# pcodec/pcodec

Hardware: AMD Instinct MI355X
Metric: encode+decode GB/s (uncompressed) per chunk, u64/f64 2^18-elem (higher is better)
Workload: dtype u64

## Files before the change

### include/pco_gfx.h

```cpp
#ifndef PCO_GFX_H
#define PCO_GFX_H

#include <stddef.h>
#include <stdint.h>

#if defined(__cplusplus)
extern "C" {
#endif


#define PCO_TYPE_U32 1
#define PCO_TYPE_U64 2
#define PCO_TYPE_I32 3
#define PCO_TYPE_I64 4
#define PCO_TYPE_F32 5
#define PCO_TYPE_F64 6
#define PCO_TYPE_U16 7
#define PCO_TYPE_I16 8
#define PCO_TYPE_F16 9
#define PCO_TYPE_U8 10
#define PCO_TYPE_I8 11

typedef enum PcoError {
  PcoSuccess,
  PcoInvalidType,
  PcoCompressionError,
  PcoDecompressionError,
} PcoError;

typedef struct PcoChunkConfig {
  unsigned int compression_level;
  size_t max_page_n;
} PcoChunkConfig;

size_t pco_standalone_guarantee_file_size(size_t n, unsigned char dtype);

enum PcoError pco_standalone_simple_compress_into(const void* nums, size_t n, unsigned char dtype,
                                                  const struct PcoChunkConfig* config, void* dst,
                                                  size_t dst_cap, size_t* n_written);

enum PcoError pco_standalone_simple_decompress_into(const void* compressed, size_t compressed_len,
                                                    unsigned char dtype, void* dst, size_t dst_cap,
                                                    size_t* n_written);


enum PcoModeSpecKind {
  PCO_MODE_AUTO = 0,
  PCO_MODE_CLASSIC = 1,
  PCO_MODE_TRY_FLOAT_MULT = 2,
  PCO_MODE_TRY_FLOAT_QUANT = 3,
  PCO_MODE_TRY_INT_MULT = 4,
  PCO_MODE_TRY_DICT = 5,
};
enum PcoDeltaSpecKind {
  PCO_DELTA_AUTO = 0,
  PCO_DELTA_NOOP = 1,
  PCO_DELTA_TRY_CONSECUTIVE = 2,
  PCO_DELTA_TRY_LOOKBACK = 3,
  PCO_DELTA_TRY_CONV1 = 4,
};
typedef struct PcoChunkConfigEx {
  uint32_t compression_level;
  uint32_t mode_kind;
  double mode_f64;
  uint64_t mode_u64;
  uint32_t delta_kind;
  uint32_t delta_order;
  uint64_t max_page_n;
  uint32_t enable_8_bit;
  uint32_t flags;
} PcoChunkConfigEx;
#define PCO_GFX_CFG_STRICT_HISTOGRAM 1u
#define PCO_GFX_CFG_CONV1 2u
#define PCO_GFX_CFG_DICT 4u

enum PcoGfxStatus {
  PCO_GFX_OK = 0,
  PCO_GFX_CORRUPTION = 1,
  PCO_GFX_INSUFFICIENT_DATA = 2,
  PCO_GFX_INVALID_ARGUMENT = 3,
  PCO_GFX_UNSUPPORTED = 4,
  PCO_GFX_DEVICE_ERROR = 5,
};
int pco_gfx_last_status(void);
const char* pco_gfx_last_error(void);
int pco_gfx_device_count(void);

enum PcoError pco_gfx_simple_compress_into_ex(const void* nums, size_t n, unsigned char dtype,
                                              const PcoChunkConfigEx* config, int uniform_type,
                                              void* dst, size_t dst_cap, size_t* n_written);
enum PcoError pco_gfx_simple_compress_into_exact(const void* nums, size_t n, unsigned char dtype, const PcoChunkConfigEx* config,
                                                 int uniform_type, const size_t* page_sizes, size_t n_pages, void* dst,
                                                 size_t dst_cap, size_t* n_written);
size_t pco_gfx_guarantee_file_size(size_t n, unsigned char dtype, uint64_t max_page_n);
size_t pco_gfx_guarantee_chunk_size(size_t n, unsigned char dtype);


typedef struct PcoGfxEncodeTask {
  const void* src;
  uint64_t n;
  void* dst;
  uint64_t dst_cap;
  uint32_t dtype;
  uint32_t reserved;
} PcoGfxEncodeTask;

typedef struct PcoGfxDecodeTask {
  const void* src;
  uint64_t src_len;
  void* dst;
  uint64_t dst_cap;
  uint32_t dtype;
  uint32_t flags;
} PcoGfxDecodeTask;
#define PCO_GFX_TASK_HAS_FILE_HEADER 1u
#define PCO_GFX_TASK_WRAPPED_PAGE 2u
#define PCO_GFX_TASK_META_ONLY 4u
#define PCO_GFX_TASK_ONE_CHUNK 8u

typedef struct PcoGfxTaskResult {
  uint64_t n_out;
  uint64_t consumed;
  uint32_t status;
  uint32_t aux;
} PcoGfxTaskResult;

enum PcoError pco_gfx_compress_chunks(size_t n_tasks, const PcoGfxEncodeTask* tasks,
                                      const PcoChunkConfigEx* config, PcoGfxTaskResult* results,
                                      PcoGfxTaskResult* d_results, void* stream);
enum PcoError pco_gfx_decompress_chunks(size_t n_tasks, const PcoGfxDecodeTask* tasks,
                                        PcoGfxTaskResult* results, PcoGfxTaskResult* d_results,
                                        void* stream);

enum PcoError pco_gfx_compact_chunks(size_t n_tasks, const PcoGfxEncodeTask* tasks, const PcoGfxTaskResult* d_results, void* d_dst,
                                     uint64_t dst_cap, uint64_t dst_offset, uint64_t* d_offsets, uint64_t* total, void* stream);

size_t pco_gfx_write_standalone_header(void* dst, size_t dst_cap, uint64_t n_hint, unsigned char uniform_dtype);
size_t pco_gfx_write_standalone_footer(void* dst, size_t dst_cap);

void pco_gfx_release_workspace(void);
size_t pco_gfx_workspace_bytes(void);
unsigned long long pco_gfx_strict_histogram_fallbacks(void);
unsigned long long pco_gfx_trail_givebacks(void);
unsigned long long pco_gfx_trail_marked(void);

void pco_gfx_profile_begin(void);
int pco_gfx_profile_end(char* names, size_t names_cap, float* ms, int cap);

typedef struct PcoGfxChunkCompressor PcoGfxChunkCompressor;
typedef struct PcoGfxChunkDecompressor PcoGfxChunkDecompressor;

size_t pco_wrapped_write_header(void* dst, size_t dst_cap);
enum PcoError pco_wrapped_read_header(const void* src, size_t len, size_t* consumed,
                                      uint8_t* major, uint8_t* minor);
enum PcoError pco_chunk_compressor_new(const void* nums, size_t n, unsigned char dtype,
                                       const PcoChunkConfigEx* config,
                                       PcoGfxChunkCompressor** out);
enum PcoError pco_chunk_compressor_new_exact(const void* nums, size_t n, unsigned char dtype, const PcoChunkConfigEx* config,
                                             const size_t* page_sizes, size_t n_pages, PcoGfxChunkCompressor** out);
size_t pco_chunk_compressor_n_pages(const PcoGfxChunkCompressor*);
size_t pco_chunk_compressor_meta_size(const PcoGfxChunkCompressor*);
size_t pco_chunk_compressor_page_size(const PcoGfxChunkCompressor*, size_t page_idx);
size_t pco_chunk_compressor_page_n(const PcoGfxChunkCompressor*, size_t page_idx);
size_t pco_chunk_compressor_meta_size_hint(const PcoGfxChunkCompressor*);
size_t pco_chunk_compressor_page_size_hint(const PcoGfxChunkCompressor*, size_t page_idx);
enum PcoError pco_chunk_compressor_write_meta(const PcoGfxChunkCompressor*, void* dst, size_t dst_cap, size_t* n_written);
enum PcoError pco_chunk_compressor_write_page(const PcoGfxChunkCompressor*, size_t page_idx, void* dst, size_t dst_cap, size_t* n_written);
void pco_chunk_compressor_free(PcoGfxChunkCompressor*);

enum PcoError pco_chunk_decompressor_new(const void* src, size_t len, unsigned char dtype,
                                         uint8_t format_major, PcoGfxChunkDecompressor** out,
                                         size_t* consumed);
enum PcoError pco_chunk_decompressor_read_page(PcoGfxChunkDecompressor*, const void* src, size_t len,
                                               size_t page_n, void* dst, size_t dst_cap,
                                               size_t* n_processed, size_t* consumed);
void pco_chunk_decompressor_free(PcoGfxChunkDecompressor*);

typedef struct PcoGfxPageDecompressor PcoGfxPageDecompressor;
enum PcoError pco_page_decompressor_new(PcoGfxChunkDecompressor*, const void* src, size_t len, size_t page_n, PcoGfxPageDecompressor** out);
enum PcoError pco_page_decompressor_read(PcoGfxPageDecompressor*, void* dst, size_t dst_len, size_t* n_processed, int* finished);
size_t pco_page_decompressor_consumed(const PcoGfxPageDecompressor*);
void pco_page_decompressor_free(PcoGfxPageDecompressor*);

typedef struct PcoGfxPageInfo {
  uint64_t offset;
  uint64_t len;
  uint64_t n;
  uint32_t status;
  uint32_t aux;
} PcoGfxPageInfo;
size_t pco_gfx_wrapped_n_pages(size_t n, uint64_t max_page_n);
size_t pco_gfx_wrapped_chunk_cap(size_t n, unsigned char dtype, const PcoChunkConfigEx* config);
enum PcoError pco_gfx_compress_wrapped_chunks(size_t n_tasks, const PcoGfxEncodeTask* tasks, const PcoChunkConfigEx* config,
                                              PcoGfxPageInfo* infos, void* stream);

typedef struct PcoGfxWrappedTask {
  const void* src;
  uint64_t n;
  void* dst;
  uint64_t dst_cap;
  uint32_t dtype;
  uint32_t n_pages;
  const uint64_t* page_sizes;
} PcoGfxWrappedTask;
size_t pco_gfx_wrapped_chunk_cap_exact(const uint64_t* page_sizes, size_t n_pages, unsigned char dtype, const PcoChunkConfigEx* config);
enum PcoError pco_gfx_compress_wrapped_chunks_ex(size_t n_tasks, const PcoGfxWrappedTask* tasks, const PcoChunkConfigEx* config,
                                                 PcoGfxPageInfo* infos, PcoGfxPageInfo* d_infos, void* stream);
size_t pco_gfx_wrapped_scratch_estimate(size_t n_tasks, const PcoGfxWrappedTask* tasks, const PcoChunkConfigEx* config);
enum PcoError pco_gfx_compact_wrapped_chunks(size_t n_tasks, const PcoGfxWrappedTask* tasks, const PcoChunkConfigEx* config,
                                             const PcoGfxPageInfo* d_infos, uint32_t gap, void* d_dst, uint64_t dst_cap, uint64_t dst_offset,
                                             uint64_t* d_offsets, uint64_t* total, void* stream);

typedef struct PcoGfxPageTask {
  const void* meta;
  uint64_t meta_len;
  const void* page;
  uint64_t page_len;
  void* dst;
  uint64_t page_n;
  uint32_t dtype;
  uint32_t format_major;
} PcoGfxPageTask;
enum PcoError pco_gfx_decompress_pages(size_t n_tasks, const PcoGfxPageTask* tasks, PcoGfxTaskResult* results,
                                       PcoGfxTaskResult* d_results, void* stream);

typedef struct PcoGfxPageRangeTask {
  const void* meta;
  uint64_t meta_len;
  const void* page;
  uint64_t page_len;
  void* dst;
  uint64_t page_n;
  uint64_t first, count;
  uint32_t dtype;
  uint32_t format_major;
} PcoGfxPageRangeTask;
enum PcoError pco_gfx_decompress_page_ranges(size_t n_tasks, const PcoGfxPageRangeTask* tasks, PcoGfxTaskResult* results,
                                             PcoGfxTaskResult* d_results, void* stream);

typedef struct PcoGfxChunkMetaInfo {
  uint32_t mode_kind;
  uint32_t mode_k;
  uint64_t mode_base_latent;
  uint32_t delta_kind;
  uint32_t delta_order;
  uint32_t window_n_log, state_n_log;
  uint32_t secondary_uses_delta;
  uint32_t n_vars_parsed;
  uint32_t present[3], ans_size_log[3], n_bins[3];
  uint64_t meta_bytes;
} PcoGfxChunkMetaInfo;
enum PcoError pco_gfx_chunk_meta_info(const void* meta, size_t len, unsigned char dtype, uint8_t format_major, PcoGfxChunkMetaInfo* out);
enum PcoError pco_chunk_compressor_meta_info(const PcoGfxChunkCompressor*, unsigned char dtype, PcoGfxChunkMetaInfo* out);
enum PcoError pco_chunk_decompressor_meta_info(const PcoGfxChunkDecompressor*, PcoGfxChunkMetaInfo* out);
enum PcoError pco_gfx_chunk_meta_conv1(const void* meta, size_t len, unsigned char dtype, uint8_t format_major, uint32_t* quantization,
                                       int64_t* bias, int32_t* weights, uint32_t* order);
enum PcoError pco_gfx_chunk_meta_dict(const void* meta, size_t len, unsigned char dtype, uint8_t format_major, uint32_t* n_unique, void* values,
                                      size_t cap);

typedef struct PcoGfxComm PcoGfxComm;
enum PcoError pco_gfx_comm_unique_id(void* id128);
enum PcoError pco_gfx_comm_init(const void* id128, int n_ranks, int rank, PcoGfxComm** out);
void pco_gfx_comm_free(PcoGfxComm*);
int pco_gfx_comm_rank(const PcoGfxComm*);
int pco_gfx_comm_size(const PcoGfxComm*);
enum PcoError pco_gfx_gather_chunks(PcoGfxComm*, int root, const void* d_stream, uint64_t n_bytes, void* d_file, uint64_t file_cap,
                                    uint64_t file_offset, uint64_t* offsets, void* stream);
enum PcoError pco_gfx_scatter_chunks(PcoGfxComm*, int root, const void* d_file, uint64_t file_offset, const uint64_t* offsets,
                                     void* d_stream, uint64_t stream_cap, uint64_t* n_bytes, void* stream);

int pco_gfx_debug_float_screen(const void* values, size_t n, uint32_t dtype, uint32_t* out);

#if defined(__cplusplus)
}
#endif
#endif
```

### pcodec_amd/_lib.py

```python
import ctypes as C
import os

HERE = os.path.dirname(os.path.abspath(__file__))
LIB_PATH = os.environ.get("PCO_GFX_LIB", os.path.join(HERE, "libpco_gfx.so"))

PcoSuccess, PcoInvalidType, PcoCompressionError, PcoDecompressionError = range(4)
ST_OK, ST_CORRUPTION, ST_INSUFFICIENT_DATA, ST_INVALID_ARGUMENT, ST_UNSUPPORTED, ST_DEVICE_ERROR = range(6)
TASK_HAS_FILE_HEADER = 1

MODE_AUTO, MODE_CLASSIC, MODE_TRY_FLOAT_MULT, MODE_TRY_FLOAT_QUANT, MODE_TRY_INT_MULT, MODE_TRY_DICT = range(6)
DELTA_AUTO, DELTA_NOOP, DELTA_TRY_CONSECUTIVE, DELTA_TRY_LOOKBACK, DELTA_TRY_CONV1 = range(5)

CFG_STRICT_HISTOGRAM = 1
CFG_CONV1 = 2
CFG_DICT = 4

DTYPE_BYTE = {"uint32": 1, "uint64": 2, "int32": 3, "int64": 4, "float32": 5, "float64": 6,
              "uint16": 7, "int16": 8, "float16": 9, "uint8": 10, "int8": 11}
DTYPE_BYTES = {1: 4, 2: 8, 3: 4, 4: 8, 5: 4, 6: 8, 7: 2, 8: 2, 9: 2, 10: 1, 11: 1}


class PcoChunkConfig(C.Structure):
    _fields_ = [("compression_level", C.c_uint), ("max_page_n", C.c_size_t)]


class PcoChunkConfigEx(C.Structure):
    _fields_ = [("compression_level", C.c_uint32), ("mode_kind", C.c_uint32), ("mode_f64", C.c_double),
                ("mode_u64", C.c_uint64), ("delta_kind", C.c_uint32), ("delta_order", C.c_uint32),
                ("max_page_n", C.c_uint64), ("enable_8_bit", C.c_uint32), ("flags", C.c_uint32)]


class EncodeTask(C.Structure):
    _fields_ = [("src", C.c_void_p), ("n", C.c_uint64), ("dst", C.c_void_p), ("dst_cap", C.c_uint64),
                ("dtype", C.c_uint32), ("reserved", C.c_uint32)]


class DecodeTask(C.Structure):
    _fields_ = [("src", C.c_void_p), ("src_len", C.c_uint64), ("dst", C.c_void_p), ("dst_cap", C.c_uint64),
                ("dtype", C.c_uint32), ("flags", C.c_uint32)]


class TaskResult(C.Structure):
    _fields_ = [("n_out", C.c_uint64), ("consumed", C.c_uint64), ("status", C.c_uint32), ("aux", C.c_uint32)]


KIND_NAMES = {ST_CORRUPTION: "Corruption", ST_INSUFFICIENT_DATA: "InsufficientData", ST_INVALID_ARGUMENT: "InvalidArgument",
              ST_UNSUPPORTED: "Unsupported", ST_DEVICE_ERROR: "DeviceError"}


class PageInfo(C.Structure):
    _fields_ = [("offset", C.c_uint64), ("len", C.c_uint64), ("n", C.c_uint64), ("status", C.c_uint32), ("aux", C.c_uint32)]


class PageTask(C.Structure):
    _fields_ = [("meta", C.c_void_p), ("meta_len", C.c_uint64), ("page", C.c_void_p), ("page_len", C.c_uint64),
                ("dst", C.c_void_p), ("page_n", C.c_uint64), ("dtype", C.c_uint32), ("format_major", C.c_uint32)]


class PageRangeTask(C.Structure):
    _fields_ = [("meta", C.c_void_p), ("meta_len", C.c_uint64), ("page", C.c_void_p), ("page_len", C.c_uint64),
                ("dst", C.c_void_p), ("page_n", C.c_uint64), ("first", C.c_uint64), ("count", C.c_uint64),
                ("dtype", C.c_uint32), ("format_major", C.c_uint32)]


class WrappedTask(C.Structure):
    _fields_ = [("src", C.c_void_p), ("n", C.c_uint64), ("dst", C.c_void_p), ("dst_cap", C.c_uint64),
                ("dtype", C.c_uint32), ("n_pages", C.c_uint32), ("page_sizes", C.c_void_p)]


class PcoGfxError(RuntimeError):

    def __init__(self, code, status, msg):
        super().__init__(f"pco error: pco {KIND_NAMES.get(status, status)} error: {msg} (libpco_gfx code={code} status={status})")
        self.code, self.status = code, status


_lib = None


def lib():
    global _lib
    if _lib is None:
        if not os.path.exists(LIB_PATH):
            raise ImportError(f"{LIB_PATH} is missing: build it with `python -m pcodec_amd.build` (needs hipcc). "
                              "pcodec_amd has no CPU fallback.")
        try:
            import torch
        except Exception:
            pass
        L = C.CDLL(LIB_PATH)
        L.pco_gfx_last_error.restype = C.c_char_p
        L.pco_standalone_guarantee_file_size.restype = C.c_size_t
        L.pco_standalone_guarantee_file_size.argtypes = [C.c_size_t, C.c_ubyte]
        L.pco_gfx_guarantee_file_size.restype = C.c_size_t
        L.pco_gfx_guarantee_file_size.argtypes = [C.c_size_t, C.c_ubyte, C.c_uint64]
        L.pco_gfx_guarantee_chunk_size.restype = C.c_size_t
        L.pco_gfx_workspace_bytes.restype = C.c_size_t
        L.pco_gfx_workspace_bytes.argtypes = []
        L.pco_gfx_strict_histogram_fallbacks.restype = C.c_ulonglong
        L.pco_gfx_strict_histogram_fallbacks.argtypes = []
        L.pco_gfx_trail_givebacks.restype = C.c_ulonglong
        L.pco_gfx_trail_givebacks.argtypes = []
        L.pco_gfx_trail_marked.restype = C.c_ulonglong
        L.pco_gfx_trail_marked.argtypes = []
        L.pco_gfx_guarantee_chunk_size.argtypes = [C.c_size_t, C.c_ubyte]
        L.pco_standalone_simple_compress_into.argtypes = [C.c_void_p, C.c_size_t, C.c_ubyte, C.c_void_p, C.c_void_p,
                                                          C.c_size_t, C.POINTER(C.c_size_t)]
        L.pco_standalone_simple_decompress_into.argtypes = [C.c_void_p, C.c_size_t, C.c_ubyte, C.c_void_p, C.c_size_t,
                                                            C.POINTER(C.c_size_t)]
        L.pco_gfx_simple_compress_into_ex.argtypes = [C.c_void_p, C.c_size_t, C.c_ubyte, C.c_void_p, C.c_int,
                                                      C.c_void_p, C.c_size_t, C.POINTER(C.c_size_t)]
        L.pco_gfx_compress_chunks.argtypes = [C.c_size_t, C.c_void_p, C.c_void_p, C.c_void_p, C.c_void_p, C.c_void_p]
        L.pco_gfx_decompress_chunks.argtypes = [C.c_size_t, C.c_void_p, C.c_void_p, C.c_void_p, C.c_void_p]
        L.pco_gfx_write_standalone_header.restype = C.c_size_t
        L.pco_gfx_write_standalone_header.argtypes = [C.c_void_p, C.c_size_t, C.c_uint64, C.c_ubyte]
        L.pco_gfx_write_standalone_footer.restype = C.c_size_t
        L.pco_gfx_write_standalone_footer.argtypes = [C.c_void_p, C.c_size_t]
        L.pco_wrapped_write_header.restype = C.c_size_t
        L.pco_wrapped_write_header.argtypes = [C.c_void_p, C.c_size_t]
        L.pco_gfx_wrapped_n_pages.restype = C.c_size_t
        L.pco_gfx_wrapped_n_pages.argtypes = [C.c_size_t, C.c_uint64]
        L.pco_gfx_wrapped_chunk_cap.restype = C.c_size_t
        L.pco_gfx_wrapped_chunk_cap.argtypes = [C.c_size_t, C.c_ubyte, C.c_void_p]
        L.pco_gfx_compress_wrapped_chunks.argtypes = [C.c_size_t, C.c_void_p, C.c_void_p, C.c_void_p, C.c_void_p]
        L.pco_gfx_decompress_pages.argtypes = [C.c_size_t, C.c_void_p, C.c_void_p, C.c_void_p, C.c_void_p]
        L.pco_gfx_decompress_page_ranges.argtypes = [C.c_size_t, C.c_void_p, C.c_void_p, C.c_void_p, C.c_void_p]
        L.pco_gfx_wrapped_chunk_cap_exact.restype = C.c_size_t
        L.pco_gfx_wrapped_chunk_cap_exact.argtypes = [C.c_void_p, C.c_size_t, C.c_ubyte, C.c_void_p]
        L.pco_gfx_compress_wrapped_chunks_ex.argtypes = [C.c_size_t, C.c_void_p, C.c_void_p, C.c_void_p, C.c_void_p, C.c_void_p]
        L.pco_gfx_wrapped_scratch_estimate.restype = C.c_size_t
        L.pco_gfx_wrapped_scratch_estimate.argtypes = [C.c_size_t, C.c_void_p, C.c_void_p]
        L.pco_gfx_compact_wrapped_chunks.argtypes = [C.c_size_t, C.c_void_p, C.c_void_p, C.c_void_p, C.c_uint32, C.c_void_p, C.c_uint64, C.c_uint64,
                                                     C.c_void_p, C.c_void_p, C.c_void_p]
        _lib = L
    return _lib


def check(code):
    if code != PcoSuccess:
        L = lib()
        raise PcoGfxError(code, L.pco_gfx_last_status(), (L.pco_gfx_last_error() or b"").decode())


def make_config(level=8, mode=MODE_AUTO, mode_f64=0.0, mode_u64=0, delta=DELTA_AUTO, delta_order=0, max_page_n=0,
                enable_8_bit=False, strict_histogram=False, conv1=False, dict=False):
    return PcoChunkConfigEx(level, mode, mode_f64, mode_u64, delta, delta_order, max_page_n, 1 if enable_8_bit else 0,
                            (CFG_STRICT_HISTOGRAM if strict_histogram else 0) | (CFG_CONV1 if conv1 else 0) | (CFG_DICT if dict else 0))


def chunk_meta_conv1(meta, dtype_byte, format_major=4):
    buf = (C.c_uint8 * max(len(meta), 1)).from_buffer_copy(bytes(meta) or b"\0")
    q, b, order, w = C.c_uint32(), C.c_int64(), C.c_uint32(), (C.c_int32 * 32)()
    rc = lib().pco_gfx_chunk_meta_conv1(buf, C.c_size_t(len(meta)), C.c_ubyte(dtype_byte), C.c_uint8(format_major), C.byref(q), C.byref(b), w,
                                        C.byref(order))
    if rc != 0:
        raise PcoGfxError(rc, lib().pco_gfx_last_status(), lib().pco_gfx_last_error().decode())
    return None if order.value == 0 else (q.value, b.value, list(w[:order.value]))


def chunk_meta_dict(meta, dtype_byte, format_major=4):
    import numpy as np
    buf = (C.c_uint8 * max(len(meta), 1)).from_buffer_copy(bytes(meta) or b"\0")
    width = {1: 4, 2: 8, 3: 4, 4: 8, 5: 4, 6: 8, 7: 2, 8: 2, 9: 2, 10: 1, 11: 1}[dtype_byte]
    cap = max(len(meta) // width, 1)
    out = np.zeros(cap, dtype={1: np.uint8, 2: np.uint16, 4: np.uint32, 8: np.uint64}[width])
    k = C.c_uint32()
    rc = lib().pco_gfx_chunk_meta_dict(buf, C.c_size_t(len(meta)), C.c_ubyte(dtype_byte), C.c_uint8(format_major), C.byref(k),
                                       out.ctypes.data_as(C.c_void_p), C.c_size_t(cap))
    if rc != 0:
        raise PcoGfxError(rc, lib().pco_gfx_last_status(), lib().pco_gfx_last_error().decode())
    return None if k.value == 0 else out[:k.value].copy()
```

### pcodec_amd/csrc/encode_kernels.hip

```cpp
#include <type_traits>

#include "pco_dev.h"

namespace pcogfx {

constexpr uint32_t kC16KeyRange = 32768u;

#ifndef PCO_LDS
#define PCO_LDS __attribute__((address_space(3)))
#endif

constexpr uint32_t kMaxUnoptBinsLog = 8;
constexpr uint32_t kMaxBins = 1u << kMaxUnoptBinsLog;
constexpr uint32_t kMaxEncTableLog = 12;
constexpr uint32_t kDirectHistRange = 4096;
constexpr uint32_t kFastEncMaxAsl = 10;

struct EncVar {
  uint32_t present, latent_bits, n_lat, lat_start;
  unsigned long long minv, maxv;
  uint32_t n_hist, n_bins, ans_size_log, max_ob;
  uint32_t is_trivial, needs_ans, hist_path, walk_pending;
};
static_assert(sizeof(EncVar) == 64, "EncVar");
struct EncChunk {
  uint64_t n;
  uint32_t dtype, status;
  uint32_t mode_kind, mode_k;
  uint64_t mode_base;
  uint64_t mode_aux;
  uint64_t mode_aux2;
  uint32_t delta_kind, delta_order, window_n_log, state_n_log;
  uint32_t fallback, unopt_bins_log;
  uint32_t n_pages, page_low, page_r, page_first;
  uint32_t fast_ok;
  uint32_t c16_ok;
  uint32_t exact_paging;
  uint32_t big;
  uint64_t c16_ref[2];
  EncVar v[3];
  uint32_t dict_dtype;
  uint32_t dict_k;
};
static_assert(sizeof(EncChunk) % 8 == 0, "EncChunk");

struct EncPage {
  uint32_t chunk, page_idx;
  uint64_t start, n;
  void* dst; uint64_t dst_cap;
  uint32_t flags, pad;
  uint64_t moments[8];
};
constexpr uint32_t kPageFlagPreamble = 1u, kPageFlagMetaOnly = 2u;

constexpr uint32_t kConv1MaxOrder = 32;
struct EncConv {
  double dots[kConv1MaxOrder + 1];
  int64_t isum;
  uint64_t vmax;
  uint64_t center;
  int64_t bias, w[kConv1MaxOrder];
  uint32_t quant, order, planned, pad;
};

struct DictTask {
  const void* src;
  uint32_t* idx;
  uint8_t* values;
  uint64_t n;
  uint32_t dtype, k;
  uint32_t hslot;
  uint32_t pad;
};

__device__ __forceinline__ uint64_t page_start_of(uint64_t i, uint32_t low, uint32_t r) {
  const uint64_t boundary = (uint64_t)r * (low + 1);
  if (i < boundary) return (i / (low + 1)) * (low + 1);
  return boundary + ((i - boundary) / low) * low;
}

constexpr uint32_t kBigBins = 1u << 12;
__host__ __device__ constexpr uint64_t plan_bytes_for(uint32_t cap) { return ((uint64_t)cap * (24 + 16 + 1) + (2ull << kMaxEncTableLog) + 63) & ~63ull; }
struct PlanRef {
  uint8_t PCO_GLOBAL* base; uint32_t cap;
  __device__ __forceinline__ uint64_t PCO_GLOBAL* hlower() const { return (uint64_t PCO_GLOBAL*)base; }
  __device__ __forceinline__ uint64_t PCO_GLOBAL* hupper() const { return (uint64_t PCO_GLOBAL*)base + cap; }
  __device__ __forceinline__ uint64_t PCO_GLOBAL* blower() const { return (uint64_t PCO_GLOBAL*)base + 2 * (uint64_t)cap; }
  __device__ __forceinline__ uint32_t PCO_GLOBAL* hcount() const { return (uint32_t PCO_GLOBAL*)(base + 24ull * cap); }
  __device__ __forceinline__ uint32_t PCO_GLOBAL* bweight() const { return (uint32_t PCO_GLOBAL*)(base + 28ull * cap); }
  __device__ __forceinline__ uint32_t PCO_GLOBAL* bcount() const { return (uint32_t PCO_GLOBAL*)(base + 32ull * cap); }
  __device__ __forceinline__ uint32_t PCO_GLOBAL* syminfo() const { return (uint32_t PCO_GLOBAL*)(base + 36ull * cap); }
  __device__ __forceinline__ uint16_t PCO_GLOBAL* next_states() const { return (uint16_t PCO_GLOBAL*)(base + 40ull * cap); }
  __device__ __forceinline__ uint8_t PCO_GLOBAL* bob() const { return (uint8_t PCO_GLOBAL*)(base + 40ull * cap + (2ull << kMaxEncTableLog)); }
};
struct EncWorkspace {
  EncChunk* chunks;
  uint8_t* plans;
  uint32_t plan_cap, pad_cap;
  EncPage* pages;
  uint8_t* lat;
  uint8_t* lat2;
  uint32_t* lat_slot;
  uint32_t* lat_used;
  uint32_t lat_cap1;
  uint32_t lat_esz;
  uint8_t* sort;
  uint8_t* walk;
  uint32_t* dissect;
  uint64_t n_stride;
  uint32_t n_slots;
  uint32_t slot_of_var[3];
  uint32_t* need_sort;
  uint32_t* need_full0;
  EncConv* conv;
  uint32_t* conv_state;
  DictTask* dict;
};

__device__ __forceinline__ uint8_t PCO_LDS* enc_lds_base() {
  extern __shared__ __attribute__((aligned(16))) uint8_t pco_lds[];
  return (uint8_t PCO_LDS*)pco_lds;
}
__device__ __forceinline__ void enc_wave_sync() {
  __builtin_amdgcn_fence(__ATOMIC_RELEASE, "workgroup");
  __builtin_amdgcn_wave_barrier();
}

__device__ __forceinline__ PlanRef plan_ref(const EncWorkspace& ws, uint32_t task, uint32_t var) {
  return PlanRef{(uint8_t PCO_GLOBAL*)ws.plans + ((uint64_t)task * 3 + var) * plan_bytes_for(ws.plan_cap), ws.plan_cap};
}
constexpr uint32_t kNoLatSlot = 0xffffffffu;
template <class L> __device__ __forceinline__ L PCO_GLOBAL* lat_ptr(const EncWorkspace& ws, uint32_t task, uint32_t var) {
  uint32_t s = ws.lat_slot[task];
  if (s == kNoLatSlot) s = 0;
  const uint64_t per_var = ws.n_stride * ws.lat_esz, per_slot = (uint64_t)ws.n_slots * per_var;
  uint8_t* base = s < ws.lat_cap1 ? ws.lat + (uint64_t)s * per_slot : ws.lat2 + (uint64_t)(s - ws.lat_cap1) * per_slot;
  return (L PCO_GLOBAL*)(base + (uint64_t)ws.slot_of_var[var] * per_var);
}
__device__ __forceinline__ uint32_t PCO_GLOBAL* dissect_ptr(const EncWorkspace& ws, uint32_t task, uint32_t var) {
  return (uint32_t PCO_GLOBAL*)(ws.dissect + ((uint64_t)task * ws.n_slots + ws.slot_of_var[var]) * ws.n_stride);
}
__device__ __forceinline__ uint16_t PCO_GLOBAL* clat_ptr(const EncWorkspace& ws, uint32_t task, uint32_t var) {
  return (uint16_t PCO_GLOBAL*)dissect_ptr(ws, task, var);
}
template <class L> __device__ __forceinline__ L PCO_GLOBAL* sort_ptr(const EncWorkspace& ws, uint32_t task, uint32_t which) {
  return (L PCO_GLOBAL*)(ws.sort + ((uint64_t)task * 2 + which) * ws.n_stride * ws.lat_esz);
}

__host__ __device__ inline uint32_t choose_unoptimized_bins_log(uint32_t level, uint64_t n) {
  const uint32_t log_n = 63u - (uint32_t)__builtin_clzll(n);
  const uint32_t fast = log_n >= 4 ? log_n - 4 : 0;
  if (level <= fast) return level;
  return fast + (level - fast) / 2;
}

struct EncModePlan {
  uint32_t mode_kind, mode_k; uint64_t mode_base, mode_aux, mode_aux2;
  uint32_t delta_kind, delta_order, window_n_log, state_n_log;
  uint32_t n_pages, page_low, page_r, page_first;
  uint32_t ubl_override, exact_paging;
};

__global__ void enc_init_kernel(EncWorkspace ws, const PcoGfxEncodeTask* tasks, const EncModePlan* plans, uint32_t n_tasks, uint32_t level, uint32_t c16_enable) {
  const uint32_t t = blockIdx.x * blockDim.x + threadIdx.x;
  if (t >= n_tasks) return;
  const PcoGfxEncodeTask task = tasks[t];
  const EncModePlan mp = plans[t];
  EncChunk c{};
  c.n = task.n; c.dtype = task.dtype; c.status = PCO_GFX_OK;
  c.mode_kind = mp.mode_kind; c.mode_k = mp.mode_k; c.mode_base = mp.mode_base; c.mode_aux = mp.mode_aux; c.mode_aux2 = mp.mode_aux2;
  c.delta_kind = mp.delta_kind; c.delta_order = mp.delta_order; c.window_n_log = mp.window_n_log; c.state_n_log = mp.state_n_log;
  c.unopt_bins_log = mp.ubl_override != 0xffffffffu ? mp.ubl_override : choose_unoptimized_bins_log(level, task.n);
  const uint32_t lbits = (uint32_t)dtype_bits(task.dtype);
  const uint32_t nlps = (mp.delta_kind == kDeltaConsecutive || mp.delta_kind == kDeltaConv1) ? mp.delta_order : (mp.delta_kind == kDeltaLookback ? (1u << mp.state_n_log) : 0u);
  const uint64_t n = task.n;
  c.n_pages = mp.n_pages; c.page_low = mp.page_low; c.page_r = mp.page_r; c.page_first = mp.page_first;
  uint64_t stored = 0;
  for (uint32_t p = 0; p < mp.n_pages; p++) { const uint64_t pn = mp.exact_paging ? ws.pages[mp.page_first + p].n : (uint64_t)(mp.page_low + (p < mp.page_r ? 1u : 0u)); stored += pn > nlps ? pn - nlps : 0; }
  c.exact_paging = mp.exact_paging;
  for (int v = 0; v < 3; v++) { c.v[v].minv = ~0ull; c.v[v].maxv = 0; }
  c.v[0].present = mp.delta_kind == kDeltaLookback; c.v[0].latent_bits = 32;
  c.v[0].lat_start = nlps; c.v[0].n_lat = (uint32_t)stored;
  c.v[1].present = 1; c.v[1].latent_bits = lbits; c.v[1].lat_start = nlps; c.v[1].n_lat = (uint32_t)stored;
  c.v[2].present = mp.mode_kind == kIntMult || mp.mode_kind == kFloatMult || mp.mode_kind == kFloatQuant;
  c.v[2].latent_bits = lbits; c.v[2].lat_start = 0; c.v[2].n_lat = (uint32_t)n;
  c.big = c.unopt_bins_log > kMaxUnoptBinsLog ? 1u : 0u;
  if (c.unopt_bins_log > 12 || (c.big && ws.plan_cap < kBigBins)) c.status = PCO_GFX_INVALID_ARGUMENT;
  c.c16_ok = c16_enable && mp.delta_kind != kDeltaLookback && mp.delta_kind != kDeltaConv1 && !c.big ? 1u : 0u;
  if (ws.dict) { c.dict_dtype = ws.dict[t].dtype; c.dict_k = ws.dict[t].k; }
  ws.chunks[t] = c;
}

struct GatherTask { const void* src; void* dst; const uint32_t* idx; uint32_t n_idx, elem_bytes; };
__global__ __launch_bounds__(256) void gather_kernel(const GatherTask* tasks, uint32_t blocks_per_task) {
  const uint32_t t = blockIdx.x / blocks_per_task;
  const GatherTask g = tasks[t];
  const uint32_t k = (blockIdx.x - t * blocks_per_task) * 256 + threadIdx.x;
  if (k >= g.n_idx) return;
  const uint32_t i = g.idx[k];
  if (g.elem_bytes == 8) ((uint64_t*)g.dst)[k] = ((const uint64_t*)g.src)[i];
  else if (g.elem_bytes == 4) ((uint32_t*)g.dst)[k] = ((const uint32_t*)g.src)[i];
  else if (g.elem_bytes == 2) ((uint16_t*)g.dst)[k] = ((const uint16_t*)g.src)[i];
  else ((uint8_t*)g.dst)[k] = ((const uint8_t*)g.src)[i];
}

struct TrialSummary {
  uint32_t status, fallback;
  uint32_t asl[2], n_bins[2], n_lat[2];
  double avg[2];
};
__global__ __launch_bounds__(64) void enc_trial_summary_kernel(EncWorkspace ws, TrialSummary* out, uint32_t n_tasks, const double* log2_of_weight) {
  const uint32_t t = blockIdx.x * 64 + threadIdx.x;
  if (t >= n_tasks) return;
  const EncChunk* ch = ws.chunks + t;
  TrialSummary o;
  o.status = ch->status; o.fallback = ch->fallback;
  for (int v = 0; v < 2; v++) {
    const PlanRef plan = plan_ref(ws, t, v);
    const uint32_t nb = ch->v[v].present ? ch->v[v].n_bins : 0, asl = ch->v[v].ans_size_log;
    o.asl[v] = asl; o.n_bins[v] = nb; o.n_lat[v] = ch->v[v].present ? ch->v[v].n_lat : 0;
    double avg = 0.0; const double tw = (double)(1ull << asl);
    for (uint32_t b = 0; b < nb; b++) {
      const uint32_t wi = plan.bweight()[b];
      const double w = (double)wi;
      avg += ((double)asl - log2_of_weight[wi] + (double)plan.bob()[b]) * w / tw;
    }
    o.avg[v] = avg;
  }
  out[t] = o;
}

template <class L, int MODE>
__device__ __forceinline__ void split_one(uint32_t num_kind, L mode_base, uint32_t mode_k, uint64_t aux_inv, uint64_t aux_base, L bits, L& p, L& s) {
  s = 0;
  if constexpr (MODE == kClassic) p = to_latent_ordered<L>(bits, num_kind);
  else if constexpr (MODE == kIntMult) { const L u = to_latent_ordered<L>(bits, num_kind); p = (L)(u / mode_base); s = (L)(u % mode_base); }
  else if constexpr (MODE == kFloatQuant) {
    const L num_ = to_latent_ordered<L>(bits, kFloat);
    const L lowmax = (L)(((L)1 << mode_k) - 1);
    p = (L)(num_ >> mode_k);
    const L low = (L)(num_ & lowmax);
    s = (bits & lmid<L>()) ? (L)(lowmax - low) : low;
  } else {
    if constexpr (sizeof(L) >= 4) {
      typedef typename FloatOf<L>::F F;
      const F num = bits_to_float(bits);
      const F inv_base = bits_to_float((L)aux_inv), base = bits_to_float((L)aux_base);
      const F mult = round_half_away(num * inv_base);
      p = int_float_to_latent<L>(mult);
      s = (L)(to_latent_ordered<L>(bits, kFloat) - to_latent_ordered<L>(float_to_bits(mult * base), kFloat) + lmid<L>());
    } else if constexpr (sizeof(L) == 2) {
      const uint32_t mult = half_round(half_mul((uint32_t)bits, (uint32_t)aux_inv));
      p = (L)half_int_float_to_latent(mult);
      s = (L)(to_latent_ordered<L>(bits, kFloat) - to_latent_ordered<L>((L)half_mul(mult, (uint32_t)aux_base), kFloat) + lmid<L>());
    } else p = 0;
  }
}

struct SplitGatherTask { const void* src; void* dst; const uint32_t* idx; uint32_t n_idx, dtype, mode_kind, mode_k; uint64_t mode_base, mode_aux, mode_aux2; };
template <class L> __device__ __forceinline__ void split_gather_one(const SplitGatherTask& g, uint32_t k, uint32_t num_kind) {
  const L bits = ((const L PCO_GLOBAL*)g.src)[g.idx[k]];
  L p = 0, s = 0;
  switch (g.mode_kind) {
    case kIntMult: split_one<L, kIntMult>(num_kind, (L)g.mode_base, g.mode_k, g.mode_aux, g.mode_aux2, bits, p, s); break;
    case kFloatMult: split_one<L, kFloatMult>(num_kind, (L)g.mode_base, g.mode_k, g.mode_aux, g.mode_aux2, bits, p, s); break;
    case kFloatQuant: split_one<L, kFloatQuant>(num_kind, (L)g.mode_base, g.mode_k, g.mode_aux, g.mode_aux2, bits, p, s); break;
    default: split_one<L, kClassic>(num_kind, (L)g.mode_base, g.mode_k, g.mode_aux, g.mode_aux2, bits, p, s); break;
  }
  ((L PCO_GLOBAL*)g.dst)[k] = p;
}
__global__ __launch_bounds__(256) void split_gather_kernel(const SplitGatherTask* tasks, uint32_t blocks_per_task) {
  const uint32_t t = blockIdx.x / blocks_per_task;
  const SplitGatherTask g = tasks[t];
  const uint32_t k = (blockIdx.x - t * blocks_per_task) * 256 + threadIdx.x;
  if (k >= g.n_idx) return;
  const uint32_t num_kind = dtype_kind(g.dtype); const int bits = dtype_bits(g.dtype);
  if (bits == 64) split_gather_one<uint64_t>(g, k, num_kind);
  else if (bits == 32) split_gather_one<uint32_t>(g, k, num_kind);
  else if (bits == 16) split_gather_one<uint16_t>(g, k, num_kind);
  else split_gather_one<uint8_t>(g, k, num_kind);
}

constexpr uint32_t kSplitE = 8, kSplitTile = 256 * kSplitE;
constexpr uint32_t kSplitLdsPrev = 0;
constexpr uint32_t kSplitLdsRed = 257 * 7 * 8;
constexpr uint32_t kSplitLdsBytes = kSplitLdsRed + 128;

template <class L, int MODE, bool kSpec>
__device__ __forceinline__ void enc_split_body(const EncWorkspace& ws, const PcoGfxEncodeTask& task, uint32_t t, EncPage PCO_GLOBAL* pg, uint32_t tile) {
  EncChunk PCO_GLOBAL* ch = (EncChunk PCO_GLOBAL*)ws.chunks + t;
  const uint64_t n = uni((uint64_t)pg->n), pstart = uni((uint64_t)pg->start);
  const uint32_t num_kind = dtype_kind(uni(task.dtype));
  const uint32_t mode_k = uni(ch->mode_k);
  const L mode_base = (L)uni((uint64_t)ch->mode_base); const uint64_t aux_inv = uni((uint64_t)ch->mode_aux), aux_base = uni((uint64_t)ch->mode_aux2);
  const uint32_t delta_kind = uni(ch->delta_kind);
  const uint32_t order = delta_kind == kDeltaConsecutive ? uni(ch->delta_order) : 0;
  constexpr bool has_sec = MODE != kClassic;
  const L PCO_GLOBAL* src = (const L PCO_GLOBAL*)task.src + pstart;
  const bool lookback = delta_kind == kDeltaLookback || delta_kind == kDeltaConv1;
  L PCO_GLOBAL* lat1 = kSpec ? nullptr : (lookback ? sort_ptr<L>(ws, t, 0) : lat_ptr<L>(ws, t, 1)) + pstart;
  L PCO_GLOBAL* lat2 = has_sec && !kSpec ? lat_ptr<L>(ws, t, 2) + pstart : nullptr;
  uint8_t PCO_LDS* smem = enc_lds_base();
  const uint32_t tid = threadIdx.x;
  const uint64_t tile0 = (uint64_t)tile * kSplitTile;
  const uint64_t e0 = tile0 + (uint64_t)tid * kSplitE;
  L raw[kSplitE], a[7 + kSplitE], sec[kSplitE];
  const bool full = e0 + kSplitE <= n;
  if (full) {
#pragma unroll
    for (uint32_t k = 0; k < kSplitE; k++) raw[k] = src[e0 + k];
  } else {
#pragma unroll
    for (uint32_t k = 0; k < kSplitE; k++) raw[k] = e0 + k < n ? src[e0 + k] : (L)0;
  }
  L halo_raw = 0;
  const bool halo_on = order > 0 && tid >= 249 && tile0 + tid >= 256 && tile0 + tid - 256 < n;
  if (halo_on) halo_raw = src[tile0 + tid - 256];
#pragma unroll
  for (uint32_t k = 0; k < kSplitE; k++) split_one<L, MODE>(num_kind, mode_base, mode_k, aux_inv, aux_base, raw[k], a[7 + k], sec[k]);
#pragma unroll
  for (uint32_t jj = 0; jj < 7; jj++) a[jj] = 0;
  if (order > 0) {
    L PCO_LDS* prevbuf = (L PCO_LDS*)(smem + kSplitLdsPrev);
#pragma unroll
    for (uint32_t jj = 0; jj < 7; jj++) if (jj + order >= 7) prevbuf[(tid + 1) * 7 + jj] = a[8 + jj];
    if (tid >= 249) { L hp = 0, hs; if (halo_on) split_one<L, MODE>(num_kind, mode_base, mode_k, aux_inv, aux_base, halo_raw, hp, hs); prevbuf[tid - 249] = hp; }
    __syncthreads();
#pragma unroll
    for (uint32_t jj = 0; jj < 7; jj++) if (jj + order >= 7) a[jj] = prevbuf[tid * 7 + jj];
    for (uint32_t r = 0; r < order; r++) {
#pragma unroll
      for (uint32_t idx = 6 + kSplitE; idx >= 1; idx--) a[idx] = (L)(a[idx] - a[idx - 1]);
    }
  }
  L mn1 = (L)~(L)0, mx1 = 0, mn2 = (L)~(L)0, mx2 = 0;
  L d[kSplitE];
  const L toggle = order > 0 ? lmid<L>() : (L)0;
#pragma unroll
  for (uint32_t k = 0; k < kSplitE; k++) d[k] = (L)(a[7 + k] + toggle);
  if (kSpec) {
  } else if (full && e0 >= order) {
#pragma unroll
    for (uint32_t k = 0; k < kSplitE; k++) {
      mn1 = d[k] < mn1 ? d[k] : mn1; mx1 = d[k] > mx1 ? d[k] : mx1;
      if (has_sec) { mn2 = sec[k] < mn2 ? sec[k] : mn2; mx2 = sec[k] > mx2 ? sec[k] : mx2; }
    }
  } else {
#pragma unroll
    for (uint32_t k = 0; k < kSplitE; k++) {
      const uint64_t i = e0 + k;
      if (i < n) {
        if (i >= order) { mn1 = d[k] < mn1 ? d[k] : mn1; mx1 = d[k] > mx1 ? d[k] : mx1; }
        if (has_sec) { mn2 = sec[k] < mn2 ? sec[k] : mn2; mx2 = sec[k] > mx2 ? sec[k] : mx2; }
      }
    }
  }
  if (lookback) { mn1 = (L)~(L)0; mx1 = 0; }
  if (kSpec) {
    constexpr L kBias = sizeof(L) == 1 ? (L)0 : (L)16384, kLmax = (L)~(L)0;
    auto clamp_ref = [&](L x) { return sizeof(L) == 1 ? (L)0 : (x < kBias ? kBias : (x > (L)(kLmax - kBias) ? (L)(kLmax - kBias) : x)); };
    L ref1 = sizeof(L) == 1 ? (L)0 : toggle, ref2 = 0;
    if (order == 0 || has_sec) { L p0, s0; split_one<L, MODE>(num_kind, mode_base, mode_k, aux_inv, aux_base, ((const L PCO_GLOBAL*)task.src)[0], p0, s0); if (order == 0) ref1 = clamp_ref(p0); ref2 = clamp_ref(s0); }
    const L lo1 = (L)(ref1 - kBias), lo2 = (L)(ref2 - kBias);
    if (pstart == 0 && e0 == 0) { ch->c16_ref[0] = (uint64_t)lo1; ch->c16_ref[1] = (uint64_t)lo2; }
    uint16_t PCO_GLOBAL* c1 = clat_ptr(ws, t, 1) + pstart;
    uint16_t PCO_GLOBAL* c2 = has_sec ? clat_ptr(ws, t, 2) + pstart : nullptr;
    uint32_t bad = 0, rmin1 = 0xffffffffu, rmax1 = 0, rmin2 = 0xffffffffu, rmax2 = 0;
    uint16_t w1[kSplitE], w2[kSplitE];
#pragma unroll
    for (uint32_t k = 0; k < kSplitE; k++) {
      const uint64_t i = e0 + k;
      const L t1 = (L)(d[k] - lo1);
      const uint32_t u1 = (uint32_t)t1;
      w1[k] = (uint16_t)u1;
      if (i < n && i >= order) { if ((uint64_t)t1 >= kC16KeyRange) bad = 1; rmin1 = u1 < rmin1 ? u1 : rmin1; rmax1 = u1 > rmax1 ? u1 : rmax1; }
      if (has_sec) {
        const L t2 = (L)(sec[k] - lo2);
        const uint32_t u2 = (uint32_t)t2;
        w2[k] = (uint16_t)u2;
        if (i < n) { if ((uint64_t)t2 >= kC16KeyRange) bad = 1; rmin2 = u2 < rmin2 ? u2 : rmin2; rmax2 = u2 > rmax2 ? u2 : rmax2; }
      }
    }
    if (full) {
      typedef uint32_t u32x4 __attribute__((ext_vector_type(4)));
      typedef u32x4 __attribute__((aligned(2))) u32x4_a2;
      static_assert(kSplitE == 8, "eight 16-bit latents per thread");
      u32x4 q1; q1.x = w1[0] | ((uint32_t)w1[1] << 16); q1.y = w1[2] | ((uint32_t)w1[3] << 16); q1.z = w1[4] | ((uint32_t)w1[5] << 16); q1.w = w1[6] | ((uint32_t)w1[7] << 16);
      *(u32x4_a2 PCO_GLOBAL*)(c1 + e0) = q1;
      if (has_sec) {
        u32x4 q2; q2.x = w2[0] | ((uint32_t)w2[1] << 16); q2.y = w2[2] | ((uint32_t)w2[3] << 16); q2.z = w2[4] | ((uint32_t)w2[5] << 16); q2.w = w2[6] | ((uint32_t)w2[7] << 16);
        *(u32x4_a2 PCO_GLOBAL*)(c2 + e0) = q2;
      }
    } else {
#pragma unroll
      for (uint32_t k = 0; k < kSplitE; k++) if (e0 + k < n) { c1[e0 + k] = w1[k]; if (has_sec) c2[e0 + k] = w2[k]; }
    }
    {
      auto umin = [](uint32_t p, uint32_t q) { return p < q ? p : q; }; auto umax = [](uint32_t p, uint32_t q) { return p > q ? p : q; };
      rmin1 = wave_reduce_u32(rmin1, umin); rmax1 = wave_reduce_u32(rmax1, umax);
      if (has_sec) { rmin2 = wave_reduce_u32(rmin2, umin); rmax2 = wave_reduce_u32(rmax2, umax); }
    }
    const uint32_t wbad = __any(bad != 0) ? 1u : 0u;
    uint32_t PCO_LDS* red32 = (uint32_t PCO_LDS*)(smem + kSplitLdsRed);
    if (lane_id() == 0) { const uint32_t w = tid >> 6; red32[w * 5 + 0] = rmin1; red32[w * 5 + 1] = rmax1; red32[w * 5 + 2] = rmin2; red32[w * 5 + 3] = rmax2; red32[w * 5 + 4] = wbad; }
    __syncthreads();
    if (tid == 0) {
      uint32_t m1 = 0xffffffffu, x1 = 0, m2 = 0xffffffffu, x2 = 0, anybad = 0;
      for (uint32_t w = 0; w < 4; w++) {
        m1 = red32[w * 5] < m1 ? red32[w * 5] : m1; x1 = red32[w * 5 + 1] > x1 ? red32[w * 5 + 1] : x1;
        m2 = red32[w * 5 + 2] < m2 ? red32[w * 5 + 2] : m2; x2 = red32[w * 5 + 3] > x2 ? red32[w * 5 + 3] : x2;
        anybad |= red32[w * 5 + 4];
      }
      if (anybad) atomicCAS(&ws.chunks[t].c16_ok, 1u, 2u);
      else {
        if (m1 <= x1) { atomicMin((unsigned long long*)&ws.chunks[t].v[1].minv, (unsigned long long)(L)(lo1 + (L)m1)); atomicMax((unsigned long long*)&ws.chunks[t].v[1].maxv, (unsigned long long)(L)(lo1 + (L)x1)); }
        if (has_sec && m2 <= x2) { atomicMin((unsigned long long*)&ws.chunks[t].v[2].minv, (unsigned long long)(L)(lo2 + (L)m2)); atomicMax((unsigned long long*)&ws.chunks[t].v[2].maxv, (unsigned long long)(L)(lo2 + (L)x2)); }
      }
    }
  } else if (full) {
#pragma unroll
    for (uint32_t k = 0; k < kSplitE; k++) lat1[e0 + k] = d[k];
    if (has_sec) {
#pragma unroll
      for (uint32_t k = 0; k < kSplitE; k++) lat2[e0 + k] = sec[k];
    }
  } else {
#pragma unroll
    for (uint32_t k = 0; k < kSplitE; k++) if (e0 + k < n) { lat1[e0 + k] = d[k]; if (has_sec) lat2[e0 + k] = sec[k]; }
  }
  if (e0 == 0 && order > 0) {
    L q[8];
    for (uint32_t jj = 0; jj < 8; jj++) {
      if (jj < order && jj < n) { L pp, ss; split_one<L, MODE>(num_kind, mode_base, mode_k, aux_inv, aux_base, src[jj], pp, ss); q[jj] = pp; } else q[jj] = 0;
    }
    for (uint32_t oo = 0; oo < order; oo++) {
      pg->moments[oo] = oo < n ? (uint64_t)q[0] : 0ull;
      for (uint32_t jj = 0; jj + 1 < 8; jj++) q[jj] = (L)(q[jj + 1] - q[jj]);
    }
  }
  if (kSpec) return;
  for (int dlt = 32; dlt >= 1; dlt >>= 1) {
    L o1 = shfl_idx(mn1, (int)(lane_id() ^ dlt)); mn1 = o1 < mn1 ? o1 : mn1;
    L o2 = shfl_idx(mx1, (int)(lane_id() ^ dlt)); mx1 = o2 > mx1 ? o2 : mx1;
    if (has_sec) {
      L o3 = shfl_idx(mn2, (int)(lane_id() ^ dlt)); mn2 = o3 < mn2 ? o3 : mn2;
      L o4 = shfl_idx(mx2, (int)(lane_id() ^ dlt)); mx2 = o4 > mx2 ? o4 : mx2;
    }
  }
  uint64_t PCO_LDS* red = (uint64_t PCO_LDS*)(smem + kSplitLdsRed);
  if (lane_id() == 0) { const uint32_t w = tid >> 6; red[w * 4 + 0] = (uint64_t)mn1; red[w * 4 + 1] = (uint64_t)mx1; red[w * 4 + 2] = (uint64_t)mn2; red[w * 4 + 3] = (uint64_t)mx2; }
  __syncthreads();
  if (tid == 0) {
    uint64_t m1 = ~0ull, x1 = 0, m2 = ~0ull, x2 = 0;
    for (uint32_t w = 0; w < 4; w++) {
      m1 = red[w * 4] < m1 ? red[w * 4] : m1; x1 = red[w * 4 + 1] > x1 ? red[w * 4 + 1] : x1;
      m2 = red[w * 4 + 2] < m2 ? red[w * 4 + 2] : m2; x2 = red[w * 4 + 3] > x2 ? red[w * 4 + 3] : x2;
    }
    if (m1 <= x1) { atomicMin((unsigned long long*)&ws.chunks[t].v[1].minv, (unsigned long long)m1); atomicMax((unsigned long long*)&ws.chunks[t].v[1].maxv, (unsigned long long)x1); }
    if (has_sec && m2 <= x2) { atomicMin((unsigned long long*)&ws.chunks[t].v[2].minv, (unsigned long long)m2); atomicMax((unsigned long long*)&ws.chunks[t].v[2].maxv, (unsigned long long)x2); }
  }
}

template <class L, bool kSpec>
__device__ __forceinline__ void enc_split_mode(const EncWorkspace& ws, const PcoGfxEncodeTask& task, uint32_t t, EncPage PCO_GLOBAL* pg, uint32_t tile, uint32_t mode_kind) {
  if (mode_kind == kClassic) enc_split_body<L, kClassic, kSpec>(ws, task, t, pg, tile);
  else if (mode_kind == kIntMult) enc_split_body<L, kIntMult, kSpec>(ws, task, t, pg, tile);
  else if (mode_kind == kFloatQuant) enc_split_body<L, kFloatQuant, kSpec>(ws, task, t, pg, tile);
  else enc_split_body<L, kFloatMult, kSpec>(ws, task, t, pg, tile);
}

template <bool kSpec, bool kLoop>
__global__ __launch_bounds__(256, kLoop ? 1 : 8) void enc_split_kernel(EncWorkspace ws, const PcoGfxEncodeTask* tasks, uint32_t tiles_per_page, uint32_t tiles_per_block, uint32_t want) {
  const uint32_t blocks_per_page = kLoop ? (tiles_per_page + tiles_per_block - 1) / tiles_per_block : tiles_per_page;
  const uint32_t page = blockIdx.x / blocks_per_page, tile0 = (blockIdx.x % blocks_per_page) * (kLoop ? tiles_per_block : 1u);
  EncPage PCO_GLOBAL* pg = (EncPage PCO_GLOBAL*)ws.pages + page;
  if (uni(pg->flags) & kPageFlagMetaOnly) return;
  const uint32_t t = uni(pg->chunk);
  if (uni(ws.chunks[t].status) != PCO_GFX_OK) return;
  if (uni(__hip_atomic_load(&ws.chunks[t].c16_ok, __ATOMIC_RELAXED, __HIP_MEMORY_SCOPE_AGENT)) != want) return;
  const PcoGfxEncodeTask task = tasks[t];
  const int bits = dtype_bits(uni(task.dtype));
  const uint32_t mode_kind = uni(ws.chunks[t].mode_kind);
  if (!kLoop) {
    if ((uint64_t)tile0 * kSplitTile >= uni((uint64_t)pg->n)) return;
    if (bits == 64) enc_split_mode<uint64_t, kSpec>(ws, task, t, pg, tile0, mode_kind);
    else if (bits == 32) enc_split_mode<uint32_t, kSpec>(ws, task, t, pg, tile0, mode_kind);
    else if (bits == 16) enc_split_mode<uint16_t, kSpec>(ws, task, t, pg, tile0, mode_kind);
    else if (bits == 8) enc_split_mode<uint8_t, kSpec>(ws, task, t, pg, tile0, mode_kind);
    return;
  }
  for (uint32_t tile = tile0; tile < tile0 + tiles_per_block && (uint64_t)tile * kSplitTile < uni((uint64_t)pg->n); tile++) {
    if (tile != tile0) __syncthreads();
    if (bits == 64) enc_split_mode<uint64_t, kSpec>(ws, task, t, pg, tile, mode_kind);
    else if (bits == 32) enc_split_mode<uint32_t, kSpec>(ws, task, t, pg, tile, mode_kind);
    else if (bits == 16) enc_split_mode<uint16_t, kSpec>(ws, task, t, pg, tile, mode_kind);
    else if (bits == 8) enc_split_mode<uint8_t, kSpec>(ws, task, t, pg, tile, mode_kind);
  }
}

template <class L, int MODE>
__device__ __forceinline__ bool presample_bad(const PcoGfxEncodeTask& task, const EncChunk PCO_GLOBAL* ch) {
  const uint32_t lane = lane_id();
  const uint32_t num_kind = dtype_kind(uni(task.dtype));
  const uint32_t mode_k = uni(ch->mode_k);
  const L mode_base = (L)uni((uint64_t)ch->mode_base); const uint64_t aux_inv = uni((uint64_t)ch->mode_aux), aux_base = uni((uint64_t)ch->mode_aux2);
  const uint32_t order = uni(ch->delta_kind) == kDeltaConsecutive ? uni(ch->delta_order) : 0;
  constexpr bool has_sec = MODE != kClassic;
  const uint64_t n = uni((uint64_t)ch->n);
  const L PCO_GLOBAL* src = (const L PCO_GLOBAL*)task.src;
  constexpr L kBias = sizeof(L) == 1 ? (L)0 : (L)16384, kLmax = (L)~(L)0;
  if (sizeof(L) == 1) return false;
  auto clamp_ref = [&](L x) { return x < kBias ? kBias : (x > (L)(kLmax - kBias) ? (L)(kLmax - kBias) : x); };
  L ref1 = order > 0 ? lmid<L>() : (L)0, ref2 = 0;
  if (order == 0 || has_sec) { L p0, s0; split_one<L, MODE>(num_kind, mode_base, mode_k, aux_inv, aux_base, src[0], p0, s0); if (order == 0) ref1 = clamp_ref(p0); ref2 = clamp_ref(s0); }
  const uint64_t pos = (uint64_t)lane * ((n - 8) / 64);
  L a[8];
  L sec_last = 0;
#pragma unroll
  for (uint32_t k = 0; k < 8; k++) { L pp = 0, ss = 0; if (k <= order) split_one<L, MODE>(num_kind, mode_base, mode_k, aux_inv, aux_base, src[pos + k], pp, ss); a[k] = pp; if (k == order) sec_last = ss; }
  for (uint32_t r = 0; r < order; r++) {
#pragma unroll
    for (uint32_t idx = 7; idx >= 1; idx--) a[idx] = (L)(a[idx] - a[idx - 1]);
  }
  L d = 0;
#pragma unroll
  for (uint32_t k = 0; k < 8; k++) if (k == order) d = a[k];
  d = (L)(d + (order > 0 ? lmid<L>() : (L)0));
  bool bad = (uint64_t)(L)(d - (L)(ref1 - kBias)) >= kC16KeyRange;
  if (has_sec) bad = bad || (uint64_t)(L)(sec_last - (L)(ref2 - kBias)) >= kC16KeyRange;
  return __any(bad) != 0;
}
template <class L>
__device__ __forceinline__ bool presample_mode(const PcoGfxEncodeTask& task, const EncChunk PCO_GLOBAL* ch, uint32_t mode_kind) {
  if (mode_kind == kClassic) return presample_bad<L, kClassic>(task, ch);
  if (mode_kind == kIntMult) return presample_bad<L, kIntMult>(task, ch);
  if (mode_kind == kFloatQuant) return presample_bad<L, kFloatQuant>(task, ch);
  return presample_bad<L, kFloatMult>(task, ch);
}
__global__ __launch_bounds__(64) void enc_presample_kernel(EncWorkspace ws, const PcoGfxEncodeTask* tasks, uint32_t n_tasks) {
  const uint32_t t = blockIdx.x;
  if (t >= n_tasks) return;
  EncChunk PCO_GLOBAL* ch = (EncChunk PCO_GLOBAL*)ws.chunks + t;
  if (uni(ch->status) != PCO_GFX_OK || uni(ch->c16_ok) != 1 || uni(ch->n_pages) != 1 || uni((uint64_t)ch->n) < 4096) return;
  const PcoGfxEncodeTask task = tasks[t];
  const int bits = dtype_bits(uni(task.dtype));
  const uint32_t mode_kind = uni(ch->mode_kind);
  bool bad = false;
  if (bits == 64) bad = presample_mode<uint64_t>(task, ch, mode_kind);
  else if (bits == 32) bad = presample_mode<uint32_t>(task, ch, mode_kind);
  else if (bits == 16) bad = presample_mode<uint16_t>(task, ch, mode_kind);
  if (bad && lane_id() == 0) { ch->c16_ok = 0; atomicAdd(ws.need_full0, 1u); }
}
__global__ __launch_bounds__(64) void enc_lat_slots_kernel(EncWorkspace ws, uint32_t n_tasks, uint32_t want) {
  const uint32_t t = blockIdx.x * blockDim.x + threadIdx.x;
  if (t >= n_tasks) return;
  if (ws.chunks[t].c16_ok != want || ws.lat_slot[t] != kNoLatSlot) return;
  ws.lat_slot[t] = atomicAdd(ws.lat_used, 1u);
}

template <uint32_t kCounts, uint32_t kRingN> struct LbCfg {
  static constexpr uint32_t kLbCountsLds = kCounts;
  static constexpr uint32_t kLbRing = kRingN;
  static constexpr uint32_t kLbLdsCounts = 0;
  static constexpr uint32_t kLbLdsHp = kCounts * 4;
  static constexpr uint32_t kLbLdsRing = kLbLdsHp + 64 * 6 * 4;
  static constexpr uint32_t kLbLdsHpOther = kLbLdsRing + kRingN * 8;
  static constexpr uint32_t kLbLdsHpCnt = kLbLdsHpOther + 64 * 6 * 8;
  static constexpr uint32_t kLbLdsBig = kLbLdsHpCnt + 64 * 6 * 4;
  static constexpr uint32_t kLbLdsBytes = kLbLdsBig + 64 * 4;
};
typedef LbCfg<1024, 1024> LbFull;
typedef LbCfg<256, 256> LbSmall;
constexpr uint32_t kLbSmallMaxPage = 8192;

struct LookbackScratch { uint32_t* hash; uint32_t* counts; };

constexpr int kLbScope = __HIP_MEMORY_SCOPE_WORKGROUP;
__device__ __forceinline__ void lb_sync() {
  __builtin_amdgcn_fence(__ATOMIC_ACQ_REL, "wavefront");
  __builtin_amdgcn_wave_barrier();
}
template <class L, class Cfg>
__device__ void lookback_page(const EncWorkspace& ws, uint32_t t, EncPage PCO_GLOBAL* pg, uint32_t PCO_GLOBAL* hash_tbl, uint32_t PCO_GLOBAL* gcounts) {
  constexpr uint32_t kLbCountsLds = Cfg::kLbCountsLds, kLbRing = Cfg::kLbRing, kLbLdsCounts = Cfg::kLbLdsCounts, kLbLdsHp = Cfg::kLbLdsHp, kLbLdsRing = Cfg::kLbLdsRing;
  constexpr uint32_t kLbLdsHpOther = Cfg::kLbLdsHpOther, kLbLdsHpCnt = Cfg::kLbLdsHpCnt, kLbLdsBig = Cfg::kLbLdsBig;
  EncChunk PCO_GLOBAL* ch = (EncChunk PCO_GLOBAL*)ws.chunks + t;
  const uint32_t lane = lane_id();
  const uint32_t wlog = uni(ch->window_n_log), state_n = 1u << uni(ch->state_n_log);
  const uint32_t window_n = 1u << wlog, hash_table_n = 2u << wlog, hash_mask = hash_table_n - 1;
  const uint32_t n = (uint32_t)uni((uint64_t)pg->n); const uint64_t pstart = uni((uint64_t)pg->start);
  const L PCO_GLOBAL* pre = sort_ptr<L>(ws, t, 0) + pstart;
  uint32_t PCO_GLOBAL* lbs = lat_ptr<uint32_t>(ws, t, 0) + pstart;
  L PCO_GLOBAL* out = lat_ptr<L>(ws, t, 1) + pstart;
  uint32_t PCO_LDS* lcounts = (uint32_t PCO_LDS*)(enc_lds_base() + kLbLdsCounts);
  uint32_t PCO_LDS* hp = (uint32_t PCO_LDS*)(enc_lds_base() + kLbLdsHp);
  uint64_t PCO_LDS* ring = (uint64_t PCO_LDS*)(enc_lds_base() + kLbLdsRing);
  uint64_t PCO_LDS* hp_other = (uint64_t PCO_LDS*)(enc_lds_base() + kLbLdsHpOther);
  uint32_t PCO_LDS* hp_cnt = (uint32_t PCO_LDS*)(enc_lds_base() + kLbLdsHpCnt);
  uint32_t PCO_LDS* big = (uint32_t PCO_LDS*)(enc_lds_base() + kLbLdsBig);
  if (lane == 0) for (uint32_t i = 0; i < state_n && i < 8; i++) pg->moments[i] = i < n ? (uint64_t)pre[i] : 0ull;
  if (n <= state_n) return;
  for (uint32_t i = lane; i < state_n; i += 64) ring[i & (kLbRing - 1)] = (uint64_t)pre[i];
  const uint32_t n_counts = window_n < n ? window_n : n;
  for (uint32_t i = lane; i < kLbCountsLds; i += 64) lcounts[i] = 1;
  for (uint32_t i = kLbCountsLds + lane; i < n_counts; i += 64) gcounts[i] = 1;
  for (uint32_t i = lane; i < 2 * hash_table_n; i += 64) hash_tbl[i] = 0;
  __threadfence_block();
  enc_wave_sync();
  auto hash_fn = [&](uint64_t x) { x = (x ^ (x >> 32)) * 11400714819323197441ull; x = x ^ (x >> 32); return (uint32_t)x & hash_mask; };
  uint32_t proposed = 1;
  if (lane < 16) proposed = (lane + 1) < state_n ? (lane + 1) : state_n;
  uint32_t best_lookback = 1, repeating_idx = 0;
  uint32_t ring_lb0 = 1, ring_lb1 = 1, ring_lb2 = 1, ring_lb3 = 1, ring_c0 = 1, ring_c1 = 1, ring_c2 = 1, ring_c3 = 1, cnt_best = 1;
  L mn1 = (L)~(L)0, mx1 = 0; uint32_t mn0 = 0xffffffffu, mx0 = 0;
  auto latent_back = [&](uint32_t i, uint32_t lb) { return lb < kLbRing - 64 ? (L)ring[(i - lb) & (kLbRing - 1)] : pre[i - lb]; };
  auto lz_of = [&](L l, L other) { const L d1 = (L)(l - other), d2 = (L)(other - l); const L dlt = d1 < d2 ? d1 : d2; return LBits<L>::v - bitlen<L>(dlt); };
  auto tile_slots = [&](uint64_t lv_, uint32_t (&slot_)[6]) {
#pragma unroll
    for (int c = 0; c < 2; c++) {
      const uint64_t bucket = lv_ >> (c == 0 ? 0 : 8);
      slot_[3 * c + 0] = c * hash_table_n + hash_fn(bucket - 1);
      slot_[3 * c + 1] = c * hash_table_n + hash_fn(bucket);
      slot_[3 * c + 2] = c * hash_table_n + hash_fn(bucket + 1);
    }
  };
  auto tile_latent = [&](uint32_t i0t) { return i0t < n && lane < n - i0t ? (uint64_t)pre[i0t + lane] : 0ull; };
  auto tile_fetch = [&](uint32_t i0t, uint64_t lv_, uint32_t (&val_)[6]) {
    const bool a = i0t < n && lane < n - i0t;
    uint32_t sl[6]; tile_slots(lv_, sl);
#pragma unroll
    for (int r = 0; r < 6; r++) val_[r] = a ? __hip_atomic_load(&hash_tbl[sl[r]], __ATOMIC_RELAXED, kLbScope) : 0u;
  };
  uint64_t pf_lv = tile_latent(state_n), pf2_lv = tile_latent(state_n + 64); uint32_t pf_val[6];
  tile_fetch(state_n, pf_lv, pf_val);
  bool pend_act = false; uint32_t pend_ie = 0; L pend_lv = 0, pend_other = 0;
  auto apply_pending = [&]() {
    if (pend_act) { const L d = (L)(pend_lv - pend_other + lmid<L>()); out[pend_ie] = d; mn1 = d < mn1 ? d : mn1; mx1 = d > mx1 ? d : mx1; }
    pend_act = false;
  };
  for (uint32_t i0 = state_n; i0 < n; i0 += 64) {
    const uint32_t tile_n = n - i0 < 64 ? n - i0 : 64;
    const bool first_tile = i0 == state_n;
    const uint32_t ie = i0 + lane;
    const bool act = lane < tile_n;
    const uint64_t lv = pf_lv;
    if (act) ring[ie & (kLbRing - 1)] = lv;
    uint32_t slot[6], val[6], plb[6];
    tile_slots(lv, slot);
#pragma unroll
    for (int r = 0; r < 6; r++) val[r] = pf_val[r];
    {
      uint64_t vote[2][8];
#pragma unroll
      for (int c = 0; c < 2; c++) {
#pragma unroll
        for (int b = 0; b < 8; b++) vote[c][b] = __ballot(act && ((slot[3 * c + 1] >> b) & 1u));
      }
      const uint64_t earlier = __ballot(act) & (((uint64_t)1 << lane) - 1);
      uint64_t cand[6];
#pragma unroll
      for (int r = 0; r < 6; r++) {
        uint64_t m = earlier;
#pragma unroll
        for (int b = 0; b < 8; b++) m &= ((slot[r] >> b) & 1u) ? vote[r / 3][b] : ~vote[r / 3][b];
        cand[r] = act ? m : 0ull;
      }
      for (;;) {
        bool any = false;
#pragma unroll
        for (int r = 0; r < 6; r++) any = any || cand[r] != 0;
        if (!__any(any)) break;
#pragma unroll
        for (int r = 0; r < 6; r++) {
          const uint32_t j = cand[r] ? 63u - (uint32_t)__builtin_clzll(cand[r]) : 0u;
          const uint32_t theirs = (uint32_t)__shfl((int)slot[3 * (r / 3) + 1], (int)j, 64);
          if (cand[r]) {
            if (theirs == slot[r]) { val[r] = i0 + j; cand[r] = 0; }
            else cand[r] &= ~((uint64_t)1 << j);
          }
        }
      }
    }
    if (act) { (void)__hip_atomic_fetch_max(&hash_tbl[slot[1]], ie, __ATOMIC_RELAXED, kLbScope); (void)__hip_atomic_fetch_max(&hash_tbl[slot[4]], ie, __ATOMIC_RELAXED, kLbScope); }
    pf_lv = pf2_lv; pf2_lv = tile_latent(i0 + 128);
    tile_fetch(i0 + 64, pf_lv, pf_val);
#pragma unroll
    for (int r = 0; r < 6; r++) {
      const uint32_t lb = ie - val[r];
      const uint32_t pidx = 10 + r;
      plb[r] = lb <= window_n ? lb : (pidx < ie ? pidx : ie);
    }
    uint32_t my_lb = 1;
    if (first_tile) {
#pragma unroll
      for (int r = 0; r < 6; r++) {
        hp[lane * 6 + r] = plb[r];
        if (act && plb[r] >= kLbRing - 64) hp_other[lane * 6 + r] = (uint64_t)pre[ie - plb[r]];
        if (act && plb[r] - 1 >= kLbCountsLds) hp_cnt[lane * 6 + r] = __hip_atomic_load(&gcounts[plb[r] - 1], __ATOMIC_RELAXED, kLbScope);
      }
      uint32_t n_big = 0;
      lb_sync();
      for (uint32_t e = 0; e < tile_n; e++) {
        const uint32_t i = i0 + e;
        const L l = (L)ring[i & (kLbRing - 1)];
// ... 285 lines not shown
  const uint64_t n64 = n_lat;
  auto c_count = [&](uint32_t b) { return (uint32_t)((((uint64_t)b + 1) * n64 + B - 1) >> bins_log); };
  const bool mine_ok = tid >= B || ren[tid] <= c_count(tid);
  const bool simple = __syncthreads_and(mine_ok && n_lat >= B) != 0;
  if (simple) {
    if (tid < B) {
      const uint32_t c0 = tid == 0 ? 0u : c_count(tid - 1), c1 = c_count(tid);
      plan.hcount()[tid] = c1 - c0; plan.hlower()[tid] = (uint64_t)(tid == 0 ? first_value : rnext[tid - 1]); plan.hupper()[tid] = (uint64_t)rv[tid];
    }
    if (tid == 0) { ev->n_hist = B; ev->hist_path = path; }
  } else {
    uint32_t p6[6] = {0, 0, 0, 0, 0, 0};
    if (tid < B) hist_precompute(tid, n_lat, bins_log, rst[tid], ren[tid], p6);
    if (defer != nullptr) {
      if (tid < B) {
        uint32_t PCO_GLOBAL* g32 = (uint32_t PCO_GLOBAL*)defer;
#pragma unroll
        for (uint32_t k = 0; k < 6; k++) g32[k * 256 + tid] = p6[k];
        g32[6 * 256 + tid] = rst[tid]; g32[7 * 256 + tid] = ren[tid];
        uint64_t PCO_GLOBAL* g64 = (uint64_t PCO_GLOBAL*)(defer + 8192);
        g64[tid] = (uint64_t)rv[tid]; g64[256 + tid] = (uint64_t)rnext[tid]; g64[512 + tid] = (uint64_t)rpred[tid]; g64[768 + tid] = (uint64_t)rsucc[tid];
      }
      if (tid == 0) { ev->hist_path = path; ev->walk_pending = 1u; }
      return;
    }
    if (tid < B) hist_pack_record(pre, tid, p6, rst[tid], ren[tid], (uint64_t)rv[tid], (uint64_t)rnext[tid], (uint64_t)rpred[tid], (uint64_t)rsucc[tid]);
    __syncthreads();
    if (tid == 0) { const uint32_t nh = hist_walk_rec<L>(n_lat, first_value, pre, plan); ev->n_hist = nh; ev->hist_path = path; }
  }
}

constexpr uint32_t kHistLdsRecV = 0;
constexpr uint32_t kHistLdsCounts = 4 * 2048 + 2 * 1024 + 2048;
constexpr uint32_t kWideHistRange = 32768, kMidHistRange = 16384;
constexpr uint32_t kSelBucketsLog = 13, kSelBuckets = 1u << kSelBucketsLog, kSelMaxNeeded = 1600;
constexpr uint32_t kSmallHistCap = 8192;
__host__ __device__ constexpr uint32_t hist_lds_bytes(uint32_t range) { return kHistLdsCounts + (range + 8) * 4; }
constexpr uint32_t kHistLdsBytes = hist_lds_bytes(kDirectHistRange);
constexpr uint32_t kHistSortLdsBytes = kHistLdsCounts + (2048 + kSelBuckets + 8 + kSelBuckets / 32 + 2 * (kSelMaxNeeded + 1)) * 4;

template <bool B> struct BoolC { static constexpr bool value = B; };
__device__ __forceinline__ void hist_count(uint32_t PCO_LDS* counts, uint32_t c, bool on, bool aggregate) {
  if (!aggregate) { if (on) atomicAdd((uint32_t*)&counts[c], 1u); return; }
  const uint64_t act = __ballot(on);
  if (act == 0) return;
  const uint32_t c0 = (uint32_t)__builtin_amdgcn_readlane((int)c, (int)__builtin_ctzll(act));
  const uint64_t same = __ballot(on && c == c0);
  if (on) {
    if (c != c0) atomicAdd((uint32_t*)&counts[c], 1u);
    else if ((same & (((uint64_t)1 << lane_id()) - 1)) == 0) atomicAdd((uint32_t*)&counts[c0], (uint32_t)__popcll(same));
  }
}

template <class L, uint32_t T, uint32_t R, bool kWide, bool kSort>
__device__ void hist_var(const EncWorkspace& ws, uint32_t t, uint32_t var, uint32_t bins_log) {
  EncChunk PCO_GLOBAL* ch = (EncChunk PCO_GLOBAL*)ws.chunks + t;
  EncVar PCO_GLOBAL* ev = &ch->v[var];
  const PlanRef plan = plan_ref(ws, t, var);
  const uint32_t tid = threadIdx.x, lane = lane_id(), wave = tid >> 6;
  const uint32_t n_lat = ev->n_lat;
  if (n_lat == 0) { if (tid == 0) ev->n_hist = 0; return; }
  const L minv = (L)ev->minv, maxv = (L)ev->maxv;
  const L range = (L)(maxv - minv);
  if (!kSort && !kWide && ch->big != 0 && tid == 0) atomicOr(ws.need_sort, 1u);
  if (!kSort && !kWide && ch->big == 0 && (uint64_t)range >= kDirectHistRange && tid == 0) atomicOr(ws.need_sort, n_lat <= kSmallHistCap ? 8u : ((uint64_t)range >= kWideHistRange ? 1u : ((uint64_t)range >= kMidHistRange ? 4u : 2u)));
  const bool big = ch->big != 0;
  if (!kSort && big) return;
  if (!big && (kWide || kSort) && n_lat <= kSmallHistCap) return;
  if (!big && (kSort ? (uint64_t)range < kWideHistRange : (kWide ? ((uint64_t)range < (R == kWideHistRange ? kMidHistRange : kDirectHistRange) || (uint64_t)range >= R) : (uint64_t)range >= kDirectHistRange))) return;
  if (kSort && !big && ev->hist_path != 2) return;
  const L PCO_GLOBAL* lat = lat_ptr<L>(ws, t, var);
  const uint32_t n_all = (uint32_t)ch->n, skip = ev->lat_start, plow = ch->page_low, pr = ch->page_r;
  const bool single_page = ch->n_pages == 1;
  const bool exact_paging = ch->exact_paging != 0; const uint32_t n_pg = ch->n_pages;
  const EncPage PCO_GLOBAL* pgl = (const EncPage PCO_GLOBAL*)ws.pages + ch->page_first;
  auto exact_start = [&](uint32_t i) {
    uint32_t lo = 0, hi = n_pg;
    while (hi - lo > 1) { const uint32_t mid = (lo + hi) >> 1; if ((uint64_t)pgl[mid].start <= i) lo = mid; else hi = mid; }
    return (uint64_t)pgl[lo].start;
  };
  auto stored = [&](uint32_t i) { return skip == 0 || (single_page ? i >= skip : (uint64_t)i - (exact_paging ? exact_start(i) : page_start_of(i, plow, pr)) >= skip); };
  uint8_t PCO_LDS* smem = enc_lds_base();
  uint32_t PCO_LDS* counts = (uint32_t PCO_LDS*)(smem + kHistLdsCounts);
  L PCO_LDS* rv = (L PCO_LDS*)(smem + kHistLdsRecV);
  L PCO_LDS* rnext = (L PCO_LDS*)(smem + kHistLdsRecV + 2048);
  L PCO_LDS* rpred = (L PCO_LDS*)(smem + kHistLdsRecV + 4096);
  L PCO_LDS* rsucc = (L PCO_LDS*)(smem + kHistLdsRecV + 6144);
  uint32_t PCO_LDS* rst = (uint32_t PCO_LDS*)(smem + kHistLdsRecV + 8192);
  uint32_t PCO_LDS* ren = (uint32_t PCO_LDS*)(smem + kHistLdsRecV + 9216);
  uint32_t PCO_LDS* scan = (uint32_t PCO_LDS*)(smem + kHistLdsRecV + 10240);
  const uint32_t B = 1u << bins_log;
  const uint64_t n64 = n_lat;
  auto c_count = [&](uint32_t b) { return (uint32_t)((((uint64_t)b + 1) * n64 + B - 1) >> bins_log); };
  __syncthreads();
  if ((uint64_t)range < R && !big) {
    constexpr uint32_t PER = R / T;
    for (uint32_t i = tid; i < R + 8; i += T) counts[i] = 0;
    __syncthreads();
    {
      uint16_t PCO_GLOBAL* clat = clat_ptr(ws, t, var);
      const bool agg = uni((uint32_t)(((uint64_t)range < 256 || var == 0) ? 1u : 0u)) != 0;
      const bool c16 = uni(ch->c16_ok) == 1 && var != 0;
      const uint16_t c16_off = (uint16_t)((uint64_t)minv - (uint64_t)ch->c16_ref[var == 2 ? 1 : 0]);
      auto count_all = [&](auto agg_c) {
        constexpr bool kAgg = decltype(agg_c)::value;
        uint32_t base = 0;
        if (c16) {
          if (((uint64_t)(uintptr_t)clat & 15u) == 0 && n_all >= 8 * T) {
            typedef uint32_t u32x4 __attribute__((ext_vector_type(4)));
            const u32x4 PCO_GLOBAL* c4 = (const u32x4 PCO_GLOBAL*)clat;
            const uint32_t n_it = n_all / (8 * T);
            auto fetch = [&](uint32_t it) { return c4[(uint64_t)(it < n_it ? it : n_it - 1) * T + tid]; };
            u32x4 cur = fetch(0), nx1 = fetch(1);
            for (uint32_t it = 0; it < n_it; it++) {
              const u32x4 nx2 = fetch(it + 2);
              const uint32_t w[4] = {cur[0], cur[1], cur[2], cur[3]};
#pragma unroll
              for (uint32_t k = 0; k < 8; k++) {
                const uint32_t c = (uint32_t)(uint16_t)(((k & 1u) ? w[k >> 1] >> 16 : w[k >> 1]) - c16_off);
                hist_count(counts, c, c < R, kAgg);
              }
              cur = nx1; nx1 = nx2;
            }
            base = n_it * 8 * T;
          }
          for (; base + 8 * T <= n_all; base += 8 * T) {
            uint16_t x[8];
#pragma unroll
            for (int k = 0; k < 8; k++) x[k] = clat[base + k * T + tid];
#pragma unroll
            for (int k = 0; k < 8; k++) { const uint32_t c = (uint32_t)(uint16_t)(x[k] - c16_off); hist_count(counts, c, c < R, kAgg); }
          }
        } else {
          for (; base + 8 * T <= n_all; base += 8 * T) {
            L x[8];
#pragma unroll
            for (int k = 0; k < 8; k++) x[k] = lat[base + k * T + tid];
#pragma unroll
            for (int k = 0; k < 8; k++) {
              const L d = (L)(x[k] - minv);
              clat[base + k * T + tid] = (uint16_t)d;
              hist_count(counts, (uint32_t)d, (uint64_t)d < R, kAgg);
            }
          }
        }
        for (uint32_t i0 = base; i0 < n_all; i0 += T) {
          const uint32_t i = i0 + tid;
          const uint64_t d = i < n_all ? (c16 ? (uint64_t)(uint16_t)(clat[i] - c16_off) : (uint64_t)(L)(lat[i] - minv)) : 0ull;
          if (i < n_all && !c16) clat[i] = (uint16_t)d;
          hist_count(counts, (uint32_t)d, i < n_all && d < R, kAgg);
        }
      };
      const bool constant16 = (uint64_t)range == 0 && c16;
      if (constant16) { if (tid == 0) counts[0] = n_lat; }
      else if (agg) count_all(BoolC<true>{}); else count_all(BoolC<false>{});
      if (skip != 0 && !constant16) {
        __syncthreads();
        for (uint32_t q = tid; q < n_pg * skip; q += T) {
          const uint32_t pi = q / skip, j = q - pi * skip;
          const uint64_t pst = pgl[pi].start;
          if (j < (uint64_t)pgl[pi].n) {
            const uint64_t d = c16 ? (uint64_t)(uint16_t)(clat[pst + j] - c16_off) : (uint64_t)(L)(lat[pst + j] - minv);
            if (d < R) atomicSub((uint32_t*)&counts[(uint32_t)d], 1u);
          }
        }
      }
    }
    __syncthreads();
    uint32_t s = 0;
    for (uint32_t k = 0; k < PER; k++) s += counts[tid * PER + k];
    uint32_t incl = wave_incl_scan(s);
    if (lane == 63) scan[wave] = incl;
    __syncthreads();
    uint32_t wbase = 0; for (uint32_t w = 0; w < wave; w++) wbase += scan[w];
    uint32_t run = wbase + incl - s;
    for (uint32_t k = 0; k < PER; k++) { const uint32_t c = counts[tid * PER + k]; counts[tid * PER + k] = run; run += c; }
    if (tid == T - 1) counts[R] = run;
    __syncthreads();
    auto lookup = [&](uint32_t r, L& value, uint32_t& st, uint32_t& en) {
      uint32_t lo = 0, hi = R;
      while (hi - lo > 1) { const uint32_t mid = (lo + hi) >> 1; if (counts[mid] <= r) lo = mid; else hi = mid; }
      value = (L)(minv + (L)lo); st = counts[lo]; en = counts[lo + 1];
    };
    if (tid < B) {
      const uint32_t c = c_count(tid);
      L v; uint32_t st, en; lookup(c - 1, v, st, en);
      rv[tid] = v; rst[tid] = st; ren[tid] = en;
      L x; uint32_t a, b2;
      if (c < n_lat) { lookup(c, x, a, b2); rnext[tid] = x; } else rnext[tid] = 0;
      if (st > 0) { lookup(st - 1, x, a, b2); rpred[tid] = x; } else rpred[tid] = 0;
      if (en < n_lat) { lookup(en, x, a, b2); rsucc[tid] = x; } else rsucc[tid] = 0;
    }
    __syncthreads();
    hist_emit<L>(n_lat, bins_log, minv, rv, rst, ren, rnext, rpred, rsucc, plan, ev, 0u, (uint32_t PCO_LDS*)(smem + kHistLdsCounts),
                 ws.walk != nullptr ? (uint8_t PCO_GLOBAL*)ws.walk + ((uint64_t)t * 3 + var) * kWalkRecBytes : (uint8_t PCO_GLOBAL*)nullptr);
    __syncthreads();
    return;
  }
  if constexpr (!kSort) return;
  if constexpr (kSort) {
  constexpr uint32_t NB = kSelBuckets;
  const uint32_t sig_bits = bitlen<L>(range);
  const uint32_t bshift = sig_bits > kSelBucketsLog ? sig_bits - kSelBucketsLog : 0u;
  const uint32_t npass = sig_bits == 0 ? 1u : (sig_bits + 7) / 8;
  L PCO_GLOBAL* bufA = sort_ptr<L>(ws, t, 0);
  L PCO_GLOBAL* bufB = sort_ptr<L>(ws, t, 1);
  uint32_t PCO_LDS* cnt = counts;
  uint32_t PCO_LDS* cursor = counts + 1024;
  uint32_t PCO_LDS* P = counts + 2048;
  uint32_t PCO_LDS* need = P + NB + 8;
  uint32_t PCO_LDS* nl_k = need + NB / 32;
  uint32_t PCO_LDS* nl_oc = nl_k + kSelMaxNeeded;
  auto bucket_of = [&](L x) { return (uint32_t)((L)(x - minv) >> bshift); };
  for (uint32_t i = tid; i < NB + 8; i += 256) P[i] = 0;
  for (uint32_t i = tid; i < NB / 32; i += 256) need[i] = 0;
  __syncthreads();
  {
    uint32_t base = 0;
    for (; base + 8 * 256 <= n_all; base += 8 * 256) {
      L x[8];
#pragma unroll
      for (int k = 0; k < 8; k++) x[k] = lat[base + k * 256 + tid];
#pragma unroll
      for (int k = 0; k < 8; k++) if (stored(base + k * 256 + tid)) atomicAdd((uint32_t*)&P[bucket_of(x[k])], 1u);
    }
    for (uint32_t i = base + tid; i < n_all; i += 256) if (stored(i)) atomicAdd((uint32_t*)&P[bucket_of(lat[i])], 1u);
  }
  __syncthreads();
  {
    constexpr uint32_t PER = NB / 256;
    uint32_t s0 = 0;
    for (uint32_t k = 0; k < PER; k++) s0 += P[tid * PER + k];
    const uint32_t incl = wave_incl_scan(s0);
    if (lane == 63) scan[wave] = incl;
    __syncthreads();
    uint32_t wbase = 0; for (uint32_t w = 0; w < wave; w++) wbase += scan[w];
    uint32_t run = wbase + incl - s0;
    for (uint32_t k = 0; k < PER; k++) { const uint32_t c = P[tid * PER + k]; P[tid * PER + k] = run; run += c; }
    if (tid == 255) P[NB] = run;
  }
  __syncthreads();
  auto bucket_of_rank = [&](uint32_t r) {
    uint32_t lo = 0, hi = NB;
    while (hi - lo > 1) { const uint32_t mid = (lo + hi) >> 1; if (P[mid] <= r) lo = mid; else hi = mid; }
    return lo;
  };
  for (uint32_t bq = tid; bq < B; bq += 256) {
    const uint32_t c = c_count(bq);
    for (uint32_t which = 0; which < 2; which++) {
      const uint32_t r = c - 1 + which;
      if (r >= n_lat) continue;
      const uint32_t k = bucket_of_rank(r);
      atomicOr((uint32_t*)&need[k >> 5], 1u << (k & 31));
      if (P[k] > 0) { const uint32_t kp = bucket_of_rank(P[k] - 1); atomicOr((uint32_t*)&need[kp >> 5], 1u << (kp & 31)); }
      if (P[k + 1] < n_lat) { const uint32_t kn = bucket_of_rank(P[k + 1]); atomicOr((uint32_t*)&need[kn >> 5], 1u << (kn & 31)); }
    }
  }
  __syncthreads();
  uint32_t n_need = 0, n_sub = 0;
  {
    const uint32_t word = need[tid];
    uint32_t nb_here = __popc(word), el_here = 0;
    for (uint32_t w = word; w; w &= w - 1) { const uint32_t k = tid * 32 + (uint32_t)__builtin_ctz(w); el_here += P[k + 1] - P[k]; }
    const uint32_t i_nb = wave_incl_scan(nb_here), i_el = wave_incl_scan(el_here);
    if (lane == 63) { scan[wave] = i_nb; scan[16 + wave] = i_el; }
    __syncthreads();
    uint32_t b_nb = 0, b_el = 0; for (uint32_t w = 0; w < wave; w++) { b_nb += scan[w]; b_el += scan[16 + w]; }
    uint32_t slot = b_nb + i_nb - nb_here, off = b_el + i_el - el_here;
    for (uint32_t w = word; w; w &= w - 1) {
      const uint32_t k = tid * 32 + (uint32_t)__builtin_ctz(w);
      if (slot < kSelMaxNeeded) { nl_k[slot] = k; nl_oc[slot] = off; }
      slot++; off += P[k + 1] - P[k];
    }
    n_need = scan[0] + scan[1] + scan[2] + scan[3]; n_sub = scan[16] + scan[17] + scan[18] + scan[19];
  }
  __syncthreads();
  if (tid == 0) nl_oc[n_need < kSelMaxNeeded ? n_need : kSelMaxNeeded] = n_sub;
  const bool subset = n_need <= kSelMaxNeeded;
  auto needed = [&](L x) { const uint32_t k = bucket_of(x); return !subset || ((need[k >> 5] >> (k & 31)) & 1u) != 0; };
  const uint32_t n_sort = subset ? n_sub : n_lat;
  __syncthreads();
  if (subset) {
    uint32_t PCO_LDS* fill = scan + 32;
    if (tid == 0) *fill = 0;
    __syncthreads();
    auto gather_group = [&](uint32_t i, L x, bool in_range) {
      const bool act = in_range && stored(i) && needed(x);
      const uint64_t m = __ballot(act);
      if (m == 0) return;
      uint32_t base0 = 0;
      if (lane == 0) base0 = atomicAdd((uint32_t*)fill, (uint32_t)__popcll(m));
      base0 = (uint32_t)__builtin_amdgcn_readfirstlane((int)base0);
      if (act) bufB[base0 + __popcll(m & (((uint64_t)1 << lane) - 1))] = x;
    };
    uint32_t i0 = 0;
    for (; i0 + 8 * 256 <= n_all; i0 += 8 * 256) {
      L x[8];
#pragma unroll
      for (int k = 0; k < 8; k++) x[k] = lat[i0 + 256 * k + tid];
#pragma unroll
      for (int k = 0; k < 8; k++) gather_group(i0 + 256 * k + tid, x[k], true);
    }
    for (; i0 < n_all; i0 += 256) { const uint32_t i = i0 + tid; gather_group(i, i < n_all ? lat[i] : (L)0, i < n_all); }
    __threadfence_block();
    __syncthreads();
  }
  for (uint32_t p = 0; p < npass; p++) {
    const L PCO_GLOBAL* in = p == 0 ? (subset ? bufB : lat) : ((p & 1) ? bufA : bufB);
    L PCO_GLOBAL* out = (p & 1) ? bufB : bufA;
    const uint32_t shift = 8 * p;
    const bool raw0 = p == 0 && !subset;
    const uint32_t n_in = raw0 ? n_all : n_sort;
    const uint32_t q = (n_in + 3) / 4;
    const uint32_t w_begin = wave * q < n_in ? wave * q : n_in;
    const uint32_t w_end = (wave + 1) * q < n_in ? (wave + 1) * q : n_in;
    for (uint32_t i = tid; i < 1024; i += 256) cnt[i] = 0;
// ... 903 lines not shown
```

### pcodec_amd/csrc/pco_gfx.hip

```cpp
#include "pco_host.h"
#include "pco_half.h"

#include <algorithm>
#include <atomic>
#include <chrono>
#include <thread>
#include <mutex>
#include <condition_variable>
#include <functional>
#include <sched.h>
#include <pthread.h>
#include <sys/syscall.h>
#include <unistd.h>
#include <cstdlib>
#include <cstring>
#include <memory>
#include <unordered_map>

#include "pco_auto_host.inc"
#include "decode_kernel.hip"
#include "decode_trail.hip"
#include "encode_kernels.hip"
#include "encode_lookback.hip"
#include "encode_conv1.hip"
// ... 150 lines not shown
    d_sym = (uint8_t*)ws.dec_sym.ensure(n_tasks * 3 * sym_stride + 64);
    d_offpos = (uint64_t*)ws.dec_offpos.ensure(n_tasks * 3 * offpos_stride * 8);
  }
  const uint32_t need_hist = results ? kStatusNeedHist : (uint32_t)PCO_GFX_UNSUPPORTED;
  for (int g = 0; g < 4; g++) {
    if (ids[g].empty()) continue;
    const uint32_t cnt = (uint32_t)ids[g].size();
    const uint32_t grid = (uint32_t)std::min<size_t>(cnt, kGeneralGrid);
    const uint32_t* idp = mixed ? d_ids + id_off[g] : nullptr;
    const uint32_t* filt = fast ? (const uint32_t*)d_plans : nullptr;
    const uint32_t fstride = (uint32_t)(sizeof(DecPlan) / 4);
    if (fast) {
      const uint32_t n_wb = (cnt + 7) / 8;
      uint32_t* d_progress = nullptr;
      uint32_t* d_givebacks = nullptr;
      constexpr uint32_t kTrailMinChunks = 1024;
      const bool use_trail = g_decode_trail && (cnt >= kTrailMinChunks || g_trail_debug != '\0' || g_trail_always);
      if (use_trail) {
        ensure_side_stream(ws);
        d_progress = (uint32_t*)ws.dec_progress.ensure((size_t)n_wb * kTrailProgressStride * sizeof(uint32_t));
        PCO_HIP_CHECK(hipMemsetAsync(d_progress, 0, (size_t)n_wb * kTrailProgressStride * sizeof(uint32_t), stream));
        if (!ws.dec_stats.p) { ws.dec_stats.ensure(256); PCO_HIP_CHECK(hipMemsetAsync(ws.dec_stats.p, 0, 256, stream)); }
        d_givebacks = (uint32_t*)ws.dec_stats.p;
      }
      const uint32_t trail_grid = use_trail ? std::min<uint32_t>(n_wb, (uint32_t)ws.n_cus * 4u) : 0u;
#define PCO_FAST_DECODE(L, name)                                                                                                                          \
      {                                                                                                                                                   \
        static const bool _walk_ok = hipFuncSetAttribute((const void*)dec_walk_kernel<L, 8>, hipFuncAttributeMaxDynamicSharedMemorySize, (int)(4 * WalkCfg<8>::kWalkLdsBytes)) == hipSuccess && \
                                     hipFuncSetAttribute((const void*)dec_walk_kernel<L, 4>, hipFuncAttributeMaxDynamicSharedMemorySize, (int)(4 * WalkCfg<4>::kWalkLdsBytes)) == hipSuccess;   \
        if (!_walk_ok) throw HostError{PCO_GFX_DEVICE_ERROR, "cannot reserve LDS for dec_walk_kernel"};                                                   \
      }                                                                                                                                                   \
      if (use_trail) {                                                                                                                                    \
        ScopedKernelTimer _span("dec_walk+trail<" name ">", stream);                                                                                      \
        if (g_trail_debug == 'd') {    \
          hipLaunchKernelGGL((dec_trail_kernel<L, false>), dim3(trail_grid), dim3(64 * kTrailWaves), 0, stream, d_tasks, idp, cnt, d_plans, d_bins, d_sym, sym_stride, d_offpos, offpos_stride, d_progress, n_wb, d_metas); \
          hipLaunchKernelGGL((dec_trail_kernel<L, true>), dim3(trail_grid), dim3(64 * kTrailWaves), 0, stream, d_tasks, idp, cnt, d_plans, d_bins, d_sym, sym_stride, d_offpos, offpos_stride, d_progress, n_wb, d_metas);  \
        }                                                                                                                                                 \
        PCO_HIP_CHECK(hipEventRecord(ws.fork_event, stream));                                                                                             \
                              \
        static const bool _quad_ok = hipFuncSetAttribute((const void*)dec_walk_trail_kernel<L>, hipFuncAttributeMaxDynamicSharedMemorySize, (int)(4 * WalkCfg<8>::kWalkLdsBytes)) == hipSuccess; \
        if (!_quad_ok) throw HostError{PCO_GFX_DEVICE_ERROR, "cannot reserve LDS for dec_walk_trail_kernel"};                                             \
        PCO_TIMED_LAUNCH("~dec_walk_kernel<" name ">", stream, (dec_walk_trail_kernel<L>), dim3((n_wb + 3) / 4), dim3(256), 4 * WalkCfg<8>::kWalkLdsBytes, stream, \
                         d_tasks, idp, cnt, d_plans, d_bins, d_sym, sym_stride, d_offpos, offpos_stride, d_results, d_progress, d_metas);                 \
                  \
        PCO_HIP_CHECK(hipStreamWaitEvent(ws.side_stream2, ws.fork_event, 0));                                                                             \
        PCO_TIMED_LAUNCH("~dec_walk_kernel(rest)<" name ">", ws.side_stream2, (dec_walk_kernel<L, 8>), dim3((n_wb + 3) / 4), dim3(256), 4 * WalkCfg<8>::kWalkLdsBytes, ws.side_stream2, \
                         d_tasks, idp, cnt, d_plans, d_bins, d_sym, sym_stride, d_offpos, offpos_stride, 0u, d_results, d_progress, d_metas);             \
        PCO_HIP_CHECK(hipEventRecord(ws.join_event2, ws.side_stream2));                                                                                   \
        hipStream_t ts = g_trail_debug == 's' ? stream : ws.side_stream;                                                                                  \
        PCO_HIP_CHECK(hipStreamWaitEvent(ws.side_stream, ws.fork_event, 0));                                                                              \
                                                                 \
        if (g_trail_debug != 'n' && g_trail_debug != 'd') PCO_TIMED_LAUNCH("~dec_trail_kernel<" name ">", ts, (dec_trail_kernel<L, false>), dim3(trail_grid), dim3(64 * kTrailWaves), 0, ts, \
                         d_tasks, idp, cnt, d_plans, d_bins, d_sym, sym_stride, d_offpos, offpos_stride, d_progress, n_wb, d_metas);                               \
        if (g_trail_debug != 'n' && g_trail_debug != 'd') PCO_TIMED_LAUNCH("~dec_trail2_kernel<" name ">", ts, (dec_trail_kernel<L, true>), dim3(trail_grid), dim3(64 * kTrailWaves), 0, ts, \
                         d_tasks, idp, cnt, d_plans, d_bins, d_sym, sym_stride, d_offpos, offpos_stride, d_progress, n_wb, d_metas);                               \
        PCO_HIP_CHECK(hipEventRecord(ws.join_event, ws.side_stream));                                                                                     \
        PCO_HIP_CHECK(hipStreamWaitEvent(stream, ws.join_event, 0));                                                                                      \
        PCO_HIP_CHECK(hipStreamWaitEvent(stream, ws.join_event2, 0));                                                                                     \
      } else PCO_TIMED_LAUNCH("dec_walk_kernel<" name ">", stream, (dec_walk_kernel<L, 8>), dim3((n_wb + 3) / 4), dim3(256), 4 * WalkCfg<8>::kWalkLdsBytes, stream, \
                       d_tasks, idp, cnt, d_plans, d_bins, d_sym, sym_stride, d_offpos, offpos_stride, 0u, d_results, (uint32_t*)nullptr, d_metas);       \
      PCO_TIMED_LAUNCH("dec_walk4_kernel<" name ">", stream, (dec_walk_kernel<L, 4>), dim3((cnt + 15) / 16), dim3(256), 4 * WalkCfg<4>::kWalkLdsBytes, stream, \
                       d_tasks, idp, cnt, d_plans, d_bins, d_sym, sym_stride, d_offpos, offpos_stride, kStatusRetryK4, d_results, (uint32_t*)nullptr, d_metas); \
      PCO_TIMED_LAUNCH("dec_expand_kernel<" name ">", stream, (dec_expand_kernel<L, false>), dim3(grid), dim3(256), kExpLdsBytes, stream,               \
                       d_tasks, d_results, idp, cnt, d_plans, d_bins, d_sym, sym_stride, d_offpos, offpos_stride, (const uint32_t*)d_progress, d_givebacks);    \
      PCO_TIMED_LAUNCH("dec_expand_lb_kernel<" name ">", stream, (dec_expand_kernel<L, true>), dim3(grid), dim3(256), kExpLbLdsBytes, stream,           \
                       d_tasks, d_results, idp, cnt, d_plans, d_bins, d_sym, sym_stride, d_offpos, offpos_stride, (const uint32_t*)d_progress, d_givebacks);
      if (g == 0) { PCO_FAST_DECODE(uint64_t, "u64") } else if (g == 1) { PCO_FAST_DECODE(uint32_t, "u32") } else if (g == 2) { PCO_FAST_DECODE(uint16_t, "u16") } else { PCO_FAST_DECODE(uint8_t, "u8") }
#undef PCO_FAST_DECODE
    }
    if (g == 0) PCO_TIMED_LAUNCH("pco_decode_kernel<u64>", stream, pco_decode_kernel<uint64_t>, dim3(grid), dim3(64), g_decode_lds_bytes, stream, d_tasks, d_results, idp, cnt, budget, tbl, filt, fstride, kStatusRetryLegacy, (uint8_t*)nullptr, (const uint64_t*)nullptr, need_hist, d_metas);
    else if (g == 1) PCO_TIMED_LAUNCH("pco_decode_kernel<u32>", stream, pco_decode_kernel<uint32_t>, dim3(grid), dim3(64), g_decode_lds_bytes, stream, d_tasks, d_results, idp, cnt, budget, tbl, filt, fstride, kStatusRetryLegacy, (uint8_t*)nullptr, (const uint64_t*)nullptr, need_hist, d_metas);
    else if (g == 2) PCO_TIMED_LAUNCH("pco_decode_kernel<u16>", stream, pco_decode_kernel<uint16_t>, dim3(grid), dim3(64), g_decode_lds_bytes, stream, d_tasks, d_results, idp, cnt, budget, tbl, filt, fstride, kStatusRetryLegacy, (uint8_t*)nullptr, (const uint64_t*)nullptr, need_hist, d_metas);
    else PCO_TIMED_LAUNCH("pco_decode_kernel<u8>", stream, pco_decode_kernel<uint8_t>, dim3(grid), dim3(64), g_decode_lds_bytes, stream, d_tasks, d_results, idp, cnt, budget, tbl, filt, fstride, kStatusRetryLegacy, (uint8_t*)nullptr, (const uint64_t*)nullptr, need_hist, d_metas);
    PCO_HIP_CHECK(hipGetLastError());
  }
  if (results) {
    PCO_HIP_CHECK(hipMemcpyAsync(results, d_results, n_tasks * sizeof(PcoGfxTaskResult), hipMemcpyDeviceToHost, stream));
    PCO_HIP_CHECK(hipStreamSynchronize(stream));
    std::vector<uint32_t> again[4]; size_t n_again = 0;
    for (size_t i = 0; i < n_tasks; i++) if (results[i].status == kStatusNeedHist) {
      const int b = dtype_bits(tasks[i].dtype);
      again[b == 64 ? 0 : (b == 32 ? 1 : (b == 16 ? 2 : 3))].push_back((uint32_t)i); n_again++;
    }
    if (n_again) {
      std::vector<uint32_t> flat_ids; std::vector<uint64_t> offs; uint64_t hist_bytes = 0;
      size_t goff[4];
      for (int g = 0; g < 4; g++) { goff[g] = flat_ids.size(); for (uint32_t i : again[g]) { flat_ids.push_back(i); offs.push_back(hist_bytes); hist_bytes += ((tasks[i].dst_cap * (uint64_t)(dtype_bits(tasks[i].dtype) / 8)) + 255) & ~(uint64_t)255; } }
      uint8_t* d_hist = (uint8_t*)ws.dec_hist.ensure(hist_bytes + n_again * 12 + 256);
      uint64_t* d_hoff = (uint64_t*)(d_hist + ((hist_bytes + 15) & ~(uint64_t)15));
      uint32_t* d_again = (uint32_t*)(d_hoff + n_again);
      PCO_HIP_CHECK(hipMemcpyAsync(d_hoff, offs.data(), n_again * 8, hipMemcpyHostToDevice, stream));
      PCO_HIP_CHECK(hipMemcpyAsync(d_again, flat_ids.data(), n_again * 4, hipMemcpyHostToDevice, stream));
      uint8_t* tbl2 = (uint8_t*)ws.tbl_ws.ensure(std::min<size_t>(n_again, kGeneralGrid) * kTblWsBytes);
      for (int g = 0; g < 4; g++) {
        if (again[g].empty()) continue;
        const uint32_t cnt = (uint32_t)again[g].size(), grid = (uint32_t)std::min<size_t>(cnt, kGeneralGrid);
        const uint32_t* idp = d_again + goff[g]; const uint64_t* hop = d_hoff + goff[g];
        if (g == 0) PCO_TIMED_LAUNCH("pco_decode_kernel<u64>", stream, pco_decode_kernel<uint64_t>, dim3(grid), dim3(64), g_decode_lds_bytes, stream, d_tasks, d_results, idp, cnt, budget, tbl2, (const uint32_t*)nullptr, 0u, 0u, d_hist, hop, (uint32_t)PCO_GFX_UNSUPPORTED, d_metas);
        else if (g == 1) PCO_TIMED_LAUNCH("pco_decode_kernel<u32>", stream, pco_decode_kernel<uint32_t>, dim3(grid), dim3(64), g_decode_lds_bytes, stream, d_tasks, d_results, idp, cnt, budget, tbl2, (const uint32_t*)nullptr, 0u, 0u, d_hist, hop, (uint32_t)PCO_GFX_UNSUPPORTED, d_metas);
        else if (g == 2) PCO_TIMED_LAUNCH("pco_decode_kernel<u16>", stream, pco_decode_kernel<uint16_t>, dim3(grid), dim3(64), g_decode_lds_bytes, stream, d_tasks, d_results, idp, cnt, budget, tbl2, (const uint32_t*)nullptr, 0u, 0u, d_hist, hop, (uint32_t)PCO_GFX_UNSUPPORTED, d_metas);
        else PCO_TIMED_LAUNCH("pco_decode_kernel<u8>", stream, pco_decode_kernel<uint8_t>, dim3(grid), dim3(64), g_decode_lds_bytes, stream, d_tasks, d_results, idp, cnt, budget, tbl2, (const uint32_t*)nullptr, 0u, 0u, d_hist, hop, (uint32_t)PCO_GFX_UNSUPPORTED, d_metas);
      }
      PCO_HIP_CHECK(hipGetLastError());
      PCO_HIP_CHECK(hipMemcpyAsync(results, d_results, n_tasks * sizeof(PcoGfxTaskResult), hipMemcpyDeviceToHost, stream));
      PCO_HIP_CHECK(hipStreamSynchronize(stream));
    }
  }
}

}

using namespace pcogfx;

extern "C" {

int pco_gfx_last_status(void) { return g_err.status; }
const char* pco_gfx_last_error(void) { return g_err.msg.c_str(); }
int pco_gfx_device_count(void) { int n = 0; if (hipGetDeviceCount(&n) != hipSuccess) return 0; return n; }
void pco_gfx_release_workspace(void) {
  try { Workspace& w = workspace(); if (w.has_last && w.last_event) (void)hipEventSynchronize(w.last_event); w.release_all(); } catch (...) {}
}

size_t pco_gfx_workspace_bytes(void) {
  try {
    static const bool trace = std::getenv("PCO_GFX_TRACE") != nullptr;
    if (trace) fprintf(stderr, "[pco_gfx trace] workspace: %s\n", workspace().device_report().c_str());
    return workspace().device_bytes();
  } catch (...) { return 0; }
}

static unsigned long long trail_stat(int which) {
  try {
    Workspace& w = workspace();
    const unsigned long long acc = which == 0 ? w.acc_givebacks : w.acc_marked;
    if (!w.dec_stats.p) return acc;
    if (w.has_last && w.last_event) (void)hipEventSynchronize(w.last_event);
    uint32_t v[2] = {0, 0};
    if (hipMemcpy(v, w.dec_stats.p, 8, hipMemcpyDeviceToHost) != hipSuccess) return acc;
    return acc + v[which];
  } catch (...) { return 0; }
}
unsigned long long pco_gfx_trail_givebacks(void) { return trail_stat(0); }
unsigned long long pco_gfx_trail_marked(void) { return trail_stat(1); }
unsigned long long pco_gfx_strict_histogram_fallbacks(void) {
  try {
    Workspace& w = workspace();
    if (!w.enc_strict.p) return w.acc_strict;
    if (w.has_last && w.last_event) (void)hipEventSynchronize(w.last_event);
    uint32_t v = 0;
    if (hipMemcpy(&v, w.enc_strict.p, 4, hipMemcpyDeviceToHost) != hipSuccess) return w.acc_strict;
    return w.acc_strict + v;
  } catch (...) { return 0; }
}

void pco_gfx_profile_begin(void) {
  for (auto& r : g_prof.recs) { g_prof.give(r.a); g_prof.give(r.b); }
  g_prof.recs.clear(); g_prof.on = true;
}
int pco_gfx_profile_end(char* names, size_t names_cap, float* ms, int cap) {
  g_prof.on = false;
  int n = 0; size_t pos = 0;
  for (auto& r : g_prof.recs) {
    float t = 0.f;
    (void)hipEventSynchronize(r.b);
    (void)hipEventElapsedTime(&t, r.a, r.b);
    if (n < cap) {
      const size_t len = std::strlen(r.name) + 1;
      if (names && pos + len <= names_cap) { std::memcpy(names + pos, r.name, len); pos += len; }
      if (ms) ms[n] = t;
      n++;
    }
    g_prof.give(r.a); g_prof.give(r.b);
  }
  g_prof.recs.clear();
  return n;
}

size_t pco_gfx_guarantee_file_size(size_t n, unsigned char dtype, uint64_t max_page_n) {
  const int bits = dtype_bits(dtype);
  if (!bits) return 0;
  std::vector<size_t> pages;
  n_per_page(max_page_n, n, pages);
  size_t res = guarantee_standalone_header_size() + 1;
  for (size_t p : pages) res += guarantee_standalone_chunk_size(bits, p);
  return res;
}
size_t pco_standalone_guarantee_file_size(size_t n, unsigned char dtype) { return pco_gfx_guarantee_file_size(n, dtype, 0); }
size_t pco_gfx_guarantee_chunk_size(size_t n, unsigned char dtype) {
  const int bits = dtype_bits(dtype);
  return bits ? guarantee_standalone_chunk_size(bits, n) : 0;
}

size_t pco_gfx_write_standalone_header(void* dst, size_t dst_cap, uint64_t n_hint, unsigned char uniform_dtype) {
  HostBitWriter w;
  w.write(0x216f6370u, 32); w.write(3, 8); w.write(uniform_dtype, 8);
  const uint32_t power = n_hint == 0 ? 1 : (64 - (uint32_t)__builtin_clzll(n_hint));
  w.write(power - 1, kBitsVarintPower); w.write(n_hint, power); w.finish_byte();
  w.write(4, 8); w.write(1, 8);
  if (w.bytes() > dst_cap) return 0;
  std::memcpy(dst, w.buf.data(), w.bytes());
  return w.bytes();
}
size_t pco_gfx_write_standalone_footer(void* dst, size_t dst_cap) {
  if (dst_cap < 1) return 0;
  *(uint8_t*)dst = 0;
  return 1;
}
size_t pco_wrapped_write_header(void* dst, size_t dst_cap) {
  if (dst_cap < 2) return 0;
  ((uint8_t*)dst)[0] = 4; ((uint8_t*)dst)[1] = 1;
  return 2;
}
enum PcoError pco_wrapped_read_header(const void* src, size_t len, size_t* consumed, uint8_t* major, uint8_t* minor) {
  clear_error();
  const uint8_t* p = (const uint8_t*)src;
  if (len < 1) { set_error(PCO_GFX_INSUFFICIENT_DATA, "empty header"); return PcoDecompressionError; }
  uint8_t mj = p[0], mn = 0; size_t used = 1;
  if (mj >= 4) { if (len < 2) { set_error(PCO_GFX_INSUFFICIENT_DATA, "short header"); return PcoDecompressionError; } mn = p[1]; used = 2; }
  if (mj > 4) { set_error(PCO_GFX_CORRUPTION, "file's format version definitely cannot be decompressed"); return PcoDecompressionError; }
  if (consumed) *consumed = used; if (major) *major = mj; if (minor) *minor = mn;
  return PcoSuccess;
}

enum PcoError pco_gfx_decompress_chunks(size_t n_tasks, const PcoGfxDecodeTask* tasks, PcoGfxTaskResult* results,
                                        PcoGfxTaskResult* d_results, void* stream) {
  clear_error();
  try {
    require_device();
    { WorkspaceUse use(workspace(), (hipStream_t)stream); launch_decode(n_tasks, tasks, results, d_results, (hipStream_t)stream); }
    if (results) for (size_t i = 0; i < n_tasks; i++) if (results[i].status != PCO_GFX_OK) {
      set_error((int)results[i].status, "decode task " + std::to_string(i) + " failed");
      return PcoDecompressionError;
    }
    return PcoSuccess;
  } catch (const HostError& e) { return fail_with(e, PcoDecompressionError); }
}

enum PcoError pco_gfx_decompress_pages(size_t n_tasks, const PcoGfxPageTask* tasks, PcoGfxTaskResult* results, PcoGfxTaskResult* d_results, void* stream) {
  clear_error();
  try {
    require_device();
    std::vector<PcoGfxDecodeTask> dt(n_tasks); std::vector<MetaRef> refs(n_tasks);
    for (size_t i = 0; i < n_tasks; i++) {
      const PcoGfxPageTask& t = tasks[i];
      if (t.format_major > 4) throw HostError{PCO_GFX_CORRUPTION, "page task " + std::to_string(i) + ": the file's format version definitely cannot be decompressed"};
      if (t.meta == nullptr || t.page == nullptr) throw HostError{PCO_GFX_INVALID_ARGUMENT, "page task " + std::to_string(i) + ": null ChunkMeta or page"};
      dt[i] = PcoGfxDecodeTask{t.page, t.page_len, t.dst, t.page_n, t.dtype, PCO_GFX_TASK_WRAPPED_PAGE | (t.format_major << 8)};
      refs[i] = MetaRef{t.meta, t.meta_len};
    }
    { WorkspaceUse use(workspace(), (hipStream_t)stream); launch_decode(n_tasks, dt.data(), results, d_results, (hipStream_t)stream, refs.data()); }
    if (results) for (size_t i = 0; i < n_tasks; i++) if (results[i].status != PCO_GFX_OK) {
      set_error((int)results[i].status, "page task " + std::to_string(i) + " failed");
      return PcoDecompressionError;
    }
    return PcoSuccess;
  } catch (const HostError& e) { return fail_with(e, PcoDecompressionError); }
}

enum PcoError pco_gfx_compact_chunks(size_t n_tasks, const PcoGfxEncodeTask* tasks, const PcoGfxTaskResult* d_results, void* d_dst,
                                     uint64_t dst_cap, uint64_t dst_offset, uint64_t* d_offsets, uint64_t* total, void* stream_) {
  clear_error();
  try {
    require_device();
    hipStream_t stream = (hipStream_t)stream_;
    if (!d_results || !d_offsets || (!d_dst && dst_cap)) throw HostError{PCO_GFX_INVALID_ARGUMENT, "compact: null device array"};
    if (n_tasks >= (1ull << 31)) throw HostError{PCO_GFX_INVALID_ARGUMENT, "compact: too many chunks"};
    Workspace& ws = workspace();
    WorkspaceUse use(ws, stream);
    uint8_t* d_base = (uint8_t*)ws.compact_tasks.ensure(n_tasks * sizeof(PcoGfxEncodeTask) + 64);
    uint32_t* d_over = (uint32_t*)d_base; PcoGfxEncodeTask* d_tasks = (PcoGfxEncodeTask*)(d_base + 64);
    uint64_t max_cap = 0;
    for (size_t i = 0; i < n_tasks; i++) max_cap = std::max<uint64_t>(max_cap, tasks[i].dst_cap);
    if (n_tasks) PCO_HIP_CHECK(hipMemcpyAsync(d_tasks, tasks, n_tasks * sizeof(PcoGfxEncodeTask), hipMemcpyHostToDevice, stream));
    PCO_TIMED_LAUNCH("compact_scan_kernel", stream, compact_scan_kernel, dim3(1), dim3(1024), 0, stream, d_results, (uint32_t)n_tasks, dst_offset, dst_cap, d_offsets, d_over);
    if (n_tasks) {
      const uint64_t slice = 64 * 1024;
      const uint32_t slices = (uint32_t)std::max<uint64_t>(1, (max_cap + slice - 1) / slice);
      if ((uint64_t)slices * n_tasks >= (1ull << 31)) throw HostError{PCO_GFX_INVALID_ARGUMENT, "compact: too many chunks for one call"};
      PCO_TIMED_LAUNCH("compact_copy_kernel", stream, compact_copy_kernel, dim3((uint32_t)(slices * n_tasks)), dim3(256), 0, stream, d_tasks, d_results, d_offsets, (uint8_t*)d_dst, d_over, (uint32_t)n_tasks, slice, slices);
    }
    PCO_HIP_CHECK(hipGetLastError());
    if (total) {
      uint32_t over = 0;
      PCO_HIP_CHECK(hipMemcpyAsync(total, d_offsets + n_tasks, 8, hipMemcpyDeviceToHost, stream));
      PCO_HIP_CHECK(hipMemcpyAsync(&over, d_over, 4, hipMemcpyDeviceToHost, stream));
      PCO_HIP_CHECK(hipStreamSynchronize(stream));
      if (over) throw HostError{PCO_GFX_INVALID_ARGUMENT, "compact: destination too small"};
    }
    return PcoSuccess;
  } catch (const HostError& e) { return fail_with(e, PcoCompressionError); }
}

static bool parse_standalone_header_host(const uint8_t* p, size_t len, unsigned char dtype, size_t& off, uint32_t& fmt_major) {
  if (len < 6 || p[0] != 'p' || p[1] != 'c' || p[2] != 'o' || p[3] != '!') return false;
  const uint32_t sv = p[4];
  if (sv < 2 || sv > 3) return false;
  size_t pos = 5;
  if (sv >= 3) { const uint32_t uniform = p[pos++]; if (uniform != 0 && uniform != dtype) return false; }
  if (pos + 9 > len) return false;
  uint64_t bits = 0; for (int i = 0; i < 9 && i < 8; i++) bits |= (uint64_t)p[pos + i] << (8 * i);
  const uint32_t power = 1 + (uint32_t)(bits & 63u);
  const uint32_t vbits = kBitsVarintPower + power, vbytes = (vbits + 7) / 8;
  if (vbits & 7) {
    const uint32_t last = p[pos + vbytes - 1];
    if ((last >> (vbits & 7)) != 0) return false;
  }
// ... 87 lines not shown
```

### pcodec_amd/csrc/pco_gfx_encode_api.inc

```
namespace pcogfx {

struct ResolvedConfig {
  uint32_t level;
  uint32_t mode_kind; double mode_f64; uint64_t mode_u64;
  uint32_t delta_kind, delta_order;
  uint64_t max_page_n; bool enable_8_bit;
  bool strict_hist;
  bool conv1 = false;
  bool dict = false;
  DictTask* d_dict = nullptr;
  uint32_t unknown_flags = 0;
};

static bool g_strict_hist_env = env_is_one("PCO_GFX_STRICT_HISTOGRAM");
static ResolvedConfig resolve_config(const PcoChunkConfigEx* c) {
  ResolvedConfig r{8, PCO_MODE_AUTO, 0.0, 0, PCO_DELTA_AUTO, 0, 1u << 18, true, g_strict_hist_env};
  if (c) {
    r.level = c->compression_level; r.mode_kind = c->mode_kind; r.mode_f64 = c->mode_f64; r.mode_u64 = c->mode_u64;
    r.delta_kind = c->delta_kind; r.delta_order = c->delta_order; r.max_page_n = c->max_page_n ? c->max_page_n : (1u << 18);
    r.enable_8_bit = c->enable_8_bit != 0;
    r.strict_hist = g_strict_hist_env || (c->flags & PCO_GFX_CFG_STRICT_HISTOGRAM) != 0;
    r.conv1 = (c->flags & PCO_GFX_CFG_CONV1) != 0;
    r.dict = (c->flags & PCO_GFX_CFG_DICT) != 0;
    r.unknown_flags = c->flags & ~(uint32_t)(PCO_GFX_CFG_STRICT_HISTOGRAM | PCO_GFX_CFG_CONV1 | PCO_GFX_CFG_DICT);
  }
  return r;
}

static void validate_config(const ResolvedConfig& c, int latent_bits) {
  if (c.unknown_flags) throw HostError{PCO_GFX_INVALID_ARGUMENT, "PcoChunkConfigEx::flags holds bits this library does not know (zero-initialise the struct)"};
  if (c.level > 12) throw HostError{PCO_GFX_INVALID_ARGUMENT, "compression level may not exceed 12"};
  if (c.delta_kind == PCO_DELTA_TRY_CONSECUTIVE && c.delta_order > 7) throw HostError{PCO_GFX_INVALID_ARGUMENT, "consecutive delta order may not exceed 7"};
  if (c.delta_kind == PCO_DELTA_TRY_CONV1 && !c.conv1) throw HostError{PCO_GFX_UNSUPPORTED, "Conv1 delta encoding is outside the hot-path scope"};
  if (c.delta_kind == PCO_DELTA_TRY_CONV1) {
    if (c.delta_order > kConv1MaxOrder) throw HostError{PCO_GFX_INVALID_ARGUMENT, "conv1 delta order may not exceed 32 (was " + std::to_string(c.delta_order) + ")"};
    if (latent_bits > 32) throw HostError{PCO_GFX_INVALID_ARGUMENT, "Conv1 delta encoding is only supported for types with 32 or fewer bits"};
  }
  if (c.delta_kind > PCO_DELTA_TRY_CONV1 || c.mode_kind > PCO_MODE_TRY_DICT) throw HostError{PCO_GFX_INVALID_ARGUMENT, "unknown mode / delta spec"};
  if (c.mode_kind == PCO_MODE_TRY_DICT && !c.dict) throw HostError{PCO_GFX_UNSUPPORTED, "Dict mode is outside the hot-path scope"};
  if (c.mode_kind == PCO_MODE_TRY_DICT && c.delta_kind == PCO_DELTA_TRY_CONV1) throw HostError{PCO_GFX_UNSUPPORTED, "Conv1 delta on Dict mode is outside the hot-path scope"};
  if (latent_bits == 8 && !c.enable_8_bit) throw HostError{PCO_GFX_INVALID_ARGUMENT, "compressing 8-bit types with Pco is often a mistake; enable them on the ChunkConfig"};
}

static void plan_mode_explicit(EncModePlan& p, const ResolvedConfig& c, uint32_t dtype) {
  const uint32_t kind = dtype_kind(dtype); const int bits = dtype_bits(dtype);
  p.ubl_override = 0xffffffffu;
  switch (c.mode_kind) {
    case PCO_MODE_CLASSIC: p.mode_kind = kClassic; break;
    case PCO_MODE_TRY_INT_MULT: {
      if (kind == kFloat) throw HostError{PCO_GFX_INVALID_ARGUMENT, "unable to use int mult mode on floats"};
      p.mode_kind = kIntMult; p.mode_base = bits == 64 ? c.mode_u64 : (bits == 32 ? (uint64_t)(uint32_t)c.mode_u64 : (bits == 16 ? (uint64_t)(uint16_t)c.mode_u64 : (uint64_t)(uint8_t)c.mode_u64));
      if (p.mode_base == 0) throw HostError{PCO_GFX_INVALID_ARGUMENT, "The chosen mode was invalid for the number type"};
      break;
    }
    case PCO_MODE_TRY_FLOAT_MULT: {
      if (kind != kFloat) throw HostError{PCO_GFX_INVALID_ARGUMENT, "unable to use float mode for ints"};
      p.mode_kind = kFloatMult;
      if (bits == 64) {
        const double base = c.mode_f64, inv = 1.0 / base;
        if (!std::isfinite(base) || base == 0.0) throw HostError{PCO_GFX_INVALID_ARGUMENT, "The chosen mode was invalid for the number type"};
        uint64_t b; std::memcpy(&b, &base, 8); p.mode_aux2 = b; uint64_t iv; std::memcpy(&iv, &inv, 8); p.mode_aux = iv;
        p.mode_base = (b & (1ull << 63)) ? ~b : (b ^ (1ull << 63));
      } else if (bits == 32) {
        const float base = (float)c.mode_f64, inv = 1.0f / base;
        if (!std::isfinite(base) || base == 0.0f) throw HostError{PCO_GFX_INVALID_ARGUMENT, "The chosen mode was invalid for the number type"};
        uint32_t b; std::memcpy(&b, &base, 4); p.mode_aux2 = b; uint32_t iv; std::memcpy(&iv, &inv, 4); p.mode_aux = iv;
        p.mode_base = (b & 0x80000000u) ? (uint32_t)~b : (b ^ 0x80000000u);
      } else {
        const F16 base = F16::from_f64(c.mode_f64), inv = F16(1.0) / base;
        if ((base.bits & 0x7c00u) == 0x7c00u || (base.bits & 0x7fffu) == 0) throw HostError{PCO_GFX_INVALID_ARGUMENT, "The chosen mode was invalid for the number type"};
        p.mode_aux2 = base.bits; p.mode_aux = inv.bits;
        p.mode_base = (base.bits & 0x8000u) ? (uint16_t)~base.bits : (uint16_t)(base.bits ^ 0x8000u);
      }
      break;
    }
    case PCO_MODE_TRY_FLOAT_QUANT: {
      if (kind != kFloat) throw HostError{PCO_GFX_INVALID_ARGUMENT, "unable to use float mode for ints"};
      const uint32_t prec = bits == 64 ? 52 : (bits == 32 ? 23 : 10);
      if (c.mode_u64 == 0 || c.mode_u64 > prec) throw HostError{PCO_GFX_INVALID_ARGUMENT, "The chosen mode was invalid for the number type"};
      p.mode_kind = kFloatQuant; p.mode_k = (uint32_t)c.mode_u64; break;
    }
    default: throw HostError{PCO_GFX_INVALID_ARGUMENT, "ModeSpec::Auto must be resolved before planning"};
  }
}
static uint32_t lookback_window_log(uint64_t n) {
  const uint32_t m = (uint32_t)n - 1; const uint32_t b = m == 0 ? 0 : 32 - (uint32_t)__builtin_clz(m);
  return b < 4 ? 4 : (b > 15 ? 15 : b);
}
static void plan_delta_explicit(EncModePlan& p, const ResolvedConfig& c, uint64_t n) {
  p.delta_kind = kDeltaNone; p.delta_order = 0; p.window_n_log = 0; p.state_n_log = 0;
  switch (c.delta_kind) {
    case PCO_DELTA_NOOP: p.delta_kind = kDeltaNone; break;
    case PCO_DELTA_TRY_CONSECUTIVE: if (c.delta_order == 0) p.delta_kind = kDeltaNone; else { p.delta_kind = kDeltaConsecutive; p.delta_order = c.delta_order; } break;
    case PCO_DELTA_TRY_LOOKBACK: p.delta_kind = kDeltaLookback; p.window_n_log = lookback_window_log(n); p.state_n_log = 0; break;
    case PCO_DELTA_TRY_CONV1:
      if (c.delta_order == 0) p.delta_kind = kDeltaNone; else { p.delta_kind = kDeltaConv1; p.delta_order = c.delta_order; }
      break;
    default: throw HostError{PCO_GFX_INVALID_ARGUMENT, "DeltaSpec::Auto must be resolved before planning"};
  }
}

static const bool g_trace = std::getenv("PCO_GFX_TRACE") != nullptr;
struct TracePhase {
  const char* name; hipStream_t stream; std::chrono::steady_clock::time_point t0;
  TracePhase(const char* n, hipStream_t s) : name(n), stream(s) { if (g_trace) { (void)hipStreamSynchronize(s); t0 = std::chrono::steady_clock::now(); } }
  ~TracePhase() { if (g_trace) { (void)hipStreamSynchronize(stream); fprintf(stderr, "[pco_gfx trace] %-28s %8.3f ms\n", name, std::chrono::duration<double, std::milli>(std::chrono::steady_clock::now() - t0).count()); } }
};

static uint32_t* strict_fell_back_counter(hipStream_t stream) {
  Workspace& w = workspace();
  if (!w.enc_strict.p) { w.enc_strict.ensure(256); PCO_HIP_CHECK(hipMemsetAsync(w.enc_strict.p, 0, 256, stream)); }
  return (uint32_t*)w.enc_strict.p;
}
static void run_encode(size_t n_tasks, const PcoGfxEncodeTask* tasks, std::vector<EncModePlan>& plans, std::vector<EncPage>& pages,
                       const ResolvedConfig& cfg, PcoGfxTaskResult* results, PcoGfxTaskResult* d_results_user, hipStream_t stream,
                       EncWorkspace* ws_out = nullptr, int stop_after = 0 , PcoGfxPageInfo* d_infos = nullptr ) {
  Workspace& wsp = workspace();
  uint64_t n_max = 0, page_max = 0; bool any_sec = false, any_lookback = false, any_conv1 = false;
  for (size_t i = 0; i < n_tasks; i++) {
    n_max = std::max<uint64_t>(n_max, tasks[i].n);
    any_sec |= plans[i].mode_kind != kClassic; any_lookback |= plans[i].delta_kind == kDeltaLookback; any_conv1 |= plans[i].delta_kind == kDeltaConv1;
  }
  for (auto& p : pages) page_max = std::max<uint64_t>(page_max, p.n);
  const size_t n_pages = pages.size();
  EncWorkspace ws{};
  ws.dict = cfg.d_dict;
  ws.n_stride = ((n_max + 255) & ~(uint64_t)255) + 256;
  ws.n_slots = 0;
  ws.slot_of_var[0] = any_lookback ? ws.n_slots++ : 0xffffffffu;
  ws.slot_of_var[1] = ws.n_slots++;
  ws.slot_of_var[2] = any_sec ? ws.n_slots++ : 0xffffffffu;
  const size_t state_bytes = n_tasks * sizeof(EncChunk) + 256;
  bool any_big = false;
  for (size_t i = 0; i < n_tasks; i++) any_big |= (plans[i].ubl_override != 0xffffffffu ? plans[i].ubl_override : choose_unoptimized_bins_log(cfg.level, tasks[i].n)) > kMaxUnoptBinsLog;
  ws.plan_cap = any_big ? kBigBins : kMaxBins;
  const size_t plan_bytes = n_tasks * 3 * plan_bytes_for(ws.plan_cap);
  const size_t off_plans = (n_tasks * sizeof(PcoGfxEncodeTask) + 63) & ~(size_t)63;
  const size_t off_pages = (off_plans + n_tasks * sizeof(EncModePlan) + 63) & ~(size_t)63;
  const size_t off_flags = (off_pages + n_pages * sizeof(EncPage) + 63) & ~(size_t)63;
  const size_t off_slots = off_flags + 64;
  uint8_t* d_small = (uint8_t*)wsp.enc_small.ensure(off_slots + n_tasks * sizeof(uint32_t) + 256);
  ws.need_sort = (uint32_t*)(d_small + off_flags);
  ws.need_full0 = ws.need_sort + 1;
  ws.lat_used = ws.need_sort + 2;
  ws.lat_slot = (uint32_t*)(d_small + off_slots);
  PCO_HIP_CHECK(hipMemsetAsync(ws.need_sort, 0, 12, stream));
  PCO_HIP_CHECK(hipMemsetAsync(ws.lat_slot, 0xff, n_tasks * sizeof(uint32_t), stream));
  PcoGfxEncodeTask* d_tasks = (PcoGfxEncodeTask*)d_small;
  EncModePlan* d_plans = (EncModePlan*)(d_small + off_plans);
  ws.pages = (EncPage*)(d_small + off_pages);
  uint8_t* d_state = (uint8_t*)wsp.enc_state.ensure(state_bytes + plan_bytes);
  ws.chunks = (EncChunk*)d_state;
  ws.plans = d_state + ((n_tasks * sizeof(EncChunk) + 255) & ~(size_t)255);
  ws.lat_esz = 4; for (size_t i = 0; i < n_tasks; i++) if (dtype_bits(tasks[i].dtype) == 64) ws.lat_esz = 8;
  const size_t lat_slot_bytes = (size_t)ws.n_slots * ws.n_stride * ws.lat_esz;
  const bool lat_exact = results != nullptr;
  ws.lat = nullptr; ws.lat2 = nullptr; ws.lat_cap1 = 0;
  if (!lat_exact) { ws.lat_cap1 = (uint32_t)n_tasks; ws.lat = (uint8_t*)wsp.enc_lat.ensure(n_tasks * lat_slot_bytes); ws.lat2 = ws.lat; }
  const size_t sort_bytes = n_tasks * 2 * ws.n_stride * ws.lat_esz;
  const bool sort_upfront = any_lookback || any_conv1 || results == nullptr || stop_after != 0 || cfg.strict_hist;
  ws.sort = sort_upfront ? (uint8_t*)wsp.enc_sort.ensure(sort_bytes) : (uint8_t*)wsp.enc_sort.p;
  ws.dissect = (uint32_t*)wsp.enc_ans.ensure(n_tasks * ws.n_slots * ws.n_stride * 4);
  PcoGfxTaskResult* d_results = d_results_user ? d_results_user : (PcoGfxTaskResult*)wsp.results.ensure(n_pages * sizeof(PcoGfxTaskResult));
  PCO_HIP_CHECK(hipMemcpyAsync(d_tasks, tasks, n_tasks * sizeof(PcoGfxEncodeTask), hipMemcpyHostToDevice, stream));
  PCO_HIP_CHECK(hipMemcpyAsync(d_plans, plans.data(), n_tasks * sizeof(EncModePlan), hipMemcpyHostToDevice, stream));
  PCO_HIP_CHECK(hipMemcpyAsync(ws.pages, pages.data(), n_pages * sizeof(EncPage), hipMemcpyHostToDevice, stream));
  const uint32_t nt = (uint32_t)n_tasks, np = (uint32_t)n_pages;
  uint32_t skip_fast = 0;
  const uint32_t c16_enable = stop_after != 1 ? 1u : 0u;
  PCO_TIMED_LAUNCH("enc_init_kernel", stream, enc_init_kernel, dim3((nt + 63) / 64), dim3(64), 0, stream, ws, d_tasks, d_plans, nt, cfg.level, c16_enable);
  const uint32_t tiles_per_page = (uint32_t)std::max<uint64_t>((page_max + kSplitTile - 1) / kSplitTile, 1);
  if ((uint64_t)np * tiles_per_page >= (1ull << 31)) throw HostError{PCO_GFX_INVALID_ARGUMENT, "too many pages in one call"};
  bool any_full0 = !c16_enable, any_spec = c16_enable != 0;
  size_t n_lookback = 0;
  for (size_t i = 0; i < n_tasks; i++) n_lookback += plans[i].delta_kind == kDeltaLookback;
  any_full0 = any_full0 || n_lookback != 0 || any_big;
  if (c16_enable) PCO_TIMED_LAUNCH("enc_presample_kernel", stream, enc_presample_kernel, dim3(nt), dim3(64), 0, stream, ws, d_tasks, nt);
  PCO_TIMED_LAUNCH("enc_lat_slots_kernel", stream, enc_lat_slots_kernel, dim3((nt + 63) / 64), dim3(64), 0, stream, ws, nt, 0u);
  uint32_t n_full = 0;
  if (lat_exact) {
    uint32_t flags[3] = {0, 0, 0};
    PCO_HIP_CHECK(hipMemcpyAsync(flags, ws.need_sort, 12, hipMemcpyDeviceToHost, stream));
    PCO_HIP_CHECK(hipStreamSynchronize(stream));
    n_full = flags[2];
    any_full0 = n_full != 0; any_spec = c16_enable && n_full < n_tasks;
    ws.lat_cap1 = std::max<uint32_t>(n_full, 1u);
    ws.lat = (uint8_t*)wsp.enc_lat.ensure((size_t)ws.lat_cap1 * lat_slot_bytes);
    ws.lat2 = ws.lat;
  } else if (c16_enable) any_full0 = true;
  if (any_spec) PCO_TIMED_LAUNCH("enc_split_kernel<c16>", stream, (enc_split_kernel<true, false>), dim3(np * tiles_per_page), dim3(256), kSplitLdsBytes, stream, ws, d_tasks, tiles_per_page, 1u, 1u);
  if (any_full0) PCO_TIMED_LAUNCH("enc_split_kernel", stream, (enc_split_kernel<false, false>), dim3(np * tiles_per_page), dim3(256), kSplitLdsBytes, stream, ws, d_tasks, tiles_per_page, 1u, 0u);
  if (any_spec) {
    PCO_TIMED_LAUNCH("enc_lat_slots_kernel", stream, enc_lat_slots_kernel, dim3((nt + 63) / 64), dim3(64), 0, stream, ws, nt, 2u);
    bool any_redo = true;
    if (lat_exact) {
      uint32_t used = 0;
      PCO_HIP_CHECK(hipMemcpyAsync(&used, ws.lat_used, 4, hipMemcpyDeviceToHost, stream));
      PCO_HIP_CHECK(hipStreamSynchronize(stream));
      const uint32_t n_redo = used > ws.lat_cap1 ? used - ws.lat_cap1 : 0u;
      any_redo = used > n_full;
      if (n_redo) ws.lat2 = (uint8_t*)wsp.enc_lat2.ensure((size_t)n_redo * lat_slot_bytes);
    }
    if (any_redo) {
      const uint32_t tpb = 32, bpp = (tiles_per_page + tpb - 1) / tpb;
      PCO_TIMED_LAUNCH("enc_split_kernel(redo)", stream, (enc_split_kernel<false, true>), dim3(np * bpp), dim3(256), kSplitLdsBytes, stream, ws, d_tasks, tiles_per_page, tpb, 2u);
    }
  }
  if (stop_after == 1) { PCO_HIP_CHECK(hipGetLastError()); if (ws_out) *ws_out = ws; return; }
  if (any_conv1) {
    const size_t conv_bytes = (n_tasks * sizeof(EncConv) + 255) & ~(size_t)255;
    uint8_t* d_conv = (uint8_t*)wsp.enc_conv.ensure(conv_bytes + n_pages * kConv1MaxOrder * sizeof(uint32_t) + 256);
    ws.conv = (EncConv*)d_conv; ws.conv_state = (uint32_t*)(d_conv + conv_bytes);
    PCO_TIMED_LAUNCH("enc_conv1_stats_kernel", stream, enc_conv1_stats_kernel, dim3(nt), dim3(kConv1Threads), 0, stream, ws, nt);
    PCO_TIMED_LAUNCH("enc_conv1_solve_kernel", stream, enc_conv1_solve_kernel, dim3(nt), dim3(64), 0, stream, ws, nt);
    PCO_TIMED_LAUNCH("enc_conv1_resid_kernel", stream, enc_conv1_resid_kernel, dim3(np * tiles_per_page), dim3(kConv1Threads), 0, stream, ws, tiles_per_page);
  }
  if (any_lookback) {
    uint32_t wmax = 4; for (size_t i = 0; i < n_tasks; i++) if (plans[i].delta_kind == kDeltaLookback) wmax = std::max(wmax, plans[i].window_n_log);
    const uint64_t stride_u32 = (4ull << wmax) + (1ull << wmax) + 64;
    std::vector<uint32_t> lb_pages;
    uint64_t page_min_lb = ~0ull;
    for (size_t pi = 0; pi < n_pages; pi++) if (plans[pages[pi].chunk].delta_kind == kDeltaLookback && !(pages[pi].flags & kPageFlagMetaOnly)) { lb_pages.push_back((uint32_t)pi); page_min_lb = std::min<uint64_t>(page_min_lb, pages[pi].n); }
    const uint32_t n_lb = (uint32_t)lb_pages.size();
    if (n_lb) {
      uint32_t* d_lb = (uint32_t*)wsp.enc_lb.ensure((size_t)n_lb * stride_u32 * 4 + (size_t)n_lb * 12 + 256);
      uint32_t* d_ids = d_lb + (size_t)n_lb * stride_u32;
      PCO_HIP_CHECK(hipMemcpyAsync(d_ids, lb_pages.data(), (size_t)n_lb * 4, hipMemcpyHostToDevice, stream));
      uint32_t* redo = d_ids + n_lb;
      uint32_t* d_skip = redo + n_lb;
      const bool small = page_max <= kLbPipeSmallMaxPage && wmax <= 13;
      const uint64_t prop_stride = ((page_max + 63) & ~(uint64_t)63) + 64;
      uint16_t* d_props = (uint16_t*)wsp.enc_lbprops.ensure((size_t)n_lb * 6 * prop_stride * 2 + 256);
      static const bool hash_ok = hipFuncSetAttribute((const void*)enc_lookback_hash_kernel, hipFuncAttributeMaxDynamicSharedMemorySize, (int)lh_lds_bytes(15)) == hipSuccess;
      if (!hash_ok) throw HostError{PCO_GFX_DEVICE_ERROR, "cannot reserve LDS for enc_lookback_hash_kernel"};
      PCO_TIMED_LAUNCH("enc_lookback_hash_kernel", stream, enc_lookback_hash_kernel, dim3(2 * n_lb), dim3(kLhThreads), lh_lds_bytes(std::min(wmax, 15u)), stream, ws, (const uint32_t*)d_ids, n_lb, d_props, prop_stride, lh_queue_off(std::min(wmax, 15u)), d_skip);
      int n_cu = 256; { int dev = 0; hipDeviceProp_t pr; if (hipGetDevice(&dev) == hipSuccess && hipGetDeviceProperties(&pr, dev) == hipSuccess && pr.multiProcessorCount > 0) n_cu = pr.multiProcessorCount; }
      const uint32_t per_round = 4u * (uint32_t)n_cu, rounds = (n_lb + per_round - 1) / per_round;
      const uint32_t slots = std::min((n_lb + rounds - 1) / rounds, n_lb);
      typedef LbPipe<false, true, true> PipeF; typedef LbPipe<true, true, true> PipeSF;
      if (small) PCO_TIMED_LAUNCH("enc_lookback_pipe_kernel<small,props,fastd>", stream, (enc_lookback_pipe_kernel<PipeSF>), dim3(slots), dim3(PipeSF::kThreads), PipeSF::kLdsBytes, stream, ws, (const uint32_t*)d_ids, n_lb, d_lb, stride_u32, redo, (const uint16_t*)d_props, prop_stride, (const uint32_t*)d_skip);
      else PCO_TIMED_LAUNCH("enc_lookback_pipe_kernel<props,fastd>", stream, (enc_lookback_pipe_kernel<PipeF>), dim3(slots), dim3(PipeF::kThreads), PipeF::kLdsBytes, stream, ws, (const uint32_t*)d_ids, n_lb, d_lb, stride_u32, redo, (const uint16_t*)d_props, prop_stride, (const uint32_t*)d_skip);
      if (page_min_lb <= kLbSeqMaxPage) {
        const uint32_t n_round = lbseq_round((uint32_t)std::min<uint64_t>(page_max, kLbSeqMaxPage));
        PCO_TIMED_LAUNCH("enc_lookback_seq_kernel", stream, enc_lookback_seq_kernel, dim3(n_lb), dim3(64), lbseq_lds_bytes(n_round), stream, ws, (const uint32_t*)d_ids, n_lb, (const uint16_t*)d_props, prop_stride, (const uint32_t*)d_skip, redo, n_round);
      }
      if (page_max <= kLbSmallMaxPage) PCO_TIMED_LAUNCH("enc_lookback_kernel<small>", stream, (enc_lookback_kernel<LbSmall>), dim3(n_lb), dim3(64), LbSmall::kLbLdsBytes, stream, ws, (const uint32_t*)d_ids, n_lb, d_lb, stride_u32, redo);
      else PCO_TIMED_LAUNCH("enc_lookback_kernel", stream, (enc_lookback_kernel<LbFull>), dim3(n_lb), dim3(64), LbFull::kLbLdsBytes, stream, ws, (const uint32_t*)d_ids, n_lb, d_lb, stride_u32, redo);
    }
  }
  PCO_TIMED_LAUNCH("enc_hist_kernel", stream, enc_hist_kernel, dim3(nt), dim3(256), kHistLdsBytes, stream, ws, nt);
  {
    static const bool wide_ok = hipFuncSetAttribute((const void*)enc_hist_wide_kernel<kWideHistRange>, hipFuncAttributeMaxDynamicSharedMemorySize, (int)hist_lds_bytes(kWideHistRange)) == hipSuccess &&
                                hipFuncSetAttribute((const void*)enc_hist_wide_kernel<kMidHistRange>, hipFuncAttributeMaxDynamicSharedMemorySize, (int)hist_lds_bytes(kMidHistRange)) == hipSuccess;
    if (!wide_ok) throw HostError{PCO_GFX_DEVICE_ERROR, "cannot reserve LDS for enc_hist_wide_kernel"};
    static const bool sort_ok = hipFuncSetAttribute((const void*)enc_hist_sort_kernel, hipFuncAttributeMaxDynamicSharedMemorySize, (int)kHistSortLdsBytes) == hipSuccess;
    if (!sort_ok) throw HostError{PCO_GFX_DEVICE_ERROR, "cannot reserve LDS for enc_hist_sort_kernel"};
    uint64_t max_n = 0; uint32_t small_lds = 0;
    for (size_t i = 0; i < n_tasks; i++) {
      max_n = std::max<uint64_t>(max_n, tasks[i].n);
      const uint32_t kb = dtype_bits(tasks[i].dtype) == 64 ? 8u : 4u;
      small_lds = std::max(small_lds, small_lds_bytes((uint32_t)std::min<uint64_t>(tasks[i].n, kSmallHistCap), kb));
    }
    const bool any_long = max_n > kSmallHistCap;
    bool run_mid = any_long, run_wide = any_long, run_sort = any_long || any_big, run_small = true;
    if (results != nullptr && stop_after == 0) {
      uint32_t flag = 0;
      PCO_HIP_CHECK(hipMemcpyAsync(&flag, ws.need_sort, 4, hipMemcpyDeviceToHost, stream));
      PCO_HIP_CHECK(hipStreamSynchronize(stream));
      run_sort = (flag & 1u) != 0; run_mid = (flag & 2u) != 0; run_wide = (flag & 4u) != 0; run_small = (flag & 8u) != 0;
    }
    if (run_sort && !sort_upfront) ws.sort = (uint8_t*)wsp.enc_sort.ensure(sort_bytes);
    if (run_mid || run_wide || run_small || run_sort) ws.walk = (uint8_t*)wsp.enc_walk.ensure((size_t)nt * 3 * kWalkRecBytes);
    if (run_mid) PCO_TIMED_LAUNCH("enc_hist_wide_kernel<16384>", stream, enc_hist_wide_kernel<kMidHistRange>, dim3(nt), dim3(1024), hist_lds_bytes(kMidHistRange), stream, ws, nt);
    if (run_wide) PCO_TIMED_LAUNCH("enc_hist_wide_kernel<32768>", stream, enc_hist_wide_kernel<kWideHistRange>, dim3(nt), dim3(1024), hist_lds_bytes(kWideHistRange), stream, ws, nt);
    if (run_small) {
      static const bool small_ok = hipFuncSetAttribute((const void*)enc_hist_small_kernel, hipFuncAttributeMaxDynamicSharedMemorySize, (int)small_lds_bytes(kSmallHistCap, 8)) == hipSuccess;
      if (!small_ok) throw HostError{PCO_GFX_DEVICE_ERROR, "cannot reserve LDS for enc_hist_small_kernel"};
      PCO_TIMED_LAUNCH("enc_hist_small_kernel", stream, enc_hist_small_kernel, dim3(nt), dim3(kSelT), small_lds, stream, ws, nt);
    }
    if (run_sort) {
      auto launch_sel = [&](auto kernel, const char* name) {
        if (hipFuncSetAttribute((const void*)kernel, hipFuncAttributeMaxDynamicSharedMemorySize, (int)kSelLdsBytes) != hipSuccess) throw HostError{PCO_GFX_DEVICE_ERROR, "cannot reserve LDS for enc_hist_select_kernel"};
        PCO_TIMED_LAUNCH(name, stream, kernel, dim3(nt), dim3(kSelThr), kSelLdsBytes, stream, ws, nt);
      };
      uint32_t widths = 0;
      for (size_t i = 0; i < n_tasks; i++) widths |= (uint32_t)dtype_bits(tasks[i].dtype);
      if (widths & 64u) launch_sel(enc_hist_select_kernel<uint64_t>, "enc_hist_select_kernel");
      if (widths & 32u) launch_sel(enc_hist_select_kernel<uint32_t>, "enc_hist_select_kernel");
      if (widths & 16u) launch_sel(enc_hist_select_kernel<uint16_t>, "enc_hist_select_kernel");
      if (widths & 8u) launch_sel(enc_hist_select_kernel<uint8_t>, "enc_hist_select_kernel");
      PCO_TIMED_LAUNCH("enc_hist_sort_kernel", stream, enc_hist_sort_kernel, dim3(nt), dim3(256), kHistSortLdsBytes, stream, ws, nt);
    }
    if (ws.walk != nullptr) PCO_TIMED_LAUNCH("enc_hist_walk_kernel", stream, enc_hist_walk_kernel, dim3(nt), dim3(64), kWalkLdsBytes, stream, ws, nt);
    if (cfg.strict_hist) PCO_TIMED_LAUNCH("enc_hist_literal_kernel", stream, enc_hist_literal_kernel, dim3(nt), dim3(64), kLitLdsBytes, stream, ws, nt, strict_fell_back_counter(stream));
  }
  PCO_TIMED_LAUNCH("enc_train_kernel", stream, enc_train_kernel, dim3(nt), dim3(64), kTrainLdsBytes, stream, ws, nt);
  if (any_big) {
    static const bool big_ok = hipFuncSetAttribute((const void*)enc_train_big_kernel, hipFuncAttributeMaxDynamicSharedMemorySize, (int)kTrainBigLdsBytes) == hipSuccess;
    if (!big_ok) throw HostError{PCO_GFX_DEVICE_ERROR, "cannot reserve LDS for enc_train_big_kernel"};
    PCO_TIMED_LAUNCH("enc_train_big_kernel", stream, enc_train_big_kernel, dim3(nt), dim3(1024), kTrainBigLdsBytes, stream, ws, nt);
  }
  if (stop_after == 2) { PCO_HIP_CHECK(hipGetLastError()); if (ws_out) *ws_out = ws; return; }
  uint32_t page_lds = kPageLdsVar + ws.n_slots * page_var_bytes(cfg.level <= 8 ? 10 : kMaxEncTableLog);
  if (any_big) {
    page_lds = kPageLdsVar + std::min<uint32_t>(ws.n_slots, 2) * page_var_bytes(kMaxEncTableLog, kBigBins) + (ws.n_slots > 2 ? page_var_bytes(kMaxEncTableLog) : 0);
    static const bool page_ok = hipFuncSetAttribute((const void*)enc_page_kernel, hipFuncAttributeMaxDynamicSharedMemorySize, 160 * 1024) == hipSuccess;
    if (!page_ok) throw HostError{PCO_GFX_DEVICE_ERROR, "cannot reserve LDS for enc_page_kernel"};
  }
  {
    EncFast fx{};
    const uint64_t max_batches = (page_max + kBatchN - 1) / kBatchN;
    fx.bat_stride = (uint32_t)max_batches + 1;
    fx.runs_per_page = (uint32_t)((max_batches + kRunBatches - 1) / kRunBatches); if (fx.runs_per_page == 0) fx.runs_per_page = 1;
    fx.run_stride = fx.runs_per_page + 1;
    uint32_t max_page_idx = 0; for (auto& pgi : pages) max_page_idx = std::max(max_page_idx, pgi.page_idx);
    fx.stride = ws.n_stride + 16ull * (max_page_idx + 1) + 64;
    fx.sym = (uint8_t*)wsp.enc_sym.ensure(n_tasks * ws.n_slots * fx.stride + 64);
    fx.answ = (uint16_t*)wsp.enc_answ.ensure(n_tasks * ws.n_slots * fx.stride * 2 + 64);
    fx.bat = (uint32_t*)wsp.enc_bat.ensure(n_pages * 3 * (size_t)fx.bat_stride * 8);
    fx.run_start = (uint64_t*)wsp.enc_run.ensure(n_pages * (size_t)fx.run_stride * 8);
    const size_t fstate_bytes = (n_pages * 12 * 4 + 63) & ~(size_t)63, body_bytes = (n_pages * 16 + 63) & ~(size_t)63, wpb_bytes = ((n_pages * (size_t)ws.n_slots + 15) / 16) * 4 + 64;
    fx.fstate = (uint32_t*)wsp.enc_fstate.ensure(fstate_bytes + body_bytes + wpb_bytes);
    const uint64_t n_blocks = (uint64_t)np * fx.runs_per_page;
    if (n_blocks < (1ull << 31)) {
      const uint32_t n_items = np * ws.n_slots;
      const size_t vlut_bytes = n_tasks * (size_t)ws.n_slots * kDirectHistRange * 2;
      uint64_t input_bytes = 0; for (size_t i = 0; i < n_tasks; i++) input_bytes += tasks[i].n * (uint64_t)(dtype_bits(tasks[i].dtype) / 8);
      const bool lookups = vlut_bytes <= std::max<uint64_t>(64ull << 20, input_bytes / 2);
      static const bool walkp_on = env_not_zero("PCO_GFX_WALKP");
      const bool keep_fused = walkp_on && lookups && ws.n_slots == 1;
      fx.fused = n_items > 8192 && !keep_fused ? 2u : 1u;
      if (lookups) fx.fused |= kFusedLookups;
      const bool any_seg = page_max >= (uint64_t)kWsMinBatches * kBatchN && n_items <= kWsMaxItems;
      if (any_seg) fx.fused |= kFusedSegments;
      PCO_TIMED_LAUNCH("enc_dissect_kernel", stream, enc_dissect_kernel, dim3(np * ((fx.runs_per_page + kDisRuns - 1) / kDisRuns)), dim3(256), kDisLdsBytes, stream, ws, fx, np);
      if (fx.fused & kFusedLookups) {
        fx.vlut = (uint16_t*)wsp.enc_vlut.ensure(vlut_bytes + 64);
        PCO_TIMED_LAUNCH("enc_vlut_kernel", stream, enc_vlut_kernel, dim3(nt * 3), dim3(256), 0, stream, ws, fx, nt);
      }
      static const bool walkd_ok = hipFuncSetAttribute((const void*)enc_walkd_kernel, hipFuncAttributeMaxDynamicSharedMemorySize, (int)kWdLdsBytes) == hipSuccess;
      if (!walkd_ok) throw HostError{PCO_GFX_DEVICE_ERROR, "cannot reserve LDS for enc_walkd_kernel"};
      if (any_seg) PCO_TIMED_LAUNCH("enc_walkseg_kernel", stream, enc_walkseg_kernel, dim3(n_items), dim3(128), kWsLdsBytes, stream, ws, fx, np);
      if (walkp_on && !any_seg && (fx.fused & kFusedLookups) != 0) {
// ... 1273 lines not shown
```

### pcodec_amd/csrc/pco_host.h

```cpp
#pragma once
#include <hip/hip_runtime.h>
#include <stdint.h>

#include <algorithm>
#include <cstdlib>
#include <string>
#include <vector>

#include "../../include/pco_gfx.h"

namespace pcogfx {

struct HostError {
  int status;
  std::string msg;
  bool oom = false;
};

void set_error(int status, const std::string& msg);
void clear_error();

inline bool env_is_one(const char* name) { const char* e = std::getenv(name); return e != nullptr && e[0] == '1'; }
inline bool env_not_zero(const char* name) { const char* e = std::getenv(name); return !(e != nullptr && e[0] == '0'); }
inline char env_char(const char* name) { const char* e = std::getenv(name); return e != nullptr ? e[0] : '\0'; }
inline bool env_first_is(const char* name, char c) { const char* e = std::getenv(name); return e != nullptr && e[0] == c; }

#define PCO_HIP_CHECK(expr)                                                                   \
  do {                                                                                        \
    hipError_t _e = (expr);                                                                   \
    if (_e != hipSuccess) throw pcogfx::HostError{PCO_GFX_DEVICE_ERROR, std::string(#expr) + ": " + hipGetErrorString(_e)}; \
  } while (0)

struct DevBuf {
  void* p = nullptr;
  size_t cap = 0;
  void* ensure(size_t bytes) {
    if (bytes > cap) {
      if (p) { (void)hipFree(p); p = nullptr; cap = 0; }
      size_t want = bytes + std::min<size_t>(bytes / 8, (size_t)64 << 20) + 256;
      hipError_t e = hipMalloc(&p, want);
      if (e != hipSuccess) { p = nullptr; (void)hipGetLastError(); throw HostError{PCO_GFX_DEVICE_ERROR, std::string("hipMalloc failed: ") + hipGetErrorString(e), true}; }
      cap = want;
    }
    return p;
  }
  void release() { if (p) (void)hipFree(p); p = nullptr; cap = 0; }
};

struct HostBuf {
  void* p = nullptr;
  size_t cap = 0;
  void* ensure(size_t bytes) {
    if (bytes > cap) {
      if (p) { (void)hipHostFree(p); p = nullptr; cap = 0; }
      size_t want = bytes + bytes / 8 + 256;
      hipError_t e = hipHostMalloc(&p, want, hipHostMallocDefault);
      if (e != hipSuccess) { p = nullptr; (void)hipGetLastError(); throw HostError{PCO_GFX_DEVICE_ERROR, std::string("hipHostMalloc failed: ") + hipGetErrorString(e), true}; }
      cap = want;
    }
    return p;
  }
  void release() { if (p) (void)hipHostFree(p); p = nullptr; cap = 0; }
};

struct Workspace {
  int device = -1;
  hipStream_t last_stream = nullptr; hipEvent_t last_event = nullptr; bool has_last = false;
  DevBuf tasks, results, tbl_ws;
  DevBuf dec_plans, dec_bins, dec_sym, dec_offpos;
  DevBuf dec_progress;
  DevBuf dec_stats;
  hipStream_t side_stream = nullptr, side_stream2 = nullptr; hipEvent_t fork_event = nullptr, join_event = nullptr, join_event2 = nullptr;
  int n_cus = 0;
  DevBuf dec_hist;
  DevBuf io_in, io_out;
  DevBuf compact_tasks;
  DevBuf enc_state;
  DevBuf enc_lat, enc_lat2, enc_sort, enc_ans, enc_small, enc_lb, enc_walk;
  DevBuf enc_lbprops;
  DevBuf enc_sym, enc_answ, enc_bat, enc_run, enc_fstate, enc_vlut;
  DevBuf enc_strict;
  DevBuf enc_conv;
  DevBuf enc_dict, enc_dict_hbm;
  DevBuf auto_idx, auto_samp, auto_tasks, auto_sum, auto_log2;
  HostBuf h_samp, h_sum;
#define PCO_WS_BUFS(X) X(tasks) X(results) X(tbl_ws) X(dec_plans) X(dec_bins) X(dec_sym) X(dec_offpos) X(dec_progress) X(dec_stats) X(dec_hist) X(io_in) X(io_out) X(compact_tasks) X(enc_state) \
  X(enc_lat) X(enc_lat2) X(enc_sort) X(enc_ans) X(enc_small) X(enc_lb) X(enc_lbprops) X(enc_walk) X(enc_sym) X(enc_answ) X(enc_bat) X(enc_run) X(enc_fstate) X(enc_vlut) X(enc_strict) X(enc_conv) X(enc_dict) X(enc_dict_hbm) X(auto_idx) X(auto_samp) X(auto_tasks) X(auto_sum) X(auto_log2)
  size_t device_bytes() const {
    size_t b = 0;
#define PCO_WS_ADD(name) b += name.cap;
    PCO_WS_BUFS(PCO_WS_ADD)
#undef PCO_WS_ADD
    return b;
  }
  std::string device_report() const {
    std::string r;
#define PCO_WS_REP(name) if (name.cap) r += std::string(#name) + "=" + std::to_string(name.cap) + " ";
    PCO_WS_BUFS(PCO_WS_REP)
#undef PCO_WS_REP
    return r;
  }
  unsigned long long acc_givebacks = 0, acc_marked = 0, acc_strict = 0;
  void fold_counters() {
    uint32_t v[2] = {0, 0};
    if (dec_stats.p && hipMemcpy(v, dec_stats.p, 8, hipMemcpyDeviceToHost) == hipSuccess) { acc_givebacks += v[0]; acc_marked += v[1]; }
    uint32_t f = 0;
    if (enc_strict.p && hipMemcpy(&f, enc_strict.p, 4, hipMemcpyDeviceToHost) == hipSuccess) acc_strict += f;
  }
  void release_all() {
    fold_counters();
    if (side_stream) { (void)hipStreamSynchronize(side_stream); (void)hipStreamDestroy(side_stream); side_stream = nullptr; }
    if (side_stream2) { (void)hipStreamSynchronize(side_stream2); (void)hipStreamDestroy(side_stream2); side_stream2 = nullptr; }
    if (fork_event) { (void)hipEventDestroy(fork_event); fork_event = nullptr; }
    if (join_event) { (void)hipEventDestroy(join_event); join_event = nullptr; }
    if (join_event2) { (void)hipEventDestroy(join_event2); join_event2 = nullptr; }
    tasks.release(); results.release(); tbl_ws.release(); dec_plans.release(); dec_bins.release(); dec_sym.release(); dec_offpos.release(); dec_progress.release(); dec_stats.release(); dec_hist.release(); io_in.release(); io_out.release(); compact_tasks.release();
    enc_state.release(); enc_lat.release(); enc_lat2.release(); enc_sort.release(); enc_ans.release(); enc_small.release(); enc_lb.release(); enc_lbprops.release(); enc_walk.release(); enc_sym.release(); enc_answ.release(); enc_bat.release(); enc_run.release(); enc_fstate.release(); enc_vlut.release(); enc_strict.release(); enc_conv.release(); enc_dict.release(); enc_dict_hbm.release(); auto_idx.release(); auto_samp.release(); auto_tasks.release(); auto_sum.release(); auto_log2.release(); h_samp.release(); h_sum.release();
  }
};
Workspace& workspace();
struct WorkspaceUse {
  Workspace& ws; hipStream_t stream;
  WorkspaceUse(Workspace& w, hipStream_t s) : ws(w), stream(s) {
    if (ws.has_last && ws.last_stream != stream && ws.last_event) (void)hipStreamWaitEvent(stream, ws.last_event, 0);
  }
  ~WorkspaceUse() {
    if (!ws.last_event && hipEventCreateWithFlags(&ws.last_event, hipEventDisableTiming) != hipSuccess) { ws.last_event = nullptr; return; }
    if (hipEventRecord(ws.last_event, stream) == hipSuccess) { ws.last_stream = stream; ws.has_last = true; }
  }
};

struct HostBitWriter {
  std::vector<uint8_t> buf;
  uint64_t bit = 0;
  void write(uint64_t v, uint32_t n) {
    if (n == 0) return;
    if (n < 64) v &= ((uint64_t)1 << n) - 1;
    size_t need = (size_t)((bit + n + 7) >> 3) + 9;
    if (buf.size() < need) buf.resize(need * 2, 0);
    for (uint32_t i = 0; i < n;) {
      size_t byte = (size_t)(bit >> 3); uint32_t sh = (uint32_t)(bit & 7);
      uint32_t take = 8 - sh; if (take > n - i) take = n - i;
      buf[byte] |= (uint8_t)(((v >> i) & ((1u << take) - 1)) << sh);
      i += take; bit += take;
    }
  }
  void finish_byte() { bit = (bit + 7) & ~(uint64_t)7; }
  size_t bytes() const { return (size_t)((bit + 7) >> 3); }
};

size_t guarantee_wrapped_chunk_size(int latent_bits, size_t n);
size_t guarantee_standalone_chunk_size(int latent_bits, size_t n);
size_t guarantee_standalone_header_size();
bool n_per_page(uint64_t max_page_n, size_t n, std::vector<size_t>& out);

}
```

Before: 1695.

## Fuse histogram counting into the c16 split kernel via per-block LDS partial counts

The presample kernel now estimates a narrow 4096-key window for each classic-mode chunk. A new split kernel variant processes several tiles per block and accumulates packed u16 histogram counts in LDS alongside the split, writing per-block partials to global memory. The histogram stage then sums these partials instead of rescanning the latents, with a fallback when keys fall outside the window. This adds workspace, a fused kernel with more LDS use and fewer blocks, and fallback bookkeeping counters.

```diff
diff --git a/include/pco_gfx.h b/include/pco_gfx.h
--- a/include/pco_gfx.h
+++ b/include/pco_gfx.h
@@ -141,6 +141,7 @@
 void pco_gfx_release_workspace(void);
 size_t pco_gfx_workspace_bytes(void);
 unsigned long long pco_gfx_strict_histogram_fallbacks(void);
+unsigned long long pco_gfx_split_count_stat(int which);
 unsigned long long pco_gfx_trail_givebacks(void);
 unsigned long long pco_gfx_trail_marked(void);
 
diff --git a/pcodec_amd/_lib.py b/pcodec_amd/_lib.py
--- a/pcodec_amd/_lib.py
+++ b/pcodec_amd/_lib.py
@@ -99,6 +99,8 @@
         L.pco_gfx_workspace_bytes.argtypes = []
         L.pco_gfx_strict_histogram_fallbacks.restype = C.c_ulonglong
         L.pco_gfx_strict_histogram_fallbacks.argtypes = []
+        L.pco_gfx_split_count_stat.restype = C.c_ulonglong
+        L.pco_gfx_split_count_stat.argtypes = [C.c_int]
         L.pco_gfx_trail_givebacks.restype = C.c_ulonglong
         L.pco_gfx_trail_givebacks.argtypes = []
         L.pco_gfx_trail_marked.restype = C.c_ulonglong
diff --git a/pcodec_amd/csrc/encode_kernels.hip b/pcodec_amd/csrc/encode_kernels.hip
--- a/pcodec_amd/csrc/encode_kernels.hip
+++ b/pcodec_amd/csrc/encode_kernels.hip
@@ -41,6 +41,10 @@
   EncVar v[3];
   uint32_t dict_dtype;
   uint32_t dict_k;
+  uint32_t cnt_state;
+  uint32_t cnt_lo;
+  uint32_t cnt_slot;
+  uint32_t pad_cnt;
 };
 static_assert(sizeof(EncChunk) % 8 == 0, "EncChunk");
 
@@ -115,6 +119,11 @@
   EncConv* conv;
   uint32_t* conv_state;
   DictTask* dict;
+  uint32_t* cnt_part;
+  uint32_t* cnt_used;
+  uint32_t* cnt_stats;
+  uint32_t cnt_blocks;
+  uint32_t cnt_tiles;
 };
 
 __device__ __forceinline__ uint8_t PCO_LDS* enc_lds_base() {
@@ -285,9 +294,16 @@
 constexpr uint32_t kSplitLdsPrev = 0;
 constexpr uint32_t kSplitLdsRed = 257 * 7 * 8;
 constexpr uint32_t kSplitLdsBytes = kSplitLdsRed + 128;
-
-template <class L, int MODE, bool kSpec>
-__device__ __forceinline__ void enc_split_body(const EncWorkspace& ws, const PcoGfxEncodeTask& task, uint32_t t, EncPage PCO_GLOBAL* pg, uint32_t tile) {
+constexpr uint32_t kSplitCntBytes = kDirectHistRange * 2;
+constexpr uint32_t kSplitCountTiles = 16;
+static_assert(kSplitCountTiles * kSplitTile < 65536, "a u16 counter of enc_split_count_kernel must hold a block's keys");
+__host__ __device__ constexpr uint32_t split_count_lds_bytes(uint32_t hs) { return kSplitCntBytes + 257 * hs * 8 + 128; }
+
+template <class L, int MODE, bool kSpec, bool kCount = false>
+__device__ __forceinline__ void enc_split_body(const EncWorkspace& ws, const PcoGfxEncodeTask& task, uint32_t t, EncPage PCO_GLOBAL* pg, uint32_t tile,
+                                               uint32_t hs = 7, uint32_t cnt_lo = 0, bool* flagged = nullptr) {
+  static_assert(!kCount || kSpec, "the count rides on the 16-bit keys");
+  const uint32_t prev_off = kCount ? kSplitCntBytes : kSplitLdsPrev, red_off = kCount ? kSplitCntBytes + 257 * hs * 8 : kSplitLdsRed;
   EncChunk PCO_GLOBAL* ch = (EncChunk PCO_GLOBAL*)ws.chunks + t;
   const uint64_t n = uni((uint64_t)pg->n), pstart = uni((uint64_t)pg->start);
   const uint32_t num_kind = dtype_kind(uni(task.dtype));
@@ -321,13 +337,13 @@
 #pragma unroll
   for (uint32_t jj = 0; jj < 7; jj++) a[jj] = 0;
   if (order > 0) {
-    L PCO_LDS* prevbuf = (L PCO_LDS*)(smem + kSplitLdsPrev);
-#pragma unroll
-    for (uint32_t jj = 0; jj < 7; jj++) if (jj + order >= 7) prevbuf[(tid + 1) * 7 + jj] = a[8 + jj];
-    if (tid >= 249) { L hp = 0, hs; if (halo_on) split_one<L, MODE>(num_kind, mode_base, mode_k, aux_inv, aux_base, halo_raw, hp, hs); prevbuf[tid - 249] = hp; }
+    L PCO_LDS* prevbuf = (L PCO_LDS*)(smem + prev_off);
+#pragma unroll
+    for (uint32_t jj = 0; jj < 7; jj++) if (jj + order >= 7) prevbuf[(tid + 1) * hs + jj + hs - 7] = a[8 + jj];
+    if (tid + hs >= 256) { L hp = 0, hsec; if (halo_on) split_one<L, MODE>(num_kind, mode_base, mode_k, aux_inv, aux_base, halo_raw, hp, hsec); prevbuf[tid + hs - 256] = hp; }
     __syncthreads();
 #pragma unroll
-    for (uint32_t jj = 0; jj < 7; jj++) if (jj + order >= 7) a[jj] = prevbuf[tid * 7 + jj];
+    for (uint32_t jj = 0; jj < 7; jj++) if (jj + order >= 7) a[jj] = prevbuf[tid * hs + jj + hs - 7];
     for (uint32_t r = 0; r < order; r++) {
 #pragma unroll
       for (uint32_t idx = 6 + kSplitE; idx >= 1; idx--) a[idx] = (L)(a[idx] - a[idx - 1]);
@@ -367,18 +383,24 @@
     uint16_t PCO_GLOBAL* c2 = has_sec ? clat_ptr(ws, t, 2) + pstart : nullptr;
     uint32_t bad = 0, rmin1 = 0xffffffffu, rmax1 = 0, rmin2 = 0xffffffffu, rmax2 = 0;
     uint16_t w1[kSplitE], w2[kSplitE];
+    uint32_t PCO_LDS* cnt = (uint32_t PCO_LDS*)smem;
 #pragma unroll
     for (uint32_t k = 0; k < kSplitE; k++) {
       const uint64_t i = e0 + k;
       const L t1 = (L)(d[k] - lo1);
       const uint32_t u1 = (uint32_t)t1;
       w1[k] = (uint16_t)u1;
-      if (i < n && i >= order) { if ((uint64_t)t1 >= kC16KeyRange) bad = 1; rmin1 = u1 < rmin1 ? u1 : rmin1; rmax1 = u1 > rmax1 ? u1 : rmax1; }
+      if (i < n && i >= order) { if ((uint64_t)t1 >= kC16KeyRange) bad |= 1u; rmin1 = u1 < rmin1 ? u1 : rmin1; rmax1 = u1 > rmax1 ? u1 : rmax1; }
+      if (kCount && i < n) {
+        const uint32_t cw = (uint32_t)(uint16_t)(w1[k] - (uint16_t)cnt_lo);
+        if (cw < kDirectHistRange) (void)__hip_atomic_fetch_add(&cnt[cw >> 1], 1u << ((cw & 1u) * 16u), __ATOMIC_RELAXED, __HIP_MEMORY_SCOPE_WORKGROUP);
+        else if (i >= order) bad |= 2u;
+      }
       if (has_sec) {
         const L t2 = (L)(sec[k] - lo2);
         const uint32_t u2 = (uint32_t)t2;
         w2[k] = (uint16_t)u2;
-        if (i < n) { if ((uint64_t)t2 >= kC16KeyRange) bad = 1; rmin2 = u2 < rmin2 ? u2 : rmin2; rmax2 = u2 > rmax2 ? u2 : rmax2; }
+        if (i < n) { if ((uint64_t)t2 >= kC16KeyRange) bad |= 1u; rmin2 = u2 < rmin2 ? u2 : rmin2; rmax2 = u2 > rmax2 ? u2 : rmax2; }
       }
     }
     if (full) {
@@ -400,8 +422,8 @@
       rmin1 = wave_reduce_u32(rmin1, umin); rmax1 = wave_reduce_u32(rmax1, umax);
       if (has_sec) { rmin2 = wave_reduce_u32(rmin2, umin); rmax2 = wave_reduce_u32(rmax2, umax); }
     }
-    const uint32_t wbad = __any(bad != 0) ? 1u : 0u;
-    uint32_t PCO_LDS* red32 = (uint32_t PCO_LDS*)(smem + kSplitLdsRed);
+    const uint32_t wbad = (__any((bad & 1u) != 0) ? 1u : 0u) | (kCount && __any((bad & 2u) != 0) ? 2u : 0u);
+    uint32_t PCO_LDS* red32 = (uint32_t PCO_LDS*)(smem + red_off);
     if (lane_id() == 0) { const uint32_t w = tid >> 6; red32[w * 5 + 0] = rmin1; red32[w * 5 + 1] = rmax1; red32[w * 5 + 2] = rmin2; red32[w * 5 + 3] = rmax2; red32[w * 5 + 4] = wbad; }
     __syncthreads();
     if (tid == 0) {
@@ -411,7 +433,8 @@
         m2 = red32[w * 5 + 2] < m2 ? red32[w * 5 + 2] : m2; x2 = red32[w * 5 + 3] > x2 ? red32[w * 5 + 3] : x2;
         anybad |= red32[w * 5 + 4];
       }
-      if (anybad) atomicCAS(&ws.chunks[t].c16_ok, 1u, 2u);
+      if (kCount && (anybad & 2u) && !*flagged) { *flagged = true; if (atomicCAS(&ws.chunks[t].cnt_state, 1u, 2u) == 1u) atomicAdd(ws.cnt_stats + 1, 1u); }
+      if (anybad & 1u) atomicCAS(&ws.chunks[t].c16_ok, 1u, 2u);
       else {
         if (m1 <= x1) { atomicMin((unsigned long long*)&ws.chunks[t].v[1].minv, (unsigned long long)(L)(lo1 + (L)m1)); atomicMax((unsigned long long*)&ws.chunks[t].v[1].maxv, (unsigned long long)(L)(lo1 + (L)x1)); }
         if (has_sec && m2 <= x2) { atomicMin((unsigned long long*)&ws.chunks[t].v[2].minv, (unsigned long long)(L)(lo2 + (L)m2)); atomicMax((unsigned long long*)&ws.chunks[t].v[2].maxv, (unsigned long long)(L)(lo2 + (L)x2)); }
@@ -447,7 +470,7 @@
       L o4 = shfl_idx(mx2, (int)(lane_id() ^ dlt)); mx2 = o4 > mx2 ? o4 : mx2;
     }
   }
-  uint64_t PCO_LDS* red = (uint64_t PCO_LDS*)(smem + kSplitLdsRed);
+  uint64_t PCO_LDS* red = (uint64_t PCO_LDS*)(smem + red_off);
   if (lane_id() == 0) { const uint32_t w = tid >> 6; red[w * 4 + 0] = (uint64_t)mn1; red[w * 4 + 1] = (uint64_t)mx1; red[w * 4 + 2] = (uint64_t)mn2; red[w * 4 + 3] = (uint64_t)mx2; }
   __syncthreads();
   if (tid == 0) {
@@ -478,6 +501,7 @@
   const uint32_t t = uni(pg->chunk);
   if (uni(ws.chunks[t].status) != PCO_GFX_OK) return;
   if (uni(__hip_atomic_load(&ws.chunks[t].c16_ok, __ATOMIC_RELAXED, __HIP_MEMORY_SCOPE_AGENT)) != want) return;
+  if (kSpec && uni(__hip_atomic_load(&ws.chunks[t].cnt_state, __ATOMIC_RELAXED, __HIP_MEMORY_SCOPE_AGENT)) != 0) return;
   const PcoGfxEncodeTask task = tasks[t];
   const int bits = dtype_bits(uni(task.dtype));
   const uint32_t mode_kind = uni(ws.chunks[t].mode_kind);
@@ -498,8 +522,41 @@
   }
 }
 
+__global__ __launch_bounds__(256, 8) void enc_split_count_kernel(EncWorkspace ws, const PcoGfxEncodeTask* tasks, uint32_t tiles_per_page, uint32_t tiles_per_block, uint32_t hs) {
+  const uint32_t blocks_per_page = (tiles_per_page + tiles_per_block - 1) / tiles_per_block;
+  const uint32_t page = blockIdx.x / blocks_per_page, blk = blockIdx.x % blocks_per_page, tile0 = blk * tiles_per_block;
+  EncPage PCO_GLOBAL* pg = (EncPage PCO_GLOBAL*)ws.pages + page;
+  if (uni(pg->flags) & kPageFlagMetaOnly) return;
+  const uint32_t t = uni(pg->chunk);
+  EncChunk PCO_GLOBAL* ch = (EncChunk PCO_GLOBAL*)ws.chunks + t;
+  if (uni(ch->status) != PCO_GFX_OK) return;
+  if (uni(__hip_atomic_load(&ch->cnt_state, __ATOMIC_RELAXED, __HIP_MEMORY_SCOPE_AGENT)) == 0) return;
+  if (uni(__hip_atomic_load(&ch->c16_ok, __ATOMIC_RELAXED, __HIP_MEMORY_SCOPE_AGENT)) != 1) return;
+  const uint64_t pn = uni((uint64_t)pg->n);
+  if ((uint64_t)tile0 * kSplitTile >= pn) return;
+  const PcoGfxEncodeTask task = tasks[t];
+  const int bits = dtype_bits(uni(task.dtype));
+  const uint32_t cnt_lo = uni(ch->cnt_lo);
+  typedef uint32_t u32x4 __attribute__((ext_vector_type(4)));
+  u32x4 PCO_LDS* cnt4 = (u32x4 PCO_LDS*)enc_lds_base();
+  const u32x4 zero4 = {0u, 0u, 0u, 0u};
+  static_assert(kSplitCntBytes == 2 * 256 * 16, "two 16-byte rows of counters per thread");
+  cnt4[threadIdx.x] = zero4; cnt4[threadIdx.x + 256] = zero4;
+  __syncthreads();
+  bool flagged = false;
+  for (uint32_t tile = tile0; tile < tile0 + tiles_per_block && (uint64_t)tile * kSplitTile < pn; tile++) {
+    if (tile != tile0) __syncthreads();
+    if (bits == 64) enc_split_body<uint64_t, kClassic, true, true>(ws, task, t, pg, tile, hs, cnt_lo, &flagged);
+    else if (bits == 32) enc_split_body<uint32_t, kClassic, true, true>(ws, task, t, pg, tile, hs, cnt_lo, &flagged);
+    else if (bits == 16) enc_split_body<uint16_t, kClassic, true, true>(ws, task, t, pg, tile, hs, cnt_lo, &flagged);
+  }
+  __syncthreads();
+  u32x4 PCO_GLOBAL* part = (u32x4 PCO_GLOBAL*)ws.cnt_part + ((uint64_t)uni(ch->cnt_slot) * ws.cnt_blocks + blk) * (kSplitCntBytes / 16);
+  part[threadIdx.x] = cnt4[threadIdx.x]; part[threadIdx.x + 256] = cnt4[threadIdx.x + 256];
+}
+
 template <class L, int MODE>
-__device__ __forceinline__ bool presample_bad(const PcoGfxEncodeTask& task, const EncChunk PCO_GLOBAL* ch) {
+__device__ __forceinline__ bool presample_bad(const PcoGfxEncodeTask& task, const EncChunk PCO_GLOBAL* ch, uint32_t& key1) {
   const uint32_t lane = lane_id();
   const uint32_t num_kind = dtype_kind(uni(task.dtype));
   const uint32_t mode_k = uni(ch->mode_k);
@@ -509,6 +566,7 @@
   const uint64_t n = uni((uint64_t)ch->n);
   const L PCO_GLOBAL* src = (const L PCO_GLOBAL*)task.src;
   constexpr L kBias = sizeof(L) == 1 ? (L)0 : (L)16384, kLmax = (L)~(L)0;
+  key1 = 0;
   if (sizeof(L) == 1) return false;
   auto clamp_ref = [&](L x) { return x < kBias ? kBias : (x > (L)(kLmax - kBias) ? (L)(kLmax - kBias) : x); };
   L ref1 = order > 0 ? lmid<L>() : (L)0, ref2 = 0;
@@ -527,17 +585,18 @@
   for (uint32_t k = 0; k < 8; k++) if (k == order) d = a[k];
   d = (L)(d + (order > 0 ? lmid<L>() : (L)0));
   bool bad = (uint64_t)(L)(d - (L)(ref1 - kBias)) >= kC16KeyRange;
+  key1 = (uint32_t)(uint16_t)(L)(d - (L)(ref1 - kBias));
   if (has_sec) bad = bad || (uint64_t)(L)(sec_last - (L)(ref2 - kBias)) >= kC16KeyRange;
   return __any(bad) != 0;
 }
 template <class L>
-__device__ __forceinline__ bool presample_mode(const PcoGfxEncodeTask& task, const EncChunk PCO_GLOBAL* ch, uint32_t mode_kind) {
-  if (mode_kind == kClassic) return presample_bad<L, kClassic>(task, ch);
-  if (mode_kind == kIntMult) return presample_bad<L, kIntMult>(task, ch);
-  if (mode_kind == kFloatQuant) return presample_bad<L, kFloatQuant>(task, ch);
-  return presample_bad<L, kFloatMult>(task, ch);
-}
-__global__ __launch_bounds__(64) void enc_presample_kernel(EncWorkspace ws, const PcoGfxEncodeTask* tasks, uint32_t n_tasks) {
+__device__ __forceinline__ bool presample_mode(const PcoGfxEncodeTask& task, const EncChunk PCO_GLOBAL* ch, uint32_t mode_kind, uint32_t& key1) {
+  if (mode_kind == kClassic) return presample_bad<L, kClassic>(task, ch, key1);
+  if (mode_kind == kIntMult) return presample_bad<L, kIntMult>(task, ch, key1);
+  if (mode_kind == kFloatQuant) return presample_bad<L, kFloatQuant>(task, ch, key1);
+  return presample_bad<L, kFloatMult>(task, ch, key1);
+}
+__global__ __launch_bounds__(64) void enc_presample_kernel(EncWorkspace ws, const PcoGfxEncodeTask* tasks, uint32_t n_tasks, uint32_t count_enable) {
   const uint32_t t = blockIdx.x;
   if (t >= n_tasks) return;
   EncChunk PCO_GLOBAL* ch = (EncChunk PCO_GLOBAL*)ws.chunks + t;
@@ -546,10 +605,19 @@
   const int bits = dtype_bits(uni(task.dtype));
   const uint32_t mode_kind = uni(ch->mode_kind);
   bool bad = false;
-  if (bits == 64) bad = presample_mode<uint64_t>(task, ch, mode_kind);
-  else if (bits == 32) bad = presample_mode<uint32_t>(task, ch, mode_kind);
-  else if (bits == 16) bad = presample_mode<uint16_t>(task, ch, mode_kind);
+  uint32_t key1 = 0;
+  if (bits == 64) bad = presample_mode<uint64_t>(task, ch, mode_kind, key1);
+  else if (bits == 32) bad = presample_mode<uint32_t>(task, ch, mode_kind, key1);
+  else if (bits == 16) bad = presample_mode<uint16_t>(task, ch, mode_kind, key1);
   if (bad && lane_id() == 0) { ch->c16_ok = 0; atomicAdd(ws.need_full0, 1u); }
+  if (bad || !count_enable || bits < 16 || mode_kind != kClassic || uni(ch->dict_dtype) != 0) return;
+  auto umin = [](uint32_t p, uint32_t q) { return p < q ? p : q; }; auto umax = [](uint32_t p, uint32_t q) { return p > q ? p : q; };
+  const uint32_t kmin = wave_reduce_u32(key1, umin), kmax = wave_reduce_u32(key1, umax);
+  if (kmax - kmin >= kDirectHistRange / 2 || lane_id() != 0) return;
+  const uint32_t mid = (kmin + kmax) >> 1;
+  ch->cnt_lo = mid < kDirectHistRange / 2 ? 0u : (mid - kDirectHistRange / 2 > kC16KeyRange - kDirectHistRange ? kC16KeyRange - kDirectHistRange : mid - kDirectHistRange / 2);
+  ch->cnt_slot = atomicAdd(ws.cnt_used, 1u);
+  ch->cnt_state = 1;
 }
 __global__ __launch_bounds__(64) void enc_lat_slots_kernel(EncWorkspace ws, uint32_t n_tasks, uint32_t want) {
   const uint32_t t = blockIdx.x * blockDim.x + threadIdx.x;
@@ -1141,7 +1209,34 @@
         }
       };
       const bool constant16 = (uint64_t)range == 0 && c16;
+      const bool summed = !kWide && R == kDirectHistRange && c16 && var == 1 && uni(ch->cnt_state) == 1 && !constant16;
+      const uint16_t cnt_lo16 = (uint16_t)uni(ch->cnt_lo);
       if (constant16) { if (tid == 0) counts[0] = n_lat; }
+      else if (summed) {
+        typedef uint32_t u32x4 __attribute__((ext_vector_type(4)));
+        const uint32_t n_tiles = (n_all + kSplitTile - 1) / kSplitTile, n_blk = (n_tiles + ws.cnt_tiles - 1) / ws.cnt_tiles;
+        const u32x4 PCO_GLOBAL* part = (const u32x4 PCO_GLOBAL*)ws.cnt_part + (uint64_t)uni(ch->cnt_slot) * ws.cnt_blocks * (kSplitCntBytes / 16);
+        const uint32_t off = (uint32_t)(uint16_t)(c16_off - cnt_lo16);
+        static_assert(kSplitCntBytes / 16 == 2 * T || R != kDirectHistRange, "two 16-byte rows of the window per thread");
+#pragma unroll 1
+        for (uint32_t h = 0; h < 2; h++) {
+          const uint32_t row = tid + h * T;
+          uint32_t lo[4] = {0, 0, 0, 0}, hi[4] = {0, 0, 0, 0};
+#pragma unroll 4
+          for (uint32_t b = 0; b < n_blk; b++) {
+            const u32x4 v = part[(uint64_t)b * (kSplitCntBytes / 16) + row];
+#pragma unroll
+            for (uint32_t q = 0; q < 4; q++) { lo[q] += v[q] & 0xffffu; hi[q] += v[q] >> 16; }
+          }
+#pragma unroll
+          for (uint32_t q = 0; q < 4; q++) {
+            const uint32_t e = row * 8 + q * 2;
+            if (e >= off) counts[e - off] = lo[q];
+            if (e + 1 >= off) counts[e + 1 - off] = hi[q];
+          }
+        }
+        if (tid == 0) atomicAdd(ws.cnt_stats, 1u);
+      }
       else if (agg) count_all(BoolC<true>{}); else count_all(BoolC<false>{});
       if (skip != 0 && !constant16) {
         __syncthreads();
@@ -1150,7 +1245,8 @@
           const uint64_t pst = pgl[pi].start;
           if (j < (uint64_t)pgl[pi].n) {
             const uint64_t d = c16 ? (uint64_t)(uint16_t)(clat[pst + j] - c16_off) : (uint64_t)(L)(lat[pst + j] - minv);
-            if (d < R) atomicSub((uint32_t*)&counts[(uint32_t)d], 1u);
+            const bool counted = !summed || (uint16_t)(clat[pst + j] - cnt_lo16) < kDirectHistRange;
+            if (d < R && counted) atomicSub((uint32_t*)&counts[(uint32_t)d], 1u);
           }
         }
       }
diff --git a/pcodec_amd/csrc/pco_gfx.hip b/pcodec_amd/csrc/pco_gfx.hip
--- a/pcodec_amd/csrc/pco_gfx.hip
+++ b/pcodec_amd/csrc/pco_gfx.hip
@@ -326,6 +326,17 @@
     return w.acc_strict + v;
   } catch (...) { return 0; }
 }
+unsigned long long pco_gfx_split_count_stat(int which) {
+  try {
+    if (which != 0 && which != 1) return 0;
+    Workspace& w = workspace();
+    if (!w.enc_cntstat.p) return w.acc_cnt[which];
+    if (w.has_last && w.last_event) (void)hipEventSynchronize(w.last_event);
+    uint32_t v[2] = {0, 0};
+    if (hipMemcpy(v, w.enc_cntstat.p, 8, hipMemcpyDeviceToHost) != hipSuccess) return w.acc_cnt[which];
+    return w.acc_cnt[which] + v[which];
+  } catch (...) { return 0; }
+}
 
 void pco_gfx_profile_begin(void) {
   for (auto& r : g_prof.recs) { g_prof.give(r.a); g_prof.give(r.b); }
diff --git a/pcodec_amd/csrc/pco_gfx_encode_api.inc b/pcodec_amd/csrc/pco_gfx_encode_api.inc
--- a/pcodec_amd/csrc/pco_gfx_encode_api.inc
+++ b/pcodec_amd/csrc/pco_gfx_encode_api.inc
@@ -112,6 +112,13 @@
   if (!w.enc_strict.p) { w.enc_strict.ensure(256); PCO_HIP_CHECK(hipMemsetAsync(w.enc_strict.p, 0, 256, stream)); }
   return (uint32_t*)w.enc_strict.p;
 }
+static uint32_t* split_count_counters(hipStream_t stream) {
+  Workspace& w = workspace();
+  if (!w.enc_cntstat.p) { w.enc_cntstat.ensure(256); PCO_HIP_CHECK(hipMemsetAsync(w.enc_cntstat.p, 0, 256, stream)); }
+  return (uint32_t*)w.enc_cntstat.p;
+}
+static uint32_t split_count_tiles_from_env() { const char c = env_char("PCO_GFX_SPLIT_COUNT"); return c == '0' ? 0u : (c == '4' ? 4u : (c == '8' ? 8u : kSplitCountTiles)); }
+static const uint32_t g_split_count_tiles = split_count_tiles_from_env();
 static void run_encode(size_t n_tasks, const PcoGfxEncodeTask* tasks, std::vector<EncModePlan>& plans, std::vector<EncPage>& pages,
                        const ResolvedConfig& cfg, PcoGfxTaskResult* results, PcoGfxTaskResult* d_results_user, hipStream_t stream,
                        EncWorkspace* ws_out = nullptr, int stop_after = 0 , PcoGfxPageInfo* d_infos = nullptr ) {
@@ -143,8 +150,9 @@
   ws.need_sort = (uint32_t*)(d_small + off_flags);
   ws.need_full0 = ws.need_sort + 1;
   ws.lat_used = ws.need_sort + 2;
+  ws.cnt_used = ws.need_sort + 3;
   ws.lat_slot = (uint32_t*)(d_small + off_slots);
-  PCO_HIP_CHECK(hipMemsetAsync(ws.need_sort, 0, 12, stream));
+  PCO_HIP_CHECK(hipMemsetAsync(ws.need_sort, 0, 16, stream));
   PCO_HIP_CHECK(hipMemsetAsync(ws.lat_slot, 0xff, n_tasks * sizeof(uint32_t), stream));
   PcoGfxEncodeTask* d_tasks = (PcoGfxEncodeTask*)d_small;
   EncModePlan* d_plans = (EncModePlan*)(d_small + off_plans);
@@ -175,20 +183,33 @@
   size_t n_lookback = 0;
   for (size_t i = 0; i < n_tasks; i++) n_lookback += plans[i].delta_kind == kDeltaLookback;
   any_full0 = any_full0 || n_lookback != 0 || any_big;
-  if (c16_enable) PCO_TIMED_LAUNCH("enc_presample_kernel", stream, enc_presample_kernel, dim3(nt), dim3(64), 0, stream, ws, d_tasks, nt);
+  size_t n_cnt_max = 0; uint32_t cnt_hs = 0;
+  const uint32_t count_enable = c16_enable && !cfg.strict_hist && ws.dict == nullptr ? g_split_count_tiles : 0u;
+  if (count_enable) for (size_t i = 0; i < n_tasks; i++) {
+    if (plans[i].delta_kind == kDeltaConsecutive) cnt_hs = std::max(cnt_hs, plans[i].delta_order);
+    n_cnt_max += plans[i].n_pages == 1 && plans[i].mode_kind == kClassic && plans[i].delta_kind != kDeltaLookback && plans[i].delta_kind != kDeltaConv1 && dtype_bits(tasks[i].dtype) >= 16 && tasks[i].n >= 4096;
+  }
+  ws.cnt_tiles = count_enable ? count_enable : 1u; ws.cnt_blocks = (tiles_per_page + ws.cnt_tiles - 1) / ws.cnt_tiles;
+  ws.cnt_stats = split_count_counters(stream);
+  const size_t cnt_chunk_bytes = (size_t)ws.cnt_blocks * kSplitCntBytes;
+  uint32_t n_cnt = (uint32_t)n_cnt_max;
+  if (c16_enable) PCO_TIMED_LAUNCH("enc_presample_kernel", stream, enc_presample_kernel, dim3(nt), dim3(64), 0, stream, ws, d_tasks, nt, n_cnt_max != 0 ? 1u : 0u);
   PCO_TIMED_LAUNCH("enc_lat_slots_kernel", stream, enc_lat_slots_kernel, dim3((nt + 63) / 64), dim3(64), 0, stream, ws, nt, 0u);
   uint32_t n_full = 0;
   if (lat_exact) {
-    uint32_t flags[3] = {0, 0, 0};
-    PCO_HIP_CHECK(hipMemcpyAsync(flags, ws.need_sort, 12, hipMemcpyDeviceToHost, stream));
+    uint32_t flags[4] = {0, 0, 0, 0};
+    PCO_HIP_CHECK(hipMemcpyAsync(flags, ws.need_sort, 16, hipMemcpyDeviceToHost, stream));
     PCO_HIP_CHECK(hipStreamSynchronize(stream));
-    n_full = flags[2];
+    n_full = flags[2]; n_cnt = flags[3];
     any_full0 = n_full != 0; any_spec = c16_enable && n_full < n_tasks;
     ws.lat_cap1 = std::max<uint32_t>(n_full, 1u);
     ws.lat = (uint8_t*)wsp.enc_lat.ensure((size_t)ws.lat_cap1 * lat_slot_bytes);
     ws.lat2 = ws.lat;
   } else if (c16_enable) any_full0 = true;
-  if (any_spec) PCO_TIMED_LAUNCH("enc_split_kernel<c16>", stream, (enc_split_kernel<true, false>), dim3(np * tiles_per_page), dim3(256), kSplitLdsBytes, stream, ws, d_tasks, tiles_per_page, 1u, 1u);
+  ws.cnt_part = n_cnt ? (uint32_t*)wsp.enc_cnt.ensure((size_t)n_cnt * cnt_chunk_bytes) : nullptr;
+  if ((uint64_t)np * ws.cnt_blocks >= (1ull << 31)) throw HostError{PCO_GFX_INVALID_ARGUMENT, "too many pages in one call"};
+  if (any_spec && n_cnt) PCO_TIMED_LAUNCH("enc_split_kernel<c16>", stream, enc_split_count_kernel, dim3(np * ws.cnt_blocks), dim3(256), split_count_lds_bytes(cnt_hs), stream, ws, d_tasks, tiles_per_page, ws.cnt_tiles, cnt_hs);
+  if (any_spec && !(lat_exact && (size_t)n_cnt + n_full >= n_tasks)) PCO_TIMED_LAUNCH("enc_split_kernel<c16>", stream, (enc_split_kernel<true, false>), dim3(np * tiles_per_page), dim3(256), kSplitLdsBytes, stream, ws, d_tasks, tiles_per_page, 1u, 1u);
   if (any_full0) PCO_TIMED_LAUNCH("enc_split_kernel", stream, (enc_split_kernel<false, false>), dim3(np * tiles_per_page), dim3(256), kSplitLdsBytes, stream, ws, d_tasks, tiles_per_page, 1u, 0u);
   if (any_spec) {
     PCO_TIMED_LAUNCH("enc_lat_slots_kernel", stream, enc_lat_slots_kernel, dim3((nt + 63) / 64), dim3(64), 0, stream, ws, nt, 2u);
diff --git a/pcodec_amd/csrc/pco_host.h b/pcodec_amd/csrc/pco_host.h
--- a/pcodec_amd/csrc/pco_host.h
+++ b/pcodec_amd/csrc/pco_host.h
@@ -80,12 +80,13 @@
   DevBuf enc_lbprops;
   DevBuf enc_sym, enc_answ, enc_bat, enc_run, enc_fstate, enc_vlut;
   DevBuf enc_strict;
+  DevBuf enc_cnt, enc_cntstat;
   DevBuf enc_conv;
   DevBuf enc_dict, enc_dict_hbm;
   DevBuf auto_idx, auto_samp, auto_tasks, auto_sum, auto_log2;
   HostBuf h_samp, h_sum;
 #define PCO_WS_BUFS(X) X(tasks) X(results) X(tbl_ws) X(dec_plans) X(dec_bins) X(dec_sym) X(dec_offpos) X(dec_progress) X(dec_stats) X(dec_hist) X(io_in) X(io_out) X(compact_tasks) X(enc_state) \
-  X(enc_lat) X(enc_lat2) X(enc_sort) X(enc_ans) X(enc_small) X(enc_lb) X(enc_lbprops) X(enc_walk) X(enc_sym) X(enc_answ) X(enc_bat) X(enc_run) X(enc_fstate) X(enc_vlut) X(enc_strict) X(enc_conv) X(enc_dict) X(enc_dict_hbm) X(auto_idx) X(auto_samp) X(auto_tasks) X(auto_sum) X(auto_log2)
+  X(enc_lat) X(enc_lat2) X(enc_sort) X(enc_ans) X(enc_small) X(enc_lb) X(enc_lbprops) X(enc_walk) X(enc_sym) X(enc_answ) X(enc_bat) X(enc_run) X(enc_fstate) X(enc_vlut) X(enc_strict) X(enc_cnt) X(enc_cntstat) X(enc_conv) X(enc_dict) X(enc_dict_hbm) X(auto_idx) X(auto_samp) X(auto_tasks) X(auto_sum) X(auto_log2)
   size_t device_bytes() const {
     size_t b = 0;
 #define PCO_WS_ADD(name) b += name.cap;
@@ -100,12 +101,14 @@
 #undef PCO_WS_REP
     return r;
   }
-  unsigned long long acc_givebacks = 0, acc_marked = 0, acc_strict = 0;
+  unsigned long long acc_givebacks = 0, acc_marked = 0, acc_strict = 0, acc_cnt[2] = {0, 0};
   void fold_counters() {
     uint32_t v[2] = {0, 0};
     if (dec_stats.p && hipMemcpy(v, dec_stats.p, 8, hipMemcpyDeviceToHost) == hipSuccess) { acc_givebacks += v[0]; acc_marked += v[1]; }
     uint32_t f = 0;
     if (enc_strict.p && hipMemcpy(&f, enc_strict.p, 4, hipMemcpyDeviceToHost) == hipSuccess) acc_strict += f;
+    uint32_t c[2] = {0, 0};
+    if (enc_cntstat.p && hipMemcpy(c, enc_cntstat.p, 8, hipMemcpyDeviceToHost) == hipSuccess) { acc_cnt[0] += c[0]; acc_cnt[1] += c[1]; }
   }
   void release_all() {
     fold_counters();
@@ -115,7 +118,7 @@
     if (join_event) { (void)hipEventDestroy(join_event); join_event = nullptr; }
     if (join_event2) { (void)hipEventDestroy(join_event2); join_event2 = nullptr; }
     tasks.release(); results.release(); tbl_ws.release(); dec_plans.release(); dec_bins.release(); dec_sym.release(); dec_offpos.release(); dec_progress.release(); dec_stats.release(); dec_hist.release(); io_in.release(); io_out.release(); compact_tasks.release();
-    enc_state.release(); enc_lat.release(); enc_lat2.release(); enc_sort.release(); enc_ans.release(); enc_small.release(); enc_lb.release(); enc_lbprops.release(); enc_walk.release(); enc_sym.release(); enc_answ.release(); enc_bat.release(); enc_run.release(); enc_fstate.release(); enc_vlut.release(); enc_strict.release(); enc_conv.release(); enc_dict.release(); enc_dict_hbm.release(); auto_idx.release(); auto_samp.release(); auto_tasks.release(); auto_sum.release(); auto_log2.release(); h_samp.release(); h_sum.release();
+    enc_state.release(); enc_lat.release(); enc_lat2.release(); enc_sort.release(); enc_ans.release(); enc_small.release(); enc_lb.release(); enc_lbprops.release(); enc_walk.release(); enc_sym.release(); enc_answ.release(); enc_bat.release(); enc_run.release(); enc_fstate.release(); enc_vlut.release(); enc_strict.release(); enc_cnt.release(); enc_cntstat.release(); enc_conv.release(); enc_dict.release(); enc_dict_hbm.release(); auto_idx.release(); auto_samp.release(); auto_tasks.release(); auto_sum.release(); auto_log2.release(); h_samp.release(); h_sum.release();
   }
 };
 Workspace& workspace();
```

Result: slower. 1222 (-27.9%).
